# epfl-lasa/OptimalModulationDS

Measured on NVIDIA B200. Metric: mppi_rollout_state_steps_per_sec, higher is better.
Workload: dtype f32 (scoring: split-fp16 tcgen05, fp32 accumulate, fp32-accurate; obstacle-ranking prefilter: f16 tcgen05, re-scored in fp32 inside its calibrated guard band)

## Files before the change

### include/dsmppi_b200.h

```cpp
#ifndef DSMPPI_B200_H
#define DSMPPI_B200_H

#include <stdint.h>

#ifdef __cplusplus
extern "C" {
#endif

#define DSMPPI_N_KERNEL_MAX 50
#define DSMPPI_MAX_DOF 8
#define DSMPPI_MAX_LINKS 16
#define DSMPPI_MAX_CLOSEST 8
#define DSMPPI_HIDDEN 256
#define DSMPPI_MAX_HIDDEN_LAYERS 4

typedef struct dsmppi_ctx dsmppi_ctx;

typedef struct {
  int32_t n_dof;
  int32_t n_out;
  int32_t n_point_dim;
  int16_t n_hidden;
  int16_t hidden_width;
  const float* W_host[5];
  const float* b_host[5];
} dsmppi_net;

enum {
  DSMPPI_DS_LINEAR_ATTRACTOR = 0,
  DSMPPI_DS_MATRIX = 1,
  DSMPPI_DS_SEDS = 2
};
typedef struct {
  int32_t ds_kind;
  int32_t fold_activation;
  float lvel_mid, lvel_k;
  float dist_mid, dist_k;
  float ltau_max;
  float goal_act_thr;
  float repulsion;
  float reserved;
  float ds_A[DSMPPI_MAX_DOF * DSMPPI_MAX_DOF];
} dsmppi_modulation;

enum {
  DSMPPI_PASS1_EXACT_FP32 = 0,
  DSMPPI_PASS1_TC_F16 = 1,
  DSMPPI_PASS1_TC_BF16 = 2,
  DSMPPI_PASS1_AUTO = 3
};

enum {
  DSMPPI_SCORE_FFMA = 0,
  DSMPPI_SCORE_TC_SPLIT = 1,
  DSMPPI_SCORE_AUTO = 2
};

enum {
  DSMPPI_DISTANCE_NN = 0,
  DSMPPI_DISTANCE_FK = 1
};
#define DSMPPI_FK_MAX_PTS 32

typedef struct {
  int32_t N;
  int32_t H;
  int32_t q_cur_is_batch;
  int32_t n_kernels;
  int32_t n_closest;
  uint32_t ignored_link_mask;
  float dt;
  float dst_thr;
  float lin_thr;
  float rbf_p;
  float q_goal[DSMPPI_MAX_DOF];
  dsmppi_modulation mod;
  int32_t distance_provider;
  int32_t fk_n_pts;
  float fk_span[DSMPPI_FK_MAX_PTS];
  const float* q_cur_dev;
  const float* mu_tmp_dev;
  const float* sigma_tmp_dev;
  const float* alpha_tmp_dev;
  float* all_traj_dev;
  float* closest_dist_all_dev;
  float* kernel_val_all_dev;
  float* dot_products_dev;
  float* kernel_activations_dev;
  float* qdot_dev;
  float* nn_grad_all_dev;
  float* norm_basis_dev;
} dsmppi_rollout_args;

enum {
  DSMPPI_COST_JOINT_LIMITS = 1,
  DSMPPI_COST_TERMINAL_FK = 2,
  DSMPPI_COST_ALL = 3
};
typedef struct {
  int32_t N, H;
  int32_t terms;
  int32_t reserved;
  float q_goal[DSMPPI_MAX_DOF];
  float q_min[DSMPPI_MAX_DOF];
  float q_max[DSMPPI_MAX_DOF];
  const float* all_traj_dev;
  const float* closest_dist_all_dev;
  float* cost_dev;
} dsmppi_cost_args;

typedef struct {
  int32_t N, H;
  int32_t n_kernels;
  int32_t owns_sample0;
  int32_t variant;
  int32_t reserved;
  int64_t N_global;
  float ker_thr;
  float upd_rate;
  const float* cost_dev;
  const float* kernel_val_all_dev;
  const float* kernel_activations_dev;
  const float* mu_tmp_dev;
  const float* sigma_tmp_dev;
  const float* alpha_tmp_dev;
  float* mu_c_dev;
  float* sigma_c_dev;
  float* alpha_c_dev;
} dsmppi_update_args;

const char* dsmppi_last_error(void);
int dsmppi_version(void);
void dsmppi_modulation_default(dsmppi_modulation* out);
void dsmppi_modulation_toy(dsmppi_modulation* out);

int dsmppi_ctx_create(dsmppi_ctx** out, const dsmppi_net* net, const float* dh_params_host,
                      int32_t capacity, int32_t device);
int dsmppi_ctx_destroy(dsmppi_ctx* ctx);
int dsmppi_set_pass1_mode(dsmppi_ctx* ctx, int32_t mode, float guard_band);
int dsmppi_set_score_mode(dsmppi_ctx* ctx, int32_t mode);
int dsmppi_set_whole_horizon(dsmppi_ctx* ctx, int32_t on);

int dsmppi_set_obstacles(dsmppi_ctx* ctx, const float* obs_dev, int32_t M, void* stream);
int dsmppi_set_obstacles_host(dsmppi_ctx* ctx, const float* obs_host, int32_t M, void* stream);

typedef struct {
  int32_t n_gaussians;
  float seds_thr;
  const float* priors_host;
  const float* pdf_den_host;
  const float* mu_x_host;
  const float* mu_y_host;
  const float* sigma_inv_host;
  const float* A_host;
} dsmppi_seds;
int dsmppi_set_seds(dsmppi_ctx* ctx, const dsmppi_seds* seds, void* stream);

int dsmppi_rollout(dsmppi_ctx* ctx, const dsmppi_rollout_args* args, void* stream);

int dsmppi_distance_grad(dsmppi_ctx* ctx, const float* q_dev, int32_t n, int32_t n_closest,
                         uint32_t ignored_link_mask, float* distance_dev, float* nn_grad_dev, void* stream);

int dsmppi_distance_grad_fk(dsmppi_ctx* ctx, const float* q_dev, int32_t n, int32_t fk_n_pts, const float* span_host,
                            float* distance_dev, float* grad_dev, int32_t* closest_idx_dev, void* stream);

int dsmppi_debug_pass1(dsmppi_ctx* ctx, const float* q_dev, int32_t n, uint32_t ignored_link_mask, int32_t mode,
                       float* out_dev, void* stream);

int dsmppi_norm_basis(dsmppi_ctx* ctx, const float* grad_dev, int64_t n, float* basis_dev, void* stream);

int dsmppi_cost(dsmppi_ctx* ctx, const dsmppi_cost_args* args, void* stream);

int32_t dsmppi_update_packed_len(int32_t n_kernels, int32_t n_dof);
int dsmppi_update_cost_stats(dsmppi_ctx* ctx, const float* cost_dev, int32_t N, float* stats_dev, void* stream);
int dsmppi_update_partial(dsmppi_ctx* ctx, const dsmppi_update_args* args, const float* stats_dev,
                          float* packed_dev, void* stream);
int dsmppi_update_finalize(dsmppi_ctx* ctx, const dsmppi_update_args* args, const float* packed_dev,
                           int32_t* n_updated_dev, void* stream);

typedef struct {
  int32_t N, H;
  int32_t n_kernels;
  float rbf_p;
  float thr_dist, thr_kernel, thr_dot;
  const float* all_traj_dev;
  const float* closest_dist_all_dev;
  const float* dot_products_dev;
  const float* mu_c_dev;
  const float* sigma_c_dev;
  int32_t* out_index_dev;
  int32_t* count_dev;
  int64_t capacity;
} dsmppi_candidates_args;
int dsmppi_kernel_candidates(dsmppi_ctx* ctx, const dsmppi_candidates_args* args, void* stream);

enum { DSMPPI_EXCHANGE_COST_STATS = 0, DSMPPI_EXCHANGE_PACKED_SUMS = 1 };
typedef int (*dsmppi_exchange_fn)(void* user, int32_t phase);
typedef struct {
  dsmppi_rollout_args rollout;
  float q_min[DSMPPI_MAX_DOF];
  float q_max[DSMPPI_MAX_DOF];
  float ker_thr, upd_rate;
  int32_t cost_terms;
  int32_t update_variant;
  const float* q_cur_host;
  const float* mu_tmp_host;
  const float* sigma_tmp_host;
  const float* alpha_tmp_host;
  float* mu_c_host;
  float* sigma_c_host;
  float* alpha_c_host;
  float* all_traj_host;
  float* closest_dist_all_host;
  float* kernel_val_all_host;
  float* dot_products_host;
  float* kernel_activations_host;
  float* qdot_host;
  float* cost_host;
  int32_t* n_updated_host;
  int64_t h2d_bytes, d2h_bytes;
  dsmppi_exchange_fn exchange;
  void* exchange_user;
  float* stats_dev;
  float* packed_dev;
  int32_t owns_sample0;
  int32_t reserved2;
  int64_t N_global;
} dsmppi_iteration_host_args;
int dsmppi_iteration_host(dsmppi_ctx* ctx, dsmppi_iteration_host_args* args, void* stream);

typedef struct {
  dsmppi_rollout_args rollout;
  int32_t n_obs;
  int32_t reserved;
  const float* q_cur_host;
  const float* obs_host;
  const float* mu_tmp_host;
  const float* sigma_tmp_host;
  const float* alpha_tmp_host;
  float* all_traj_host;
  float* closest_dist_all_host;
  float* kernel_val_all_host;
  float* dot_products_host;
  float* kernel_activations_host;
  float* qdot_host;
  float* nn_grad_all_host;
  int32_t recaptured;
  int32_t reserved2;
} dsmppi_tick_args;
int dsmppi_tick(dsmppi_ctx* ctx, dsmppi_tick_args* args, void* stream);

int64_t dsmppi_launch_count(const dsmppi_ctx* ctx);
int dsmppi_pass1_stats(dsmppi_ctx* ctx, int64_t* rescored_pairs, int64_t* band_overflows, int32_t* mode,
                       void* stream);
int dsmppi_exactness_stats(dsmppi_ctx* ctx, int64_t* capacity_retries, int64_t* exact_fallbacks, float* guard_band,
                           float* calibration_error);
int dsmppi_score_stats(dsmppi_ctx* ctx, int32_t* mode, int64_t* range_fixup_rows, int64_t* dropped_rows, void* stream);
int dsmppi_enable_kernel_timing(dsmppi_ctx* ctx, int32_t on);
int dsmppi_kernel_timing(dsmppi_ctx* ctx, double* pass1_ms_per_launch, int32_t* pass1_launches,
                         double* exact_ms_per_launch, int32_t* exact_launches);
int dsmppi_kernel_timing_ex(dsmppi_ctx* ctx, int32_t* kind, double* ms_per_launch, int32_t* launches);

#ifdef __cplusplus
}
#endif
#endif
```

### optimalmodulationds_b200/MPPI.py

```python
import contextlib
import os
import time
from math import pi

import numpy as np
import torch
from torch.profiler import ProfilerActivity, profile, record_function

from . import _capi
from .cost import Cost
from .fk_num import *
from .policy import *
from .policy import TensorPolicyMPPI


def generalized_sigmoid(x, y_min, y_max, x0, x1, k):
    return y_min + (y_max - y_min) / (1 + torch.exp(k * (-x + (x0 + x1) / 2)))


_ROLLOUT_TAGS = ("TAG: Nominal vector field", "TAG: evaluate NN", "TAG: evaluate NN_2 (forward pass)",
                 "TAG: evaluate NN_3 (get closest obstacle)", "TAG: evaluate NN_4 (forward+backward pass)",
                 "TAG: evaluate NN_5 (process outputs)", "TAG: QR decomposition", "TAG: Modulation-propagation",
                 "TAG: Apply policies", "TAG: Apply policy", "TAG: Propagate")
_DISTANCE_TAGS = ("TAG: evaluate NN_1 (build input)",) + _ROLLOUT_TAGS[2:6]


@contextlib.contextmanager
def _stage_tags(names):
    if not torch.autograd._profiler_enabled():
        yield
        return
    with contextlib.ExitStack() as stack:
        for n in names:
            stack.enter_context(record_function(n))
        yield


_NET_FAMILY = ("the supported distance networks are 3(d+P) -> W -> ... -> W -> O MLPs without skips: 1 to 4 hidden "
               "layers of one width W <= 256, O <= 16 outputs")


def _network_arrays(nn_model):
    if len(getattr(nn_model.model, 'skips', ()) or ()) > 0:
        raise NotImplementedError(f"skip connections are not supported; {_NET_FAMILY}")
    lin = [m for m in nn_model.model.modules() if isinstance(m, torch.nn.Linear)]
    W = [m.weight.detach().to('cpu', torch.float32).contiguous() for m in lin]
    b = [m.bias.detach().to('cpu', torch.float32).contiguous() for m in lin]
    L = len(W) - 1
    if not 1 <= L <= _capi.MAX_HIDDEN_LAYERS:
        raise NotImplementedError(f"found {max(L, 0)} hidden layers; {_NET_FAMILY}")
    width = W[0].shape[0]
    shapes = [(width, 3 * nn_model.in_channels)] + [(width, width)] * (L - 1) + [(nn_model.out_channels, width)]
    if [tuple(w.shape) for w in W] != shapes or not 1 <= width <= _capi.MAX_HIDDEN \
            or not 1 <= nn_model.out_channels <= _capi.MAX_LINKS:
        raise NotImplementedError(f"layer shapes {[tuple(w.shape) for w in W]}; {_NET_FAMILY}")
    return W, b


class MPPI:
    _TOY = False
    _COST_TERMS = _capi.COST_ALL
    _UPDATE_VARIANT = 0
    _DEFAULT_DST_THR = 0.5
    _COST_CLASS = Cost

    def __init__(self, q0: torch.Tensor, qf: torch.Tensor, dh_params: torch.Tensor, obs: torch.Tensor, dt: float,
                 dt_H: int, N_traj: int, DS_ARRAY, dh_a, nn_model, n_closest_obs):
        self.tensor_args = {'device': q0.device, 'dtype': q0.dtype}
        if q0.dtype != torch.float32:
            raise NotImplementedError("the CUDA path computes in fp32 (as every reference script does)")
        if not torch.cuda.is_available():
            raise RuntimeError("optimalmodulationds_b200.MPPI needs a CUDA device (B200); there is no CPU fallback")
        self._lib = _capi.load()
        if q0.is_cuda:
            self._dev = q0.device
        else:
            self._dev = torch.device('cuda', int(os.environ.get('DSMPPI_DEVICE', os.environ.get('LOCAL_RANK', 0))))
        self.n_dof = q0.shape[0]
        self.Policy = TensorPolicyMPPI(N_traj, self.n_dof, self.tensor_args)
        self.Policy._backend = self
        self.q0 = q0
        self.DS_idx = 0
        self.DS_ARRAY = DS_ARRAY
        self.DS = DS_ARRAY[self.DS_idx]
        self.qf = self.DS.q_goal.squeeze()
        self.dh_params = dh_params
        self.obs = obs
        self.n_obs = obs.shape[0]
        self.dt = dt
        self.dt_H = dt_H
        self.N_traj = N_traj
        self.dh_a = dh_a
        self.nn_model = nn_model
        self.q_cur = q0
        self.policy_upd_rate = 0.1
        self.dst_thr = self._DEFAULT_DST_THR
        self.ker_thr = 1e-3
        self.ignored_links = [0, 1, 2] if self.n_dof >= 7 else []
        self.n_closest_obs = n_closest_obs
        self.distance_provider = 'nn'
        self.fk_n_pts = 10
        self.traj_range = torch.arange(self.N_traj, device=q0.device)
        self.kernel_obstacle_bases_tmp = torch.zeros((self.Policy.N_KERNEL_MAX, self.n_dof, self.n_dof),
                                                     **self.tensor_args)
        self._shard = None
        self._mirror = {}
        self._norm_basis = None
        self._ctx = None
        self._make_context()
        self.Cost = self._COST_CLASS(self.qf, self.dh_params, backend=self)
        self.reset_tensors()
        self.qdot = torch.zeros((self.N_traj, self.n_dof), **self.tensor_args)
        self.nn_grad = torch.zeros(N_traj, self.n_dof, **self.tensor_args)
        self.ker_w = torch.zeros((N_traj, 0, 1), **self.tensor_args)
        self.cur_cost = torch.zeros(N_traj, **self.tensor_args)
        for _ in range(5):
            self.Policy.sample_policy()
        self.propagate()

    def _make_context(self):
        W, b = _network_arrays(self.nn_model)
        self._point_dim = int(self.nn_model.in_channels) - self.n_dof
        if self._point_dim not in (2, 3):
            raise ValueError(f"network takes {self.nn_model.in_channels} inputs, q0 has {self.n_dof} joints: "
                             "expected n_dof + 3 (or n_dof + 2 for the planar toy net)")
        net = _capi.Net()
        net.n_dof, net.n_out, net.n_point_dim = self.n_dof, self.nn_model.out_channels, self._point_dim
        net.n_hidden, net.hidden_width = len(W) - 1, W[0].shape[0]
        for i in range(len(W)):
            net.W_host[i] = W[i].data_ptr()
            net.b_host[i] = b[i].data_ptr()
        dh = self.dh_params.detach().to('cpu', torch.float32).contiguous()
        if dh.dim() != 2 or dh.shape[1] != 4 or dh.shape[0] < self.n_dof + 1:
            raise ValueError("dh_params must be (n_dof + 1, 4) = [d, theta, a, alpha]")
        dh = dh[:self.n_dof + 1].contiguous()
        handle = _capi.C.c_void_p()
        with torch.cuda.device(self._dev):
            _capi.check(self._lib.dsmppi_ctx_create(_capi.C.byref(handle), _capi.C.byref(net), dh.data_ptr(),
                                                    int(self.N_traj), int(self._dev.index or 0)))
        self._ctx = handle

    def __del__(self):
        ctx, self._ctx = getattr(self, '_ctx', None), None
        if ctx:
            try:
                self._lib.dsmppi_ctx_destroy(ctx)
            except Exception:
                pass

    def _stream(self):
        return _capi.C.c_void_p(torch.cuda.current_stream(self._dev).cuda_stream)

    def _host_vec(self, t):
        if isinstance(t, torch.Tensor):
            cache = self.__dict__.setdefault('_hostvec_cache', {})
            hit = cache.get(id(t))
            if hit is not None and hit[0] is t and hit[1] == t._version:
                return hit[2]
            vals = t.detach().reshape(-1).to('cpu', torch.float32).tolist()
            if len(cache) > 64:
                cache.clear()
            cache[id(t)] = (t, t._version, vals)
            return vals
        return torch.as_tensor(t).detach().reshape(-1).to('cpu', torch.float32).tolist()

    def _d(self, t):
        return torch.as_tensor(t).detach().to(self._dev, torch.float32).contiguous()

    def _u(self, t):
        return t if t.device == self.tensor_args['device'] else t.to(self.tensor_args['device'])

    def _dev_of(self, user_tensor):
        hit = self._mirror.get(id(user_tensor))
        if hit is not None and hit[0] is user_tensor and hit[1] == user_tensor._version:
            return hit[2]
        return self._d(user_tensor)

    def _remember(self, user_tensor, dev_tensor):
        self._mirror[id(user_tensor)] = (user_tensor, user_tensor._version, dev_tensor)

    def set_pass1_mode(self, mode='auto', guard_band=0.0):
        code = {'exact': _capi.PASS1_EXACT_FP32, 'tc_f16': _capi.PASS1_TC_F16, 'tc_bf16': _capi.PASS1_TC_BF16,
                'auto': _capi.PASS1_AUTO}[mode]
        _capi.check(self._lib.dsmppi_set_pass1_mode(self._ctx, code, float(guard_band)))
        self._pass1_forced = mode
        self.__dict__.pop('_tick', None)

    def set_score_mode(self, mode='auto'):
        code = {'ffma': _capi.SCORE_FFMA, 'tc_split': _capi.SCORE_TC_SPLIT, 'auto': _capi.SCORE_AUTO}[mode]
        _capi.check(self._lib.dsmppi_set_score_mode(self._ctx, code))
        self.__dict__.pop('_tick', None)

    def score_stats(self):
        mode, fix, drop = _capi.C.c_int32(), _capi.C.c_int64(), _capi.C.c_int64()
        _capi.check(self._lib.dsmppi_score_stats(self._ctx, _capi.C.byref(mode), _capi.C.byref(fix),
                                                 _capi.C.byref(drop), self._stream()))
        return dict(mode={_capi.SCORE_FFMA: 'ffma', _capi.SCORE_TC_SPLIT: 'tc_split'}[mode.value],
                    range_fixup_rows=fix.value, dropped_rows=drop.value)

    def set_whole_horizon(self, on=True):
        _capi.check(self._lib.dsmppi_set_whole_horizon(self._ctx, 1 if on else 0))
        self.__dict__.pop('_tick', None)

    def _upload_obstacles(self):
        src = self.obs
        hit = getattr(self, '_obs_uploaded', None)
        if (hit is not None and isinstance(src, torch.Tensor) and hit[0] is src and hit[1] == src._version):
            return hit[2]
        obs = self._d(self.obs)
        if obs.dim() != 2 or obs.shape[1] != self._point_dim + 1:
            raise ValueError("obs must be (M, 4) = [x, y, z, r]" if self._point_dim == 3 else
                             "obs must be (M, 3) = [x, y, r] for a network with n_dof + 2 inputs")
        self.n_obs = obs.shape[0]
        _capi.check(self._lib.dsmppi_set_obstacles(self._ctx, obs.data_ptr(), int(obs.shape[0]), self._stream()))
        if isinstance(src, torch.Tensor):
            self._obs_uploaded = (src, src._version, obs)
        return obs

    def _ignore_mask(self):
        mask = 0
        for link in self.ignored_links:
            mask |= 1 << int(link)
        return mask

    def reset_DS(self, DS):
        self.DS = DS
        self.qf = DS.q_goal.squeeze()
        self._rebuild_cost()

    def switch_DS_idx(self, idx):
        self.DS_idx = idx
        self.DS = self.DS_ARRAY[idx]
        self.qf = self.DS.q_goal.squeeze()
        self._rebuild_cost()

    def _rebuild_cost(self):
        old = getattr(self, 'Cost', None)
        self.Cost = self._COST_CLASS(self.qf, self.dh_params, backend=self)
        if old is not None:
            self.Cost.q_min, self.Cost.q_max = old.q_min, old.q_max

    def reset_tensors(self):
        N, H, d = self.N_traj, self.dt_H, self.n_dof
        a = self.tensor_args
        self.all_traj = torch.zeros(N, H, d, **a)
        self.closest_dist_all = 100 + torch.zeros(N, H, **a)
        self.kernel_val_all = torch.zeros(N, H, self.Policy.N_KERNEL_MAX, **a)
        self.dot_products = torch.zeros(N, H, **a)
        self.kernel_activations = torch.zeros(N, H, **a)

    def build_nn_input(self, q_tens, obs_tens):
        self.nn_input = torch.hstack((q_tens.tile(obs_tens.shape[0], 1), obs_tens.repeat_interleave(q_tens.shape[0], 0)))
        return self.nn_input

    def _modulation(self, mod):
        if self._TOY:
            self._lib.dsmppi_modulation_toy(_capi.C.byref(mod))
        else:
            self._lib.dsmppi_modulation_default(_capi.C.byref(mod))
        if hasattr(self.DS, 'Mu') and hasattr(self.DS, 'Sigma'):
            mod.ds_kind = _capi.DS_SEDS
            self._upload_seds(self.DS)
        elif hasattr(self.DS, 'lin_thr'):
            mod.ds_kind = _capi.DS_LINEAR_ATTRACTOR
        elif hasattr(self.DS, 'A'):
            mod.ds_kind = _capi.DS_MATRIX
            A = torch.as_tensor(self.DS.A).detach().to('cpu', torch.float32)
            if A.shape != (self.n_dof, self.n_dof):
                raise ValueError("the matrix DS needs A of shape (n_dof, n_dof)")
            for r in range(self.n_dof):
                for c in range(self.n_dof):
                    mod.ds_A[r * _capi.MAX_DOF + c] = float(A[r, c])
        else:
            raise NotImplementedError("the CUDA rollout implements the LinDS attractor (LinDS.py), the SEDS mixture "
                                      "(SEDS.py) and the matrix DS v = (q - qf) @ A (MPPI_toy.py:89) as nominal "
                                      "dynamics")

    def _upload_seds(self, ds):
        if getattr(self, '_seds_uploaded', None) is ds:
            return
        from .SEDS import SEDS as _SEDS
        src = ds if isinstance(ds, _SEDS) else _SEDS.from_arrays(ds.Mu, ds.Sigma, ds.Priors, ds.q_goal)
        if src.dof != self.n_dof:
            raise ValueError(f"SEDS has {src.dof} joints, the robot {self.n_dof}")
        arrs = [t.detach().to('cpu', torch.float32).contiguous() for t in src.kernel_arrays()]
        sd = _capi.Seds()
        sd.n_gaussians, sd.seds_thr = int(src.n_gaussians), float(getattr(ds, 'seds_thr', 1e-2))
        (sd.priors_host, sd.pdf_den_host, sd.mu_x_host, sd.mu_y_host, sd.sigma_inv_host,
         sd.A_host) = (t.data_ptr() for t in arrs)
        with torch.cuda.device(self._dev):
            _capi.check(self._lib.dsmppi_set_seds(self._ctx, _capi.C.byref(sd), self._stream()))
        self._seds_uploaded = ds

    def _rollout_args(self, N, H, nk, q_cur, mu, sigma, alpha, out):
        a = _capi.RolloutArgs()
        a.N, a.H, a.n_kernels, a.n_closest = N, H, nk, int(self.n_closest_obs)
        a.q_cur_is_batch = 1 if q_cur.dim() == 2 else 0
        a.ignored_link_mask = self._ignore_mask()
        a.dt, a.dst_thr = float(self.dt), float(self.dst_thr)
        self._modulation(a.mod)
        if self.distance_provider == 'fk':
            a.distance_provider, a.fk_n_pts = _capi.DISTANCE_FK, int(self.fk_n_pts)
            for i, v in enumerate(torch.linspace(0.01, 1, int(self.fk_n_pts)).tolist()):
                a.fk_span[i] = v
        elif self.distance_provider != 'nn':
            raise ValueError("distance_provider must be 'nn' or 'fk'")
        a.lin_thr, a.rbf_p = float(getattr(self.DS, 'lin_thr', 0.0)), float(self.Policy.p)
        goal = self._host_vec(self.DS.q_goal)
        for i in range(self.n_dof):
            a.q_goal[i] = goal[i]
        a.q_cur_dev = q_cur.data_ptr()
        a.mu_tmp_dev, a.sigma_tmp_dev, a.alpha_tmp_dev = mu.data_ptr(), sigma.data_ptr(), alpha.data_ptr()
        a.all_traj_dev = out['all_traj'].data_ptr()
        a.closest_dist_all_dev = out['closest'].data_ptr()
        a.kernel_val_all_dev = out['kval'].data_ptr()
        a.dot_products_dev = out['dots'].data_ptr()
        a.kernel_activations_dev = out['acts'].data_ptr()
        a.qdot_dev = out['qdot'].data_ptr()
        a.nn_grad_all_dev = out['grads'].data_ptr()
        a.norm_basis_dev = None
        return a

    _TICK_MAX_STATE_STEPS = 4096

    def _tick_eligible(self, q_cur):
        if os.environ.get('DSMPPI_GRAPH_TICK', '1') == '0' or self.tensor_args['device'].type != 'cpu':
            return False
        if self.N_traj * self.dt_H > self._TICK_MAX_STATE_STEPS or self.distance_provider != 'nn':
            return False
        if self._shard is not None or hasattr(self.DS, 'Mu') or getattr(self, '_timing_on', False):
            return False
        if int(self.obs.shape[0]) >= 64 or getattr(self, '_pass1_forced', 'auto') not in ('auto', 'exact'):
            return False
        obs = self.obs
        return (isinstance(obs, torch.Tensor) and obs.dim() == 2 and obs.shape[1] == self._point_dim + 1
                and obs.dtype == torch.float32 and q_cur.dtype == torch.float32)

    def _tick_key(self, nk, q_batch):
        DS = self.DS
        A = getattr(DS, 'A', None)
        return (nk, q_batch, int(self.n_closest_obs), self._ignore_mask(), float(self.dt), float(self.dst_thr),
                float(self.Policy.p), type(DS), tuple(self._host_vec(DS.q_goal)), float(getattr(DS, 'lin_thr', 0.0)),
                None if A is None else tuple(self._host_vec(A)))

    def _propagate_tick(self, q_cur_user, nk):
        N, H, d = self.N_traj, self.dt_H, self.n_dof
        P = self.Policy
        q_batch = q_cur_user.dim() == 2
        key = self._tick_key(nk, q_batch)
        t = self.__dict__.get('_tick')
        if t is None or t['key'] != key:
            dummy = torch.empty(1, device=self._dev)
            probe = torch.empty((N, d) if q_batch else (d,), device='meta')
            out = {k: dummy for k in ('all_traj', 'closest', 'kval', 'dots', 'acts', 'qdot', 'grads')}
            ta = _capi.TickArgs()
            ta.rollout = self._rollout_args(N, H, nk, dummy, dummy, dummy, dummy, out)
            ta.rollout.q_cur_is_batch = 1 if probe.dim() == 2 else 0
            t = self._tick = dict(key=key, args=ta, keep=dummy)
        ta = t['args']
        obs = self.obs if self.obs.is_contiguous() else self.obs.contiguous()
        q = q_cur_user if q_cur_user.is_contiguous() else q_cur_user.contiguous()
        ta.n_obs = int(obs.shape[0])
        ta.q_cur_host, ta.obs_host = q.data_ptr(), obs.data_ptr()
        mu, sg, al = P.mu_tmp, P.sigma_tmp, P.alpha_tmp
        if nk > 0:
            if not (mu.is_contiguous() and sg.is_contiguous() and al.is_contiguous()):
                mu, sg, al = mu.contiguous(), sg.contiguous(), al.contiguous()
            ta.mu_tmp_host, ta.sigma_tmp_host, ta.alpha_tmp_host = mu.data_ptr(), sg.data_ptr(), al.data_ptr()
        traj, closest, kv = torch.empty(N, H, d), torch.empty(N, H), torch.empty(N, H, P.N_KERNEL_MAX)
        dots, acts, qdot, grads = torch.empty(N, H), torch.empty(N, H), torch.empty(N, d), torch.empty(N, H, d)
        ta.all_traj_host, ta.closest_dist_all_host, ta.kernel_val_all_host = traj.data_ptr(), closest.data_ptr(), kv.data_ptr()
        ta.dot_products_host, ta.kernel_activations_host = dots.data_ptr(), acts.data_ptr()
        ta.qdot_host, ta.nn_grad_all_host = qdot.data_ptr(), grads.data_ptr()
        _capi.check(self._lib.dsmppi_tick(self._ctx, _capi.C.byref(ta), self._stream()))
        self._mirror = {}
        self._obs_uploaded = None
        self._norm_basis = None
        self._dev_last = dict(grads=None, grads_host=grads, nk=nk)
        self.all_traj, self.closest_dist_all, self.kernel_val_all = traj, closest, kv
        self.dot_products, self.kernel_activations, self.qdot = dots, acts, qdot
        self.nn_grad = grads[:, H - 1, :]
        self.ker_w = kv[:, H - 1, :nk].unsqueeze(2)
        return (traj, closest, kv[:, :, 0:nk], dots, acts)

    def propagate(self):
        N, H, d = self.N_traj, self.dt_H, self.n_dof
        P = self.Policy
        nk = int(P.n_kernels)
        dev = self._dev
        q_user = torch.as_tensor(self.q_cur)
        if self._tick_eligible(q_user):
            if q_user.shape not in ((d,), (N, d)):
                raise ValueError(f"q_cur must be ({d},) or ({N}, {d}), got {tuple(q_user.shape)}")
            with _stage_tags(_ROLLOUT_TAGS):
                return self._propagate_tick(q_user, nk)
        with torch.cuda.device(dev):
            q_cur = self._d(self.q_cur)
            if q_cur.shape not in ((d,), (N, d)):
                raise ValueError(f"q_cur must be ({d},) or ({N}, {d}), got {tuple(q_cur.shape)}")
            mu, sigma, alpha = self._d(P.mu_tmp), self._d(P.sigma_tmp), self._d(P.alpha_tmp)
            if mu.shape != (N, P.N_KERNEL_MAX, d):
                raise ValueError("Policy.mu_tmp must be (N_traj, 50, n_dof)")
            self._upload_obstacles()
            out = dict(all_traj=torch.empty(N, H, d, device=dev), closest=torch.empty(N, H, device=dev),
                       kval=torch.zeros(N, H, P.N_KERNEL_MAX, device=dev), dots=torch.empty(N, H, device=dev),
                       acts=torch.empty(N, H, device=dev), qdot=torch.empty(N, d, device=dev),
                       grads=torch.empty(N, H, d, device=dev))
            args = self._rollout_args(N, H, nk, q_cur, mu, sigma, alpha, out)
            with _stage_tags(_ROLLOUT_TAGS):
                _capi.check(self._lib.dsmppi_rollout(self._ctx, _capi.C.byref(args), self._stream()))
        self._mirror = {}
        self._dev_last = dict(out, mu=mu, sigma=sigma, alpha=alpha, nk=nk)
        self._norm_basis = None
        if self.tensor_args['device'] == dev:
            self.all_traj, self.closest_dist_all, self.kernel_val_all = out['all_traj'], out['closest'], out['kval']
            self.dot_products, self.kernel_activations, self.qdot = out['dots'], out['acts'], out['qdot']
        else:
            self.all_traj, self.closest_dist_all = self._u(out['all_traj']), self._u(out['closest'])
            self.dot_products, self.kernel_activations = self._u(out['dots']), self._u(out['acts'])
            self.qdot = self._u(out['qdot'])
            kv = torch.zeros(N, H, P.N_KERNEL_MAX, **self.tensor_args)
            if nk > 0:
                kv[:, :, :nk] = self._u(out['kval'][:, :, :nk])
            self.kernel_val_all = kv
        for user, key in ((self.all_traj, 'all_traj'), (self.closest_dist_all, 'closest'),
                          (self.kernel_val_all, 'kval'), (self.kernel_activations, 'acts')):
            self._remember(user, out[key])
        self._remember(P.mu_tmp, mu), self._remember(P.sigma_tmp, sigma), self._remember(P.alpha_tmp, alpha)
        self.nn_grad = self._u(out['grads'][:, H - 1, :])
        self.ker_w = self.kernel_val_all[:, H - 1, :nk].unsqueeze(2)
        return (self.all_traj, self.closest_dist_all, self.kernel_val_all[:, :, 0:nk], self.dot_products,
                self.kernel_activations)

    @property
    def norm_basis(self):
        if self._norm_basis is None:
            g = self._dev_last['grads']
            if g is None:
                g = self._d(self._dev_last['grads_host'])
            N, H, d = g.shape
            with torch.cuda.device(self._dev):
                E = torch.empty(N, H, d, d, device=self._dev)
                _capi.check(self._lib.dsmppi_norm_basis(self._ctx, g.data_ptr(), N * H, E.data_ptr(), self._stream()))
            self._norm_basis = self._u(E)
        return self._norm_basis

    @norm_basis.setter
    def norm_basis(self, value):
        self._norm_basis = value

    def distance_repulsion_nn(self, q_prev, aot=False):
        q = self._d(q_prev)
        n = q.shape[0]
        with torch.cuda.device(self._dev):
            self._upload_obstacles()
            dist = torch.empty(n, device=self._dev)
            grad = torch.empty(n, self.n_dof, device=self._dev)
            with _stage_tags(_DISTANCE_TAGS):
                _capi.check(self._lib.dsmppi_distance_grad(self._ctx, q.data_ptr(), n, int(self.n_closest_obs),
                                                           self._ignore_mask(), dist.data_ptr(), grad.data_ptr(),
                                                           self._stream()))
        self.nn_grad = self._u(grad)
        return self._u(dist), self.nn_grad

    def distance_repulsion_fk(self, q_prev, return_indices=False):
        q = self._d(q_prev)
        n = q.shape[0]
        n_pts = int(self.fk_n_pts)
        span = torch.linspace(0.01, 1, n_pts).contiguous()
        with torch.cuda.device(self._dev):
            self._upload_obstacles()
            dist = torch.empty(n, device=self._dev)
            grad = torch.empty(n, self.n_dof, device=self._dev)
            idx = torch.empty(n, 3, dtype=torch.int32, device=self._dev)
            _capi.check(self._lib.dsmppi_distance_grad_fk(self._ctx, q.data_ptr(), n, n_pts, span.data_ptr(),
                                                          dist.data_ptr(), grad.data_ptr(), idx.data_ptr(),
                                                          self._stream()))
        rep = torch.zeros(n, max(7, self.n_dof), device=self._dev)
        rep[:, :self.n_dof] = grad
        rep = self._u(rep)
        self.nn_grad = rep[:, 0:self.n_dof]
        if return_indices:
            return self._u(dist), rep, self._u(idx)
        return self._u(dist), rep

    def update_kernel_normal_bases(self):
        nk = int(self.Policy.n_kernels)
        if nk > 0:
            _, grad = self.distance_repulsion_nn(self.Policy.mu_c[0:nk], aot=False)
            g = self._d(grad)
            with torch.cuda.device(self._dev):
                E = torch.empty(nk, self.n_dof, self.n_dof, device=self._dev)
                _capi.check(self._lib.dsmppi_norm_basis(self._ctx, g.data_ptr(), nk, E.data_ptr(), self._stream()))
            self.Policy.kernel_obstacle_bases[0:nk] = E.to(self.Policy.kernel_obstacle_bases.device)
        return 0

    def evaluate_costs(self, cost_obj, all_traj, closest_dist_all):
        N, H, d = all_traj.shape
        a = _capi.CostArgs()
        a.N, a.H, a.terms = N, H, self._COST_TERMS
        goal, qmin, qmax = self._host_vec(cost_obj.qf), self._host_vec(cost_obj.q_min), self._host_vec(cost_obj.q_max)
        if len(qmin) < d or len(qmax) < d:
            raise ValueError("Cost.q_min / q_max must have n_dof entries")
        for i in range(d):
            a.q_goal[i], a.q_min[i], a.q_max[i] = goal[i], qmin[i], qmax[i]
        with torch.cuda.device(self._dev):
            tr, cd = self._dev_of(all_traj), self._dev_of(closest_dist_all)
            cost = torch.empty(N, device=self._dev)
            a.all_traj_dev, a.closest_dist_all_dev, a.cost_dev = tr.data_ptr(), cd.data_ptr(), cost.data_ptr()
            _capi.check(self._lib.dsmppi_cost(self._ctx, _capi.C.byref(a), self._stream()))
        user = self._u(cost)
        self._remember(user, cost)
        return user

    def kernel_candidates(self, policy, all_traj, closest_dist_all, dot_products, thr_dist, thr_kernel, thr_dot):
        N, H, d = all_traj.shape
        nk = int(policy.n_kernels)
        a = _capi.CandidatesArgs()
        a.N, a.H, a.n_kernels, a.rbf_p = N, H, nk, float(policy.p)
        a.thr_dist, a.thr_kernel, a.thr_dot = float(thr_dist), float(thr_kernel), float(thr_dot)
        with torch.cuda.device(self._dev):
            tr, cd, dp = self._dev_of(all_traj), self._dev_of(closest_dist_all), self._dev_of(dot_products)
            mu_c, sigma_c = self._d(policy.mu_c), self._d(policy.sigma_c)
            count = torch.zeros(1, dtype=torch.int32, device=self._dev)
            cap = min(N * H, 1 << 20)
            while True:
                idx = torch.empty(cap, dtype=torch.int32, device=self._dev)
                a.all_traj_dev, a.closest_dist_all_dev, a.dot_products_dev = tr.data_ptr(), cd.data_ptr(), dp.data_ptr()
                a.mu_c_dev, a.sigma_c_dev = mu_c.data_ptr(), sigma_c.data_ptr()
                a.out_index_dev, a.count_dev, a.capacity = idx.data_ptr(), count.data_ptr(), cap
                _capi.check(self._lib.dsmppi_kernel_candidates(self._ctx, _capi.C.byref(a), self._stream()))
                n = int(count.item())
                if n <= cap:
                    break
                cap = N * H
            order = torch.sort(idx[:n].long())[0]
            cand = tr.reshape(-1, d)[order]
        return self._u(cand)

    def get_cost(self):
        self.cur_cost = self.Cost.evaluate_costs(self.all_traj, self.closest_dist_all)
        return self.cur_cost

    def get_qdot(self, mode='best'):
        qdot = 0
        if mode == 'best':
            qdot = self.qdot[torch.argmin(self.cur_cost), :]
        elif mode == 'weighted':
            beta = self.cur_cost.mean() / 50
            w = torch.exp(-1 / beta * self.cur_cost)
            w = w / w.sum()
            qdot = torch.sum(w.unsqueeze(1) * self.qdot, dim=0)
        return qdot

    def enable_sample_sharding(self, group=None):
        import torch.distributed as dist
        world = dist.get_world_size(group)
        n = torch.tensor([float(self.N_traj)], device=self._dev)
        dist.all_reduce(n, group=group)
        self._shard = dict(group=group, rank=dist.get_rank(group), world=world, N_global=int(round(float(n))))

    def shift_policy_means(self):
        P = self.Policy
        nk = int(P.n_kernels)
        N, H, d = self.N_traj, self.dt_H, self.n_dof
        dev = self._dev
        with torch.cuda.device(dev):
            a = _capi.UpdateArgs()
            a.N, a.H, a.n_kernels = N, H, nk
            a.owns_sample0, a.N_global, a.variant = 1, N, self._UPDATE_VARIANT
            a.ker_thr, a.upd_rate = float(self.ker_thr), float(self.policy_upd_rate)
            cost = self._dev_of(self.cur_cost)
            kv, acts = self._dev_of(self.kernel_val_all), self._dev_of(self.kernel_activations)
            mu, sigma, alpha = self._dev_of(P.mu_tmp), self._dev_of(P.sigma_tmp), self._dev_of(P.alpha_tmp)
            mu_c, sigma_c, alpha_c = (self._d(t).clone() for t in (P.mu_c, P.sigma_c, P.alpha_c))
            a.cost_dev, a.kernel_val_all_dev, a.kernel_activations_dev = cost.data_ptr(), kv.data_ptr(), acts.data_ptr()
            a.mu_tmp_dev, a.sigma_tmp_dev, a.alpha_tmp_dev = mu.data_ptr(), sigma.data_ptr(), alpha.data_ptr()
            a.mu_c_dev, a.sigma_c_dev, a.alpha_c_dev = mu_c.data_ptr(), sigma_c.data_ptr(), alpha_c.data_ptr()
            stats = torch.empty(4, device=dev)
            packed = torch.empty(int(self._lib.dsmppi_update_packed_len(nk, d)), device=dev)
            n_upd = torch.zeros(1, dtype=torch.int32, device=dev)
            st = self._stream()
            _capi.check(self._lib.dsmppi_update_cost_stats(self._ctx, cost.data_ptr(), N, stats.data_ptr(), st))
            if self._shard is not None:
                from .parallel import allreduce_cost_stats, allreduce_packed
                a.owns_sample0 = 1 if self._shard['rank'] == 0 else 0
                a.N_global = self._shard['N_global']
                allreduce_cost_stats(stats, self._shard['group'])
            _capi.check(self._lib.dsmppi_update_partial(self._ctx, _capi.C.byref(a), stats.data_ptr(),
                                                        packed.data_ptr(), st))
            if self._shard is not None:
                allreduce_packed(packed, self._shard['group'])
            _capi.check(self._lib.dsmppi_update_finalize(self._ctx, _capi.C.byref(a), packed.data_ptr(),
                                                         n_upd.data_ptr(), st))
        if nk > 0:
            P.mu_c[0:nk] = mu_c[0:nk].to(P.mu_c.device)
            P.sigma_c[0:nk] = sigma_c[0:nk].to(P.sigma_c.device)
            P.alpha_c[0:nk] = alpha_c[0:nk].to(P.alpha_c.device)
        self._last_stats = stats
        return 0, n_upd.to(self.tensor_args['device'])[0].to(torch.int64)

    def iteration_host(self, host):
        N, H, d = self.N_traj, self.dt_H, self.n_dof
        P = self.Policy
        a = _capi.IterationHostArgs()
        dummy = torch.empty(1, device=self._dev)
        out = {k: dummy for k in ('all_traj', 'closest', 'kval', 'dots', 'acts', 'qdot', 'grads')}
        r = self._rollout_args(N, H, int(P.n_kernels), host['q_cur'], dummy, dummy, dummy, out)
        a.rollout = r
        qmin, qmax = self._host_vec(self.Cost.q_min), self._host_vec(self.Cost.q_max)
        for i in range(d):
            a.q_min[i], a.q_max[i] = qmin[i], qmax[i]
        a.ker_thr, a.upd_rate = float(self.ker_thr), float(self.policy_upd_rate)
        a.cost_terms, a.update_variant = self._COST_TERMS, self._UPDATE_VARIANT
        for name in ('q_cur', 'mu_tmp', 'sigma_tmp', 'alpha_tmp', 'mu_c', 'sigma_c', 'alpha_c', 'all_traj',
                     'closest_dist_all', 'kernel_val_all', 'dot_products', 'kernel_activations', 'qdot', 'cost',
                     'n_updated'):
            t = host[name]
            assert t.device.type == 'cpu' and t.is_contiguous(), name
            setattr(a, name + '_host', t.data_ptr())
        with torch.cuda.device(self._dev):
            self._upload_obstacles()
            if self._shard is not None:
                from .parallel import allreduce_cost_stats, allreduce_packed
                group = self._shard['group']
                stats = torch.empty(4, device=self._dev)
                packed = torch.empty(int(self._lib.dsmppi_update_packed_len(int(P.n_kernels), d)), device=self._dev)

                def exchange(_user, phase):
                    try:
                        if phase == _capi.EXCHANGE_COST_STATS:
                            allreduce_cost_stats(stats, group)
                        else:
                            allreduce_packed(packed, group)
                        return 0
                    except Exception:
                        import traceback
                        traceback.print_exc()
                        return 1
                hook = _capi.ExchangeFn(exchange)
                a.exchange, a.stats_dev, a.packed_dev = hook, stats.data_ptr(), packed.data_ptr()
                a.owns_sample0 = 1 if self._shard['rank'] == 0 else 0
                a.N_global = self._shard['N_global']
            _capi.check(self._lib.dsmppi_iteration_host(self._ctx, _capi.C.byref(a), self._stream()))
        return int(a.h2d_bytes), int(a.d2h_bytes)

    def update_obstacles(self, obs):
        self.obs = obs
        self.n_obs = obs.shape[0]
        return 0

    def launch_count(self):
        return int(self._lib.dsmppi_launch_count(self._ctx))

    def exactness_stats(self):
        r, f, g, e = _capi.C.c_int64(), _capi.C.c_int64(), _capi.C.c_float(), _capi.C.c_float()
        _capi.check(self._lib.dsmppi_exactness_stats(self._ctx, _capi.C.byref(r), _capi.C.byref(f), _capi.C.byref(g),
                                                     _capi.C.byref(e)))
        return dict(capacity_retries=r.value, exact_fallbacks=f.value, guard_band=g.value, calibration_error=e.value)

    def pass1_stats(self):
        a, b, m = _capi.C.c_int64(), _capi.C.c_int64(), _capi.C.c_int32()
        _capi.check(self._lib.dsmppi_pass1_stats(self._ctx, _capi.C.byref(a), _capi.C.byref(b), _capi.C.byref(m),
                                                 self._stream()))
        return dict(rescored_pairs=a.value, band_overflows=b.value, mode=m.value)

    def debug_pass1(self, q, mode='exact'):
        code = {'exact': _capi.PASS1_EXACT_FP32, 'tc_f16': _capi.PASS1_TC_F16, 'tc_bf16': _capi.PASS1_TC_BF16}[mode]
        qd = self._d(q)
        with torch.cuda.device(self._dev):
            obs = self._upload_obstacles()
            out = torch.empty(qd.shape[0], obs.shape[0], device=self._dev)
            _capi.check(self._lib.dsmppi_debug_pass1(self._ctx, qd.data_ptr(), int(qd.shape[0]), self._ignore_mask(),
                                                     code, out.data_ptr(), self._stream()))
        return out

    def enable_kernel_timing(self, on=True):
        _capi.check(self._lib.dsmppi_enable_kernel_timing(self._ctx, 1 if on else 0))
        self._timing_on = bool(on)

    def kernel_timing_ex(self):
        k, ms, n = _capi.C.c_int32(), _capi.C.c_double(), _capi.C.c_int32()
        _capi.check(self._lib.dsmppi_kernel_timing_ex(self._ctx, _capi.C.byref(k), _capi.C.byref(ms), _capi.C.byref(n)))
        name = {0: 'exact_mlp_kernel', 1: 'tc_pass1_kernel', 2: 'rollout_fused_kernel', 3: 'tc_exact_kernel',
                4: 'tc_exact_kernel<whole horizon>'}[k.value]
        return dict(kernel=name, ms=ms.value, launches=n.value)

    def kernel_timing(self):
        p, pn, e, en = _capi.C.c_double(), _capi.C.c_int32(), _capi.C.c_double(), _capi.C.c_int32()
        _capi.check(self._lib.dsmppi_kernel_timing(self._ctx, _capi.C.byref(p), _capi.C.byref(pn), _capi.C.byref(e),
                                                   _capi.C.byref(en)))
        return dict(pass1_ms=p.value, pass1_launches=pn.value, exact_ms=e.value, exact_launches=en.value)
```

### optimalmodulationds_b200/_capi.py

```python
import ctypes as C
import os

_HERE = os.path.dirname(os.path.abspath(__file__))
LIB_PATH = os.environ.get("DSMPPI_LIB") or os.path.join(_HERE, "libdsmppi_b200.so")

N_KERNEL_MAX = 50
MAX_DOF = 8
MAX_LINKS = 16
MAX_CLOSEST = 8
MAX_HIDDEN = 256
MAX_HIDDEN_LAYERS = 4

PASS1_EXACT_FP32, PASS1_TC_F16, PASS1_TC_BF16, PASS1_AUTO = 0, 1, 2, 3
SCORE_FFMA, SCORE_TC_SPLIT, SCORE_AUTO = 0, 1, 2

_fp = C.c_void_p


DS_LINEAR_ATTRACTOR, DS_MATRIX, DS_SEDS = 0, 1, 2
DISTANCE_NN, DISTANCE_FK = 0, 1
FK_MAX_PTS = 32
COST_JOINT_LIMITS, COST_TERMINAL_FK, COST_ALL = 1, 2, 3


class Net(C.Structure):
    _fields_ = [("n_dof", C.c_int32), ("n_out", C.c_int32), ("n_point_dim", C.c_int32),
                ("n_hidden", C.c_int16), ("hidden_width", C.c_int16),
                ("W_host", _fp * 5), ("b_host", _fp * 5)]


class Modulation(C.Structure):
    _fields_ = [
        ("ds_kind", C.c_int32), ("fold_activation", C.c_int32),
        ("lvel_mid", C.c_float), ("lvel_k", C.c_float), ("dist_mid", C.c_float), ("dist_k", C.c_float),
        ("ltau_max", C.c_float), ("goal_act_thr", C.c_float), ("repulsion", C.c_float), ("reserved", C.c_float),
        ("ds_A", C.c_float * (MAX_DOF * MAX_DOF)),
    ]


class Seds(C.Structure):
    _fields_ = [("n_gaussians", C.c_int32), ("seds_thr", C.c_float), ("priors_host", _fp), ("pdf_den_host", _fp),
                ("mu_x_host", _fp), ("mu_y_host", _fp), ("sigma_inv_host", _fp), ("A_host", _fp)]


class RolloutArgs(C.Structure):
    _fields_ = [
        ("N", C.c_int32), ("H", C.c_int32), ("q_cur_is_batch", C.c_int32), ("n_kernels", C.c_int32),
        ("n_closest", C.c_int32), ("ignored_link_mask", C.c_uint32),
        ("dt", C.c_float), ("dst_thr", C.c_float), ("lin_thr", C.c_float), ("rbf_p", C.c_float),
        ("q_goal", C.c_float * MAX_DOF), ("mod", Modulation),
        ("distance_provider", C.c_int32), ("fk_n_pts", C.c_int32), ("fk_span", C.c_float * FK_MAX_PTS),
        ("q_cur_dev", _fp), ("mu_tmp_dev", _fp), ("sigma_tmp_dev", _fp), ("alpha_tmp_dev", _fp),
        ("all_traj_dev", _fp), ("closest_dist_all_dev", _fp), ("kernel_val_all_dev", _fp),
        ("dot_products_dev", _fp), ("kernel_activations_dev", _fp), ("qdot_dev", _fp),
        ("nn_grad_all_dev", _fp), ("norm_basis_dev", _fp),
    ]


class CostArgs(C.Structure):
    _fields_ = [
        ("N", C.c_int32), ("H", C.c_int32), ("terms", C.c_int32), ("reserved", C.c_int32),
        ("q_goal", C.c_float * MAX_DOF), ("q_min", C.c_float * MAX_DOF), ("q_max", C.c_float * MAX_DOF),
        ("all_traj_dev", _fp), ("closest_dist_all_dev", _fp), ("cost_dev", _fp),
    ]


class UpdateArgs(C.Structure):
    _fields_ = [
        ("N", C.c_int32), ("H", C.c_int32), ("n_kernels", C.c_int32), ("owns_sample0", C.c_int32),
        ("variant", C.c_int32), ("reserved", C.c_int32), ("N_global", C.c_int64), ("ker_thr", C.c_float), ("upd_rate", C.c_float),
        ("cost_dev", _fp), ("kernel_val_all_dev", _fp), ("kernel_activations_dev", _fp),
        ("mu_tmp_dev", _fp), ("sigma_tmp_dev", _fp), ("alpha_tmp_dev", _fp),
        ("mu_c_dev", _fp), ("sigma_c_dev", _fp), ("alpha_c_dev", _fp),
    ]


class CandidatesArgs(C.Structure):
    _fields_ = [
        ("N", C.c_int32), ("H", C.c_int32), ("n_kernels", C.c_int32), ("rbf_p", C.c_float),
        ("thr_dist", C.c_float), ("thr_kernel", C.c_float), ("thr_dot", C.c_float),
        ("all_traj_dev", _fp), ("closest_dist_all_dev", _fp), ("dot_products_dev", _fp),
        ("mu_c_dev", _fp), ("sigma_c_dev", _fp), ("out_index_dev", _fp), ("count_dev", _fp),
        ("capacity", C.c_int64),
    ]


EXCHANGE_COST_STATS, EXCHANGE_PACKED_SUMS = 0, 1
ExchangeFn = C.CFUNCTYPE(C.c_int, C.c_void_p, C.c_int32)


class IterationHostArgs(C.Structure):
    _fields_ = [
        ("rollout", RolloutArgs),
        ("q_min", C.c_float * MAX_DOF), ("q_max", C.c_float * MAX_DOF),
        ("ker_thr", C.c_float), ("upd_rate", C.c_float), ("cost_terms", C.c_int32), ("update_variant", C.c_int32),
        ("q_cur_host", _fp), ("mu_tmp_host", _fp), ("sigma_tmp_host", _fp), ("alpha_tmp_host", _fp),
        ("mu_c_host", _fp), ("sigma_c_host", _fp), ("alpha_c_host", _fp),
        ("all_traj_host", _fp), ("closest_dist_all_host", _fp), ("kernel_val_all_host", _fp),
        ("dot_products_host", _fp), ("kernel_activations_host", _fp), ("qdot_host", _fp),
        ("cost_host", _fp), ("n_updated_host", _fp),
        ("h2d_bytes", C.c_int64), ("d2h_bytes", C.c_int64),
        ("exchange", ExchangeFn), ("exchange_user", C.c_void_p), ("stats_dev", _fp), ("packed_dev", _fp),
        ("owns_sample0", C.c_int32), ("reserved2", C.c_int32), ("N_global", C.c_int64),
    ]


class TickArgs(C.Structure):
    _fields_ = [
        ("rollout", RolloutArgs), ("n_obs", C.c_int32), ("reserved", C.c_int32),
        ("q_cur_host", _fp), ("obs_host", _fp), ("mu_tmp_host", _fp), ("sigma_tmp_host", _fp), ("alpha_tmp_host", _fp),
        ("all_traj_host", _fp), ("closest_dist_all_host", _fp), ("kernel_val_all_host", _fp),
        ("dot_products_host", _fp), ("kernel_activations_host", _fp), ("qdot_host", _fp), ("nn_grad_all_host", _fp),
        ("recaptured", C.c_int32), ("reserved2", C.c_int32),
    ]


EXPORTS = {
    "dsmppi_last_error": (C.c_char_p, []),
    "dsmppi_version": (C.c_int, []),
    "dsmppi_modulation_default": (None, [C.POINTER(Modulation)]),
    "dsmppi_modulation_toy": (None, [C.POINTER(Modulation)]),
    "dsmppi_ctx_create": (C.c_int, [C.POINTER(C.c_void_p), C.POINTER(Net), _fp, C.c_int32, C.c_int32]),
    "dsmppi_ctx_destroy": (C.c_int, [C.c_void_p]),
    "dsmppi_set_pass1_mode": (C.c_int, [C.c_void_p, C.c_int32, C.c_float]),
    "dsmppi_set_score_mode": (C.c_int, [C.c_void_p, C.c_int32]),
    "dsmppi_set_whole_horizon": (C.c_int, [C.c_void_p, C.c_int32]),
    "dsmppi_set_seds": (C.c_int, [C.c_void_p, C.POINTER(Seds), C.c_void_p]),
    "dsmppi_set_obstacles": (C.c_int, [C.c_void_p, _fp, C.c_int32, C.c_void_p]),
    "dsmppi_set_obstacles_host": (C.c_int, [C.c_void_p, _fp, C.c_int32, C.c_void_p]),
    "dsmppi_rollout": (C.c_int, [C.c_void_p, C.POINTER(RolloutArgs), C.c_void_p]),
    "dsmppi_distance_grad": (C.c_int, [C.c_void_p, _fp, C.c_int32, C.c_int32, C.c_uint32, _fp, _fp, C.c_void_p]),
    "dsmppi_distance_grad_fk": (C.c_int, [C.c_void_p, _fp, C.c_int32, C.c_int32, _fp, _fp, _fp, _fp, C.c_void_p]),
    "dsmppi_debug_pass1": (C.c_int, [C.c_void_p, _fp, C.c_int32, C.c_uint32, C.c_int32, _fp, C.c_void_p]),
    "dsmppi_norm_basis": (C.c_int, [C.c_void_p, _fp, C.c_int64, _fp, C.c_void_p]),
    "dsmppi_cost": (C.c_int, [C.c_void_p, C.POINTER(CostArgs), C.c_void_p]),
    "dsmppi_kernel_candidates": (C.c_int, [C.c_void_p, C.POINTER(CandidatesArgs), C.c_void_p]),
    "dsmppi_update_packed_len": (C.c_int32, [C.c_int32, C.c_int32]),
    "dsmppi_update_cost_stats": (C.c_int, [C.c_void_p, _fp, C.c_int32, _fp, C.c_void_p]),
    "dsmppi_update_partial": (C.c_int, [C.c_void_p, C.POINTER(UpdateArgs), _fp, _fp, C.c_void_p]),
    "dsmppi_update_finalize": (C.c_int, [C.c_void_p, C.POINTER(UpdateArgs), _fp, _fp, C.c_void_p]),
    "dsmppi_iteration_host": (C.c_int, [C.c_void_p, C.POINTER(IterationHostArgs), C.c_void_p]),
    "dsmppi_tick": (C.c_int, [C.c_void_p, C.POINTER(TickArgs), C.c_void_p]),
    "dsmppi_launch_count": (C.c_int64, [C.c_void_p]),
    "dsmppi_pass1_stats": (C.c_int, [C.c_void_p, C.POINTER(C.c_int64), C.POINTER(C.c_int64), C.POINTER(C.c_int32),
                                     C.c_void_p]),
    "dsmppi_exactness_stats": (C.c_int, [C.c_void_p, C.POINTER(C.c_int64), C.POINTER(C.c_int64), C.POINTER(C.c_float),
                                         C.POINTER(C.c_float)]),
    "dsmppi_score_stats": (C.c_int, [C.c_void_p, C.POINTER(C.c_int32), C.POINTER(C.c_int64), C.POINTER(C.c_int64),
                                     C.c_void_p]),
    "dsmppi_enable_kernel_timing": (C.c_int, [C.c_void_p, C.c_int32]),
    "dsmppi_kernel_timing": (C.c_int, [C.c_void_p, C.POINTER(C.c_double), C.POINTER(C.c_int32),
                                       C.POINTER(C.c_double), C.POINTER(C.c_int32)]),
    "dsmppi_kernel_timing_ex": (C.c_int, [C.c_void_p, C.POINTER(C.c_int32), C.POINTER(C.c_double),
                                          C.POINTER(C.c_int32)]),
}

_lib = None


def load():
    global _lib
    if _lib is not None:
        return _lib
    if not os.path.exists(LIB_PATH):
        raise RuntimeError(
            f"{LIB_PATH} is missing: build it with `python -m optimalmodulationds_b200.build` "
            "(there is no CPU or PyTorch fallback for the MPPI rollout)")
    lib = C.CDLL(LIB_PATH)
    for name, (res, args) in EXPORTS.items():
        fn = getattr(lib, name)
        fn.restype = res
        fn.argtypes = args
    _lib = lib
    return lib


def check(status):
    if status != 0:
        msg = load().dsmppi_last_error()
        raise RuntimeError("libdsmppi_b200: " + (msg.decode() if msg else f"error {status}"))
```

### optimalmodulationds_b200/csrc/capi.cu

```cuda
#include <cstdlib>
#include <cstring>
#include <vector>

#include "internal.cuh"

static thread_local std::string g_last_error;
void dsmppi_set_error(const std::string& msg) { g_last_error = msg; }

namespace {

template <typename T>
int grow(T*& p, size_t& cap, size_t need) {
  if (need <= cap) return 0;
  if (p) CUDA_TRY(cudaFree(p));
  p = nullptr;
  const size_t n = need + need / 8;
  CUDA_TRY(cudaMalloc(reinterpret_cast<void**>(&p), n * sizeof(T)));
  cap = n;
  return 0;
}

template <typename T>
int alloc(T*& p, size_t n) {
  if (p) CUDA_TRY(cudaFree(p));
  p = nullptr;
  CUDA_TRY(cudaMalloc(reinterpret_cast<void**>(&p), (n ? n : 1) * sizeof(T)));
  return 0;
}

constexpr int FUSE_M_MAX = 16;

int resolve_mode(const dsmppi_ctx* c, int requested, int M) {
  int m = requested;
  if (m == DSMPPI_PASS1_AUTO) m = (M >= 64 && c->tc_blob) ? DSMPPI_PASS1_TC_F16 : DSMPPI_PASS1_EXACT_FP32;
  if (m != DSMPPI_PASS1_EXACT_FP32 && !c->tc_blob) m = DSMPPI_PASS1_EXACT_FP32;
  return m;
}

int band_slot(int mode) { return mode == DSMPPI_PASS1_TC_BF16 ? 1 : 0; }

long long sample_block(const dsmppi_ctx* c) {
  const long long block = (1LL << 28) / c->M;
  return block > (1 << 18) ? 1 << 18 : block < 1 ? 1 : block;
}

dsmppi_rollout_args slice_samples(const dsmppi_rollout_args& a, int d, long long off, int n) {
  dsmppi_rollout_args b = a;
  b.N = n;
  if (a.q_cur_is_batch) b.q_cur_dev = a.q_cur_dev + off * d;
  if (a.mu_tmp_dev) b.mu_tmp_dev = a.mu_tmp_dev + off * NKMAX * d;
  if (a.sigma_tmp_dev) b.sigma_tmp_dev = a.sigma_tmp_dev + off * NKMAX;
  if (a.alpha_tmp_dev) b.alpha_tmp_dev = a.alpha_tmp_dev + off * NKMAX * d;
  b.all_traj_dev = a.all_traj_dev + off * a.H * d;
  b.closest_dist_all_dev = a.closest_dist_all_dev + off * a.H;
  b.kernel_val_all_dev = a.kernel_val_all_dev + off * a.H * NKMAX;
  b.dot_products_dev = a.dot_products_dev + off * a.H;
  b.kernel_activations_dev = a.kernel_activations_dev + off * a.H;
  b.qdot_dev = a.qdot_dev + off * d;
  b.nn_grad_all_dev = a.nn_grad_all_dev + off * a.H * d;
  return b;
}

constexpr int WHOLE_M_MAX = 32;

bool use_whole_horizon(const dsmppi_ctx* c, int n, int mode) {
  if (!c->fused_rollout || mode != DSMPPI_PASS1_EXACT_FP32) return false;
  if (use_tc_scoring(c)) {
    if (c->M > WHOLE_M_MAX) return false;
    const long long per_pair = 2LL * (128 / c->M);
    return (n + per_pair - 1) / per_pair <= c->sm_count / 2;
  }
  if (c->M <= FUSE_M_MAX) return true;
  return c->M <= WHOLE_M_MAX && n <= 2 * c->sm_count;
}

int timing_mark(dsmppi_ctx* c, int kind, cudaStream_t st) {
  if (!c->timing) return 0;
  if (c->ev_used >= (int)c->ev.size()) {
    cudaEvent_t e;
    CUDA_TRY(cudaEventCreate(&e));
    c->ev.push_back(e);
  }
  c->ev_kind = kind;
  CUDA_TRY(cudaEventRecord(c->ev[c->ev_used++], st));
  return 0;
}

int average_event_pairs(dsmppi_ctx* c, double* avg_ms, int* pairs) {
  double tot = 0.0;
  int n = 0;
  for (int i = 0; i + 1 < c->ev_used; i += 2) {
    CUDA_TRY(cudaEventSynchronize(c->ev[i + 1]));
    float ms = 0.f;
    CUDA_TRY(cudaEventElapsedTime(&ms, c->ev[i], c->ev[i + 1]));
    tot += ms;
    ++n;
  }
  *avg_ms = n ? tot / n : 0.0;
  *pairs = n;
  return 0;
}

int ensure_workspace(dsmppi_ctx* c, int n, int M, int mode) {
  const size_t list_rows_now = cand_list_cap(c, n);
  if (n <= c->ws_n && M <= c->ws_M && mode == c->ws_mode && list_rows_now <= c->rowlist_cap) return 0;
  const int nn = n > c->ws_n ? n : c->ws_n;
  const int mm = M > c->ws_M ? M : c->ws_M;
  const int d = c->d;
  if (nn > c->ws_n) {
    if (alloc(c->q_work, (size_t)nn * d) || alloc(c->cand_cnt, (size_t)nn) ||
        alloc(c->row_base, (size_t)nn) || alloc(c->sel, (size_t)nn * MAXK) ||
        alloc(c->sel_rows, (size_t)nn * MAXK) || alloc(c->dist_tmp, (size_t)nn) || alloc(c->grad_tmp, (size_t)nn * d))
      return 1;
  }
  const size_t list_rows = cand_list_cap(c, nn);
  size_t rows = (mode == DSMPPI_PASS1_EXACT_FP32) ? (size_t)nn * mm : list_rows;
  if (rows < list_rows) rows = list_rows;
  if (grow(c->m_rows, c->m_rows_cap, rows)) return 1;
  size_t drows = list_rows;
  if (mm <= WHOLE_M_MAX && (size_t)nn * mm > drows) drows = (size_t)nn * mm;
  if (grow(c->row_dist, c->row_dist_cap, drows)) return 1;
  if (grow(c->row_grad, c->row_grad_cap, drows * d)) return 1;
  size_t cap = c->rowlist_cap;
  if (grow(c->row_sample, cap, list_rows)) return 1;
  if (grow(c->row_obs, c->rowlist_cap, list_rows)) return 1;
  if (mode != DSMPPI_PASS1_EXACT_FP32) {
    if (grow(c->mdist, c->mdist_cap, (size_t)nn * mm)) return 1;
  }
  c->ws_n = nn;
  c->ws_M = mm;
  c->ws_mode = mode;
  return 0;
}

struct Frame {
  std::vector<float> W[5], b[5];
  dsmppi_net net{};
};

Frame embed_net(const dsmppi_net* src, int nenc, int L, int W) {
  Frame f;
  const int O = src->n_out;
  for (int l = 0; l < 4; ++l) {
    const int in = l == 0 ? nenc : HID, in_src = l == 0 ? nenc : W;
    f.W[l].assign((size_t)HID * in, 0.f);
    f.b[l].assign(HID, 0.f);
    for (int o = 0; o < W; ++o) {
      if (l < L) {
        for (int k = 0; k < in_src; ++k) f.W[l][(size_t)o * in + k] = src->W_host[l][(size_t)o * in_src + k];
        f.b[l][o] = src->b_host[l][o];
      } else {
        f.W[l][(size_t)o * in + o] = 1.f;
      }
    }
  }
  f.W[4].assign((size_t)O * HID, 0.f);
  for (int o = 0; o < O; ++o)
    for (int k = 0; k < W; ++k) f.W[4][(size_t)o * HID + k] = src->W_host[L][(size_t)o * W + k];
  f.b[4].assign(src->b_host[L], src->b_host[L] + O);
  f.net = *src;
  f.net.n_hidden = MAXL;
  f.net.hidden_width = HID;
  for (int l = 0; l < 5; ++l) {
    f.net.W_host[l] = f.W[l].data();
    f.net.b_host[l] = f.b[l].data();
  }
  return f;
}

void tick_free(dsmppi_ctx* c);

}

extern "C" {

const char* dsmppi_last_error(void) { return g_last_error.c_str(); }
int dsmppi_version(void) { return 102; }

void dsmppi_modulation_default(dsmppi_modulation* m) {
  if (!m) return;
  std::memset(m, 0, sizeof(*m));
  m->ds_kind = DSMPPI_DS_LINEAR_ATTRACTOR;
  m->lvel_mid = (-1.f + 0.f) / 2.f; m->lvel_k = 10.f;
  m->dist_mid = (0.0f + 0.1f) / 2.f; m->dist_k = 100.f;
  m->ltau_max = 5.f;
  m->goal_act_thr = 0.5f;
  m->repulsion = 0.1f;
}

void dsmppi_modulation_toy(dsmppi_modulation* m) {
  if (!m) return;
  std::memset(m, 0, sizeof(*m));
  m->ds_kind = DSMPPI_DS_MATRIX;
  for (int i = 0; i < MAXD; ++i) m->ds_A[i * MAXD + i] = -1.f;
  m->fold_activation = 1;
  m->lvel_mid = (float)((-0.2 + 0.0) / 2); m->lvel_k = 100.f;
  m->dist_mid = (0.0f + 0.5f) / 2.f; m->dist_k = 30.f;
  m->ltau_max = 3.f;
  m->goal_act_thr = 0.3f;
  m->repulsion = 0.05f;
}

int dsmppi_ctx_create(dsmppi_ctx** out, const dsmppi_net* net, const float* dh_params_host, int32_t capacity,
                      int32_t device) {
  REQUIRE(out && net && dh_params_host, "null argument");
  REQUIRE(net->n_dof >= 1 && net->n_dof <= MAXD, "n_dof out of range (1..8)");
  REQUIRE(net->n_out >= 1 && net->n_out <= MAXO, "n_out out of range (1..16)");
  REQUIRE(capacity >= 1, "capacity must be positive");
  const int P = net->n_point_dim == 0 ? 3 : net->n_point_dim;
  REQUIRE(P == 2 || P == 3, "n_point_dim must be 2 or 3");
  const int L = net->n_hidden == 0 ? MAXL : net->n_hidden;
  const int W = net->hidden_width == 0 ? HID : net->hidden_width;
  REQUIRE(L >= 1 && L <= MAXL && W >= 1 && W <= HID,
          "unsupported network shape: the supported family is 1..4 hidden layers of one width 1..256 (n_hidden, "
          "hidden_width)");
  int ndev = 0;
  CUDA_TRY(cudaGetDeviceCount(&ndev));
  REQUIRE(ndev > 0 && device < ndev, "no such CUDA device (this library has no CPU fallback)");
  CUDA_TRY(cudaSetDevice(device));
  cudaDeviceProp prop;
  CUDA_TRY(cudaGetDeviceProperties(&prop, device));
  REQUIRE(prop.major == 10, "libdsmppi_b200 is built for sm_100a (B200) only");
  dsmppi_ctx* c = new dsmppi_ctx();
  c->device = device;
  c->sm_count = prop.multiProcessorCount;
  c->d = net->n_dof;
  c->O = net->n_out;
  c->P = P;
  c->nin = c->d + P;
  c->nenc = 3 * c->nin;
  c->capacity = capacity;
  for (int i = 0; i <= c->d; ++i)
    for (int j = 0; j < 4; ++j) c->dh.v[i][j] = dh_params_host[i * 4 + j];
  const Frame fr = embed_net(net, c->nenc, L, W);
  const dsmppi_net* fnet = &fr.net;
  const int in_dim[5] = {c->nenc, HID, HID, HID, HID};
  auto pad = [](size_t x) { return (x + 63) / 64 * 64; };
  size_t total = 0, off_f[4], off_b[4], off_w4, off_bias[5];
  for (int l = 0; l < 4; ++l) { off_f[l] = total; total += pad((size_t)in_dim[l] * HID); }
  for (int l = 0; l < 4; ++l) { off_b[l] = total; total += pad((size_t)in_dim[l] * HID); }
  off_w4 = total; total += pad((size_t)c->O * HID);
  for (int l = 0; l < 5; ++l) { off_bias[l] = total; total += pad(HID); }
  std::vector<float> blob(total, 0.f);
  for (int l = 0; l < 4; ++l) {
    const float* Wl = fnet->W_host[l];
    for (int o = 0; o < HID; ++o)
      for (int k = 0; k < in_dim[l]; ++k) {
        blob[off_f[l] + (size_t)k * HID + o] = Wl[(size_t)o * in_dim[l] + k];
        blob[off_b[l] + (size_t)o * in_dim[l] + k] = Wl[(size_t)o * in_dim[l] + k];
      }
    std::memcpy(&blob[off_bias[l]], fnet->b_host[l], HID * sizeof(float));
  }
  std::memcpy(&blob[off_w4], fnet->W_host[4], (size_t)c->O * HID * sizeof(float));
  std::memcpy(&blob[off_bias[4]], fnet->b_host[4], (size_t)c->O * sizeof(float));
  if (cudaMalloc(reinterpret_cast<void**>(&c->weights_blob), total * sizeof(float)) != cudaSuccess) {
    delete c;
    dsmppi_set_error("cudaMalloc(weights) failed");
    return 1;
  }
  CUDA_TRY(cudaMemcpy(c->weights_blob, blob.data(), total * sizeof(float), cudaMemcpyHostToDevice));
  c->net.d = c->d; c->net.nin = c->nin; c->net.nenc = c->nenc; c->net.O = c->O;
  c->net.scale = (c->O == 9) ? 0.01f : 1.f;
  c->net.nh = L;
  c->net.width = W;
  for (int l = 0; l < 4; ++l) {
    c->net.Wf[l] = c->weights_blob + off_f[l];
    c->net.Wb[l] = c->weights_blob + off_b[l];
  }
  c->net.W4 = c->weights_blob + off_w4;
  for (int l = 0; l < 5; ++l) c->net.b[l] = c->weights_blob + off_bias[l];
  if (exact_set_attributes()) { delete c; return 1; }
  if (tc_build_images(c, fnet)) { delete c; return 1; }
  if (tcx_build_images(c, fnet)) { delete c; return 1; }
  if (const char* e = std::getenv("DSMPPI_HALF_TILES")) c->half_tiles = std::atoi(e) != 0;
  if (const char* e = std::getenv("DSMPPI_PASS1_ACC")) c->pass1_hacc = std::strcmp(e, "f32") != 0;
  c->upd_blocks = c->sm_count * 4;
  CUDA_TRY(cudaMalloc(reinterpret_cast<void**>(&c->upd_partials),
                      (size_t)c->upd_blocks * dsmppi_update_packed_len(NKMAX, MAXD) * sizeof(float)));
  CUDA_TRY(cudaMalloc(reinterpret_cast<void**>(&c->stats_tmp), 4 * sizeof(float)));
  CUDA_TRY(cudaMalloc(reinterpret_cast<void**>(&c->stats_part), 3 * 1024 * sizeof(float)));
  CUDA_TRY(cudaMalloc(reinterpret_cast<void**>(&c->stats_ticket), sizeof(unsigned int)));
  CUDA_TRY(cudaMemset(c->stats_ticket, 0, sizeof(unsigned int)));
  CUDA_TRY(cudaMalloc(reinterpret_cast<void**>(&c->packed_tmp), dsmppi_update_packed_len(NKMAX, MAXD) * sizeof(float)));
  CUDA_TRY(cudaMalloc(reinterpret_cast<void**>(&c->counters), N_COUNTERS * sizeof(int)));
  CUDA_TRY(cudaMemset(c->counters, 0, N_COUNTERS * sizeof(int)));
  CUDA_TRY(cudaMallocHost(reinterpret_cast<void**>(&c->counters_host), N_COUNTERS * sizeof(int)));
  *out = c;
  return 0;
}

int dsmppi_ctx_destroy(dsmppi_ctx* c) {
  if (!c) return 0;
  cudaSetDevice(c->device);
  tc_free_images(c);
  tcx_free_images(c);
  void* ptrs[] = {c->weights_blob, c->seds, c->obs, c->obs_raw, c->obs_enc, c->q_work, c->m_rows, c->mdist, c->enc_q,
                  c->cand_cnt, c->row_base, c->row_sample, c->row_obs, c->counters, c->sel, c->fix_list,
                  c->sel_rows, c->row_dist, c->row_grad, c->dist_tmp, c->grad_tmp, c->upd_partials, c->stats_tmp, c->stats_part,
                  c->stats_ticket,
                  c->packed_tmp, c->stage};
  for (void* p : ptrs)
    if (p) cudaFree(p);
  tick_free(c);
  if (c->s_tick) cudaStreamDestroy(c->s_tick);
  if (c->tick_ev) cudaEventDestroy(c->tick_ev);
  if (c->counters_host) cudaFreeHost(c->counters_host);
  for (cudaEvent_t e : c->ev) cudaEventDestroy(e);
  for (cudaEvent_t e : c->pipe_ev) cudaEventDestroy(e);
  if (c->s_in) cudaStreamDestroy(c->s_in);
  if (c->s_out) cudaStreamDestroy(c->s_out);
  delete c;
  return 0;
}

int dsmppi_set_pass1_mode(dsmppi_ctx* c, int32_t mode, float guard_band) {
  REQUIRE(c, "null ctx");
  REQUIRE(mode >= 0 && mode <= 3, "bad pass-1 mode");
  c->pass1_mode = mode;
  c->guard_band = guard_band > 0.f ? guard_band : 0.f;
  return 0;
}

int dsmppi_set_score_mode(dsmppi_ctx* c, int32_t mode) {
  REQUIRE(c, "null ctx");
  REQUIRE(mode >= 0 && mode <= 2, "bad score mode");
  REQUIRE(mode != DSMPPI_SCORE_TC_SPLIT || c->tcx_blob, "this network does not fit the tensor-core scoring tiles");
  c->score_mode = mode;
  return 0;
}

int dsmppi_set_whole_horizon(dsmppi_ctx* c, int32_t on) {
  REQUIRE(c, "null ctx");
  c->fused_rollout = on ? 1 : 0;
  return 0;
}

int dsmppi_set_seds(dsmppi_ctx* c, const dsmppi_seds* sd, void* stream) {
  REQUIRE(c && sd, "null argument");
  REQUIRE(sd->n_gaussians >= 1 && sd->n_gaussians <= 32, "n_gaussians out of range (1..32)");
  REQUIRE(sd->priors_host && sd->pdf_den_host && sd->mu_x_host && sd->mu_y_host && sd->sigma_inv_host && sd->A_host,
          "null SEDS array");
  cudaStream_t st = static_cast<cudaStream_t>(stream);
  CUDA_TRY(cudaSetDevice(c->device));
  const int G = sd->n_gaussians, d = c->d;
  std::vector<float> blob;
  blob.insert(blob.end(), sd->priors_host, sd->priors_host + G);
  blob.insert(blob.end(), sd->pdf_den_host, sd->pdf_den_host + G);
  blob.insert(blob.end(), sd->mu_x_host, sd->mu_x_host + G * d);
  blob.insert(blob.end(), sd->mu_y_host, sd->mu_y_host + G * d);
  blob.insert(blob.end(), sd->sigma_inv_host, sd->sigma_inv_host + G * d * d);
  blob.insert(blob.end(), sd->A_host, sd->A_host + G * d * d);
  if (G > c->seds_G || !c->seds) {
    if (c->seds) CUDA_TRY(cudaFree(c->seds));
    c->seds = nullptr;
    CUDA_TRY(cudaMalloc(reinterpret_cast<void**>(&c->seds), blob.size() * sizeof(float)));
  }
  CUDA_TRY(cudaStreamSynchronize(st));
  CUDA_TRY(cudaMemcpy(c->seds, blob.data(), blob.size() * sizeof(float), cudaMemcpyHostToDevice));
  c->seds_G = G;
  c->seds_thr = sd->seds_thr;
  return 0;
}

int dsmppi_set_obstacles(dsmppi_ctx* c, const float* obs_dev, int32_t M, void* stream) {
  REQUIRE(c && obs_dev, "null argument");
  REQUIRE(M >= 1, "need at least one obstacle");
  cudaStream_t st = static_cast<cudaStream_t>(stream);
  CUDA_TRY(cudaSetDevice(c->device));
  if (M > c->obs_cap) {
    if (c->obs) CUDA_TRY(cudaFree(c->obs));
    c->obs = nullptr;
    CUDA_TRY(cudaMalloc(reinterpret_cast<void**>(&c->obs), (size_t)M * 4 * sizeof(float)));
    c->obs_cap = M;
  }
  if (c->P == 3) {
    CUDA_TRY(cudaMemcpyAsync(c->obs, obs_dev, (size_t)M * 4 * sizeof(float), cudaMemcpyDefault, st));
  } else {
    if (M > c->obs_raw_cap) {
      if (c->obs_raw) CUDA_TRY(cudaFree(c->obs_raw));
      c->obs_raw = nullptr;
      CUDA_TRY(cudaMalloc(reinterpret_cast<void**>(&c->obs_raw), (size_t)M * (c->P + 1) * sizeof(float)));
      c->obs_raw_cap = M;
    }
    CUDA_TRY(cudaMemcpyAsync(c->obs_raw, obs_dev, (size_t)M * (c->P + 1) * sizeof(float), cudaMemcpyDefault, st));
    if (launch_pack_obstacles(c, c->obs_raw, M, c->P, st)) return 1;
  }
  c->M = M;
  c->obs_tables_dirty = 1;
  return 0;
}

int dsmppi_set_obstacles_host(dsmppi_ctx* c, const float* obs_host, int32_t M, void* stream) {
  return dsmppi_set_obstacles(c, obs_host, M, stream);
}

}

constexpr int CAL_Q = 256;
constexpr float CAL_SAFETY = 3.f;

static int calibrate_band(dsmppi_ctx* c, const float* q, int q_stride, int n, uint32_t ignore_mask, int mode,
                          cudaStream_t st) {
  const int slot = band_slot(mode);
  const int d = c->d, M = c->M;
  const int n_act = n < CAL_Q ? n : CAL_Q;
  const int nq = CAL_Q + n_act;
  std::vector<float> hq((size_t)nq * d);
  uint64_t lcg = 0x9E3779B97F4A7C15ull;
  for (size_t i = 0; i < (size_t)CAL_Q * d; ++i) {
    lcg = lcg * 6364136223846793005ull + 1442695040888963407ull;
    hq[i] = ((float)((lcg >> 40) & 0xFFFFFF) / 16777216.f * 2.f - 1.f) * 3.14159265f;
  }
  float *dq = nullptr, *ref = nullptr, *err = nullptr;
  CUDA_TRY(cudaMalloc(reinterpret_cast<void**>(&dq), (size_t)nq * d * sizeof(float)));
  CUDA_TRY(cudaMalloc(reinterpret_cast<void**>(&ref), (size_t)nq * M * sizeof(float)));
  CUDA_TRY(cudaMalloc(reinterpret_cast<void**>(&err), sizeof(float)));
  CUDA_TRY(cudaMemcpyAsync(dq, hq.data(), (size_t)CAL_Q * d * sizeof(float), cudaMemcpyHostToDevice, st));
  CUDA_TRY(cudaMemcpy2DAsync(dq + (size_t)CAL_Q * d, d * sizeof(float), q, (size_t)q_stride * sizeof(float),
                             d * sizeof(float), n_act, cudaMemcpyDeviceToDevice, st));
  int rc = ensure_workspace(c, nq, M, mode);
  RowSrc src{};
  src.mode = ROWS_DENSE; src.M = M; src.n_rows = nq * M;
  if (!rc) rc = launch_exact_forward(c, dq, d, src, ignore_mask, ref, st);
  if (!rc) rc = tc_pass1(c, dq, d, nq, ignore_mask, mode, st);
  if (!rc) rc = launch_max_abs_diff(c, ref, c->mdist, (long long)nq * M, err, st);
  float h = 0.f;
  if (!rc) {
    CUDA_TRY(cudaMemcpyAsync(&h, err, sizeof(float), cudaMemcpyDeviceToHost, st));
    CUDA_TRY(cudaStreamSynchronize(st));
  }
  cudaFree(dq); cudaFree(ref); cudaFree(err);
  if (rc) return rc;
  c->band_cal_err[slot] = h;
  float band = CAL_SAFETY * h;
  const float floor_band = (c->O == 9 ? 1e-3f : 1e-2f);
  if (!(band > floor_band)) band = floor_band;
  c->band_cal[slot] = band;
  c->band_cal_M[slot] = M;
  return 0;
}

static int distance_pipeline(dsmppi_ctx* c, const float* q, int q_stride, int n, int K, uint32_t ignore_mask, int mode,
                             cudaStream_t st, bool table_ready = false, bool defer_rank = false) {
  REQUIRE(c->M >= 1, "obstacles not set");
  REQUIRE(K >= 1 && K <= MAXK, "n_closest_obs out of range (1..8)");
  REQUIRE(K <= c->M, "n_closest_obs exceeds the number of obstacles");
  if (mode != DSMPPI_PASS1_EXACT_FP32 && c->guard_band <= 0.f) {
    const int slot = band_slot(mode);
    if (c->band_cal[slot] <= 0.f || c->band_cal_M[slot] != c->M) {
      if (calibrate_band(c, q, q_stride, n, ignore_mask, mode, st)) return 1;
      table_ready = false;
    }
  }
  if (ensure_workspace(c, n, c->M, mode)) return 1;
  RowSrc src{};
  src.M = c->M;
  src.K = K;
  if (mode == DSMPPI_PASS1_EXACT_FP32 && c->M <= FUSE_M_MAX) {
    src.mode = ROWS_DENSE;
    src.n_rows = n * c->M;
    if (timing_mark(c, use_tc_scoring(c) ? 3 : 0, st)) return 1;
    if (launch_exact_fwdbwd(c, q, q_stride, src, ignore_mask, c->m_rows, c->row_dist, c->row_grad, 0, st)) return 1;
    if (timing_mark(c, use_tc_scoring(c) ? 3 : 0, st)) return 1;
    return launch_rank_dense(c, n, K, true, st);
  }
  if (mode == DSMPPI_PASS1_EXACT_FP32) {
    src.mode = ROWS_DENSE;
    src.n_rows = n * c->M;
    if (timing_mark(c, use_tc_scoring(c) ? 3 : 0, st)) return 1;
    if (launch_exact_forward(c, q, q_stride, src, ignore_mask, c->m_rows, st)) return 1;
    if (timing_mark(c, use_tc_scoring(c) ? 3 : 0, st)) return 1;
    if (launch_rank_dense(c, n, K, false, st)) return 1;
    RowSrc s2{};
    s2.mode = ROWS_SELECTED;
    s2.M = c->M;
    s2.K = K;
    s2.n_rows = n * K;
    s2.sel = c->sel;
    if (launch_exact_fwdbwd(c, q, q_stride, s2, ignore_mask, nullptr, c->row_dist, c->row_grad, 0, st)) return 1;
    return launch_identity_rows(c, n, K, st);
  }
  c->prefilter_used = 1;
  const float band = c->guard_band > 0.f ? c->guard_band : c->band_cal[band_slot(mode)];
  const size_t cap_rows = cand_list_cap(c, n);
  if (timing_mark(c, 1, st)) return 1;
  if (tc_pass1(c, q, q_stride, n, ignore_mask, mode, st, table_ready)) return 1;
  if (timing_mark(c, 1, st)) return 1;
  if (launch_select_candidates(c, n, K, band, cap_rows, st)) return 1;
  src.mode = ROWS_LIST;
  src.n_rows = (int)(cap_rows < 0x7fffffffu ? cap_rows : 0x7fffffffu);
  src.n_rows_dev = c->counters;
  src.row_sample = c->row_sample;
  src.row_obs = c->row_obs;
  if (launch_exact_fwdbwd(c, q, q_stride, src, ignore_mask, c->m_rows, c->row_dist, c->row_grad,
                          (long long)n * (K + 1), st))
    return 1;
  if (defer_rank) return 0;
  return launch_rank_candidates(c, n, K, st);
}

static int prefilter_verdict(dsmppi_ctx* c, int n_max, cudaStream_t st, int* verdict, int* exact_mode) {
  *verdict = 0;
  *exact_mode = 0;
  if (!c->prefilter_used) return 0;
  CUDA_TRY(cudaMemcpyAsync(c->counters_host, c->counters, N_COUNTERS * sizeof(int), cudaMemcpyDeviceToHost, st));
  CUDA_TRY(cudaStreamSynchronize(st));
  const int* h = c->counters_host;
  REQUIRE(h[7] == 0, "tensor-core scoring: rows left the fp16 range and did not fit the FFMA re-scoring list "
                     "(use dsmppi_set_score_mode(DSMPPI_SCORE_FFMA) for this network)");
  if (h[9] != 0) {
    *verdict = 1;
    *exact_mode = 1;
    c->exact_fallbacks++;
    return 0;
  }
  const size_t high = (size_t)(unsigned)h[8];
  if (high <= cand_list_cap(c, n_max)) return 0;
  *verdict = 1;
  const size_t want = high + high / 4;
  if (want > ((size_t)1 << 27)) {
    *exact_mode = 1;
    c->exact_fallbacks++;
  } else {
    c->cand_rows_want = want;
    c->capacity_retries++;
  }
  return 0;
}

template <typename Run>
static int run_exact(dsmppi_ctx* c, int mode, int n_max, cudaStream_t st, Run&& run) {
  for (int attempt = 0;; ++attempt) {
    c->prefilter_used = 0;
    CUDA_TRY(cudaMemsetAsync(c->counters + 8, 0, 2 * sizeof(int), st));
    if (const int rc = run(mode, attempt)) return rc;
    int verdict = 0, exact = 0;
    if (const int rc = prefilter_verdict(c, n_max, st, &verdict, &exact)) return rc;
    if (!verdict) return 0;
    REQUIRE(attempt < 4, "candidate row list still too small after four attempts");
    if (exact) return run(DSMPPI_PASS1_EXACT_FP32, -1);
  }
}

static int rollout_once(dsmppi_ctx* c, const dsmppi_rollout_args* a, int mode, cudaStream_t st) {
  const int d = c->d;
  const long long block = sample_block(c);
  for (long long off = 0; off < a->N; off += block) {
    dsmppi_rollout_args b = slice_samples(*a, d, off, (int)(a->N - off < block ? a->N - off : block));
    if (launch_init_traj(c, &b, st)) return 1;
    if (a->distance_provider == DSMPPI_DISTANCE_FK) {
      if (ensure_workspace(c, b.N, c->M, mode)) return 1;
      if (launch_identity_rows(c, b.N, 1, st)) return 1;
      b.n_closest = 1;
      for (int t = 1; t <= b.H; ++t) {
        const float* q = b.all_traj_dev + (size_t)(t - 1) * d;
        if (launch_fk_distance(c, q, b.H * d, b.N, b.fk_n_pts, b.fk_span, c->row_dist, c->row_grad, d, nullptr, st))
          return 1;
        if (launch_step(c, &b, t, st)) return 1;
      }
      continue;
    }
    if (use_whole_horizon(c, b.N, mode)) {
      REQUIRE(b.n_closest >= 1 && b.n_closest <= MAXK, "n_closest_obs out of range (1..8)");
      REQUIRE(b.n_closest <= c->M, "n_closest_obs exceeds the number of obstacles");
      if (ensure_workspace(c, b.N, c->M, mode)) return 1;
      const bool tcx = use_tc_scoring(c);
      if (timing_mark(c, tcx ? 4 : 2, st)) return 1;
      if (tcx ? launch_tc_rollout(c, &b, st) : launch_rollout_fused(c, &b, st)) return 1;
      if (timing_mark(c, tcx ? 4 : 2, st)) return 1;
      continue;
    }
    if (mode != DSMPPI_PASS1_EXACT_FP32) {
      if (tc_reserve_sample_table(c, b.N)) return 1;
      for (int t = 1; t <= b.H; ++t) {
        const float* q = b.all_traj_dev + (size_t)(t - 1) * d;
        if (distance_pipeline(c, q, b.H * d, b.N, b.n_closest, b.ignored_link_mask, mode, st, t > 1, true)) return 1;
        if (launch_rank_step(c, &b, t, mode, st)) return 1;
      }
      continue;
    }
    for (int t = 1; t <= b.H; ++t) {
      const float* q = b.all_traj_dev + (size_t)(t - 1) * d;
      if (distance_pipeline(c, q, b.H * d, b.N, b.n_closest, b.ignored_link_mask, mode, st)) return 1;
      if (launch_step(c, &b, t, st)) return 1;
    }
  }
  if (a->norm_basis_dev)
    if (launch_basis(c, a->nn_grad_all_dev, (int64_t)a->N * a->H, a->norm_basis_dev, st)) return 1;
  return 0;
}

extern "C" {

int dsmppi_rollout(dsmppi_ctx* c, const dsmppi_rollout_args* a, void* stream) {
  REQUIRE(c && a, "null argument");
  REQUIRE(a->N >= 1 && a->H >= 1, "N and H must be positive");
  REQUIRE(a->n_kernels >= 0 && a->n_kernels <= NKMAX, "n_kernels out of range");
  REQUIRE(a->q_cur_dev && a->all_traj_dev && a->closest_dist_all_dev && a->kernel_val_all_dev &&
              a->dot_products_dev && a->kernel_activations_dev && a->qdot_dev && a->nn_grad_all_dev,
          "null device pointer");
  REQUIRE(a->n_kernels == 0 || (a->mu_tmp_dev && a->sigma_tmp_dev && a->alpha_tmp_dev), "null policy pointer");
  REQUIRE(a->distance_provider == DSMPPI_DISTANCE_NN || a->distance_provider == DSMPPI_DISTANCE_FK,
          "unknown distance_provider");
  REQUIRE(a->distance_provider != DSMPPI_DISTANCE_FK || (c->P == 3 && a->fk_n_pts >= 1 && a->fk_n_pts <= DSMPPI_FK_MAX_PTS),
          "the FK distance provider needs 3-D obstacles and 1..32 points per link");
  REQUIRE(a->mod.ds_kind == DSMPPI_DS_LINEAR_ATTRACTOR || a->mod.ds_kind == DSMPPI_DS_MATRIX ||
              a->mod.ds_kind == DSMPPI_DS_SEDS, "unknown mod.ds_kind");
  REQUIRE(a->mod.ds_kind != DSMPPI_DS_SEDS || (c->seds && c->seds_G > 0), "SEDS parameters not set (dsmppi_set_seds)");
  REQUIRE(a->mod.lvel_k != 0.f && a->mod.dist_k != 0.f,
          "rollout_args.mod is not initialised (dsmppi_modulation_default / _toy)");
  cudaStream_t st = static_cast<cudaStream_t>(stream);
  CUDA_TRY(cudaSetDevice(c->device));
  REQUIRE(c->M >= 1, "obstacles not set");
  if (!c->keep_counters) c->ev_used = 0;
  const int ev_start = c->ev_used;
  const long long block = sample_block(c);
  const int n_max = (int)(a->N < block ? a->N : block);
  return run_exact(c, resolve_mode(c, c->pass1_mode, c->M), n_max, st, [&](int mode, int attempt) {
    c->ev_used = ev_start;
    if (attempt > 0 || (attempt == 0 && !c->keep_counters))
      CUDA_TRY(cudaMemsetAsync(c->counters + 1, 0, 3 * sizeof(int), st));
    return rollout_once(c, a, mode, st);
  });
}

int dsmppi_distance_grad(dsmppi_ctx* c, const float* q_dev, int32_t n, int32_t n_closest, uint32_t ignored_link_mask,
                         float* distance_dev, float* nn_grad_dev, void* stream) {
  REQUIRE(c && q_dev && distance_dev && nn_grad_dev, "null argument");
  REQUIRE(n >= 1, "n must be positive");
  cudaStream_t st = static_cast<cudaStream_t>(stream);
  CUDA_TRY(cudaSetDevice(c->device));
  REQUIRE(c->M >= 1, "obstacles not set");
  const long long block = sample_block(c);
  const int mode = resolve_mode(c, c->pass1_mode, c->M);
  for (long long off = 0; off < n; off += block) {
    const int nb = (int)(n - off < block ? n - off : block);
    const int rc = run_exact(c, mode, nb, st, [&](int m, int) {
      const int r = distance_pipeline(c, q_dev + off * c->d, c->d, nb, n_closest, ignored_link_mask, m, st);
      return r ? r : launch_blend(c, nb, n_closest, distance_dev + off, nn_grad_dev + off * c->d, st);
    });
    if (rc) return rc;
  }
  return 0;
}

int dsmppi_distance_grad_fk(dsmppi_ctx* c, const float* q_dev, int32_t n, int32_t fk_n_pts, const float* span_host,
                            float* distance_dev, float* grad_dev, int32_t* closest_idx_dev, void* stream) {
  REQUIRE(c && q_dev && distance_dev && grad_dev, "null argument");
  REQUIRE(n >= 1, "n must be positive");
  REQUIRE(c->M >= 1, "obstacles not set");
  REQUIRE(c->P == 3, "the FK distance provider needs 3-D obstacles");
  CUDA_TRY(cudaSetDevice(c->device));
  return launch_fk_distance(c, q_dev, c->d, n, fk_n_pts, span_host, distance_dev, grad_dev, c->d, closest_idx_dev,
                            static_cast<cudaStream_t>(stream));
}

int dsmppi_debug_pass1(dsmppi_ctx* c, const float* q_dev, int32_t n, uint32_t ignored_link_mask, int32_t mode,
                       float* out_dev, void* stream) {
  REQUIRE(c && q_dev && out_dev, "null argument");
  REQUIRE(mode >= DSMPPI_PASS1_EXACT_FP32 && mode <= DSMPPI_PASS1_TC_BF16,
          "bad pass-1 mode (EXACT_FP32, TC_F16 or TC_BF16; AUTO is not a kernel)");
  REQUIRE(c->M >= 1, "obstacles not set");
  cudaStream_t st = static_cast<cudaStream_t>(stream);
  CUDA_TRY(cudaSetDevice(c->device));
  if (ensure_workspace(c, n, c->M, resolve_mode(c, mode, c->M))) return 1;
  const size_t bytes = (size_t)n * c->M * sizeof(float);
  if (mode == DSMPPI_PASS1_EXACT_FP32) {
    RowSrc src{};
    src.mode = ROWS_DENSE; src.M = c->M; src.n_rows = n * c->M;
    if (launch_exact_forward(c, q_dev, c->d, src, ignored_link_mask, c->m_rows, st)) return 1;
    CUDA_TRY(cudaMemcpyAsync(out_dev, c->m_rows, bytes, cudaMemcpyDeviceToDevice, st));
  } else {
    REQUIRE(c->tc_blob, "tensor-core path unavailable for this network");
    if (tc_pass1(c, q_dev, c->d, n, ignored_link_mask, mode, st)) return 1;
    CUDA_TRY(cudaMemcpyAsync(out_dev, c->mdist, bytes, cudaMemcpyDeviceToDevice, st));
  }
  return 0;
}

int dsmppi_norm_basis(dsmppi_ctx* c, const float* grad_dev, int64_t n, float* basis_dev, void* stream) {
  REQUIRE(c && grad_dev && basis_dev, "null argument");
  CUDA_TRY(cudaSetDevice(c->device));
  return launch_basis(c, grad_dev, n, basis_dev, static_cast<cudaStream_t>(stream));
}

int dsmppi_kernel_candidates(dsmppi_ctx* c, const dsmppi_candidates_args* a, void* stream) {
  REQUIRE(c && a && a->all_traj_dev && a->closest_dist_all_dev && a->dot_products_dev && a->out_index_dev &&
              a->count_dev,
          "null argument");
  REQUIRE(a->N >= 1 && a->H >= 1 && (long long)a->N * a->H < (1LL << 31), "N * H must fit 31 bits");
  REQUIRE(a->n_kernels >= 0 && a->n_kernels <= NKMAX, "n_kernels out of range");
  REQUIRE(a->n_kernels == 0 || (a->mu_c_dev && a->sigma_c_dev), "null policy pointer");
  REQUIRE(a->capacity >= 1, "capacity must be positive");
  CUDA_TRY(cudaSetDevice(c->device));
  return launch_kernel_candidates(c, a, static_cast<cudaStream_t>(stream));
}

int dsmppi_cost(dsmppi_ctx* c, const dsmppi_cost_args* a, void* stream) {
  REQUIRE(c && a && a->all_traj_dev && a->closest_dist_all_dev && a->cost_dev, "null argument");
  CUDA_TRY(cudaSetDevice(c->device));
  return launch_cost(c, a, static_cast<cudaStream_t>(stream));
}

int32_t dsmppi_update_packed_len(int32_t nk, int32_t d) { return 1 + nk * (2 * d + 3); }

int dsmppi_update_cost_stats(dsmppi_ctx* c, const float* cost_dev, int32_t N, float* stats_dev, void* stream) {
  REQUIRE(c && cost_dev && stats_dev, "null argument");
  CUDA_TRY(cudaSetDevice(c->device));
  return launch_cost_stats(c, cost_dev, N, stats_dev, static_cast<cudaStream_t>(stream));
}

int dsmppi_update_partial(dsmppi_ctx* c, const dsmppi_update_args* a, const float* stats_dev, float* packed_dev,
                          void* stream) {
  REQUIRE(c && a && stats_dev && packed_dev, "null argument");
  REQUIRE(a->n_kernels >= 0 && a->n_kernels <= NKMAX, "n_kernels out of range");
  CUDA_TRY(cudaSetDevice(c->device));
  return launch_update_partial(c, a, stats_dev, packed_dev, static_cast<cudaStream_t>(stream));
}

int dsmppi_update_finalize(dsmppi_ctx* c, const dsmppi_update_args* a, const float* packed_dev,
                           int32_t* n_updated_dev, void* stream) {
  REQUIRE(c && a && packed_dev && n_updated_dev, "null argument");
  CUDA_TRY(cudaSetDevice(c->device));
  return launch_update_finalize(c, a, packed_dev, n_updated_dev, static_cast<cudaStream_t>(stream));
}

int dsmppi_iteration_host(dsmppi_ctx* c, dsmppi_iteration_host_args* h, void* stream) {
  REQUIRE(c && h, "null argument");
  cudaStream_t st = static_cast<cudaStream_t>(stream);
  CUDA_TRY(cudaSetDevice(c->device));
  const dsmppi_rollout_args& r = h->rollout;
  const size_t N = r.N, H = r.H, d = c->d;
  REQUIRE(N >= 1 && H >= 1, "N and H must be positive");
  const size_t nk = r.n_kernels;
  size_t off = 0;
  auto take = [&](size_t n) { size_t o = off; off += (n + 3) / 4 * 4; return o; };
  const size_t o_q = take(r.q_cur_is_batch ? N * d : d), o_mu = take(N * NKMAX * d), o_sg = take(N * NKMAX),
               o_al = take(N * NKMAX * d), o_tr = take(N * H * d), o_cd = take(N * H), o_kv = take(N * H * NKMAX),
               o_dp = take(N * H), o_ka = take(N * H), o_qd = take(N * d), o_gr = take(N * H * d), o_co = take(N),
               o_muc = take(NKMAX * d), o_sgc = take(NKMAX), o_alc = take(NKMAX * d), o_nu = take(4);
  if (grow(c->stage, c->stage_cap, off)) return 1;
  float* S = c->stage;
  int64_t h2d = 0, d2h = 0;
  auto up = [&](size_t o, const float* src, size_t n) {
    h2d += (int64_t)(n * sizeof(float));
    return cudaMemcpyAsync(S + o, src, n * sizeof(float), cudaMemcpyHostToDevice, st);
  };
  auto down = [&](float* dst, size_t o, size_t n) {
    d2h += (int64_t)(n * sizeof(float));
    return cudaMemcpyAsync(dst, S + o, n * sizeof(float), cudaMemcpyDeviceToHost, st);
  };
  size_t CHUNK = (size_t)1 << 17;
  if (const char* e = std::getenv("DSMPPI_HOST_CHUNK")) CHUNK = (size_t)std::atoll(e);
  const bool pipelined = CHUNK > 0 && N > 2 * CHUNK;
  h2d += (int64_t)((r.q_cur_is_batch ? N * d : d) * sizeof(float)) + (int64_t)(N * nk * (2 * d + 1) * sizeof(float));
  if (!pipelined || !r.q_cur_is_batch)
    CUDA_TRY(cudaMemcpyAsync(S + o_q, h->q_cur_host, (r.q_cur_is_batch ? N * d : d) * sizeof(float),
                             cudaMemcpyHostToDevice, st));
  if (nk > 0 && !pipelined) {
    CUDA_TRY(cudaMemcpy2DAsync(S + o_mu, NKMAX * d * sizeof(float), h->mu_tmp_host, NKMAX * d * sizeof(float),
                               nk * d * sizeof(float), N, cudaMemcpyHostToDevice, st));
    CUDA_TRY(cudaMemcpy2DAsync(S + o_al, NKMAX * d * sizeof(float), h->alpha_tmp_host, NKMAX * d * sizeof(float),
                               nk * d * sizeof(float), N, cudaMemcpyHostToDevice, st));
    CUDA_TRY(cudaMemcpy2DAsync(S + o_sg, NKMAX * sizeof(float), h->sigma_tmp_host, NKMAX * sizeof(float),
                               nk * sizeof(float), N, cudaMemcpyHostToDevice, st));
  }
  CUDA_TRY(up(o_muc, h->mu_c_host, NKMAX * d));
  CUDA_TRY(up(o_sgc, h->sigma_c_host, NKMAX));
  CUDA_TRY(up(o_alc, h->alpha_c_host, NKMAX * d));
  dsmppi_rollout_args a = r;
  a.q_cur_dev = S + o_q; a.mu_tmp_dev = S + o_mu; a.sigma_tmp_dev = S + o_sg; a.alpha_tmp_dev = S + o_al;
  a.all_traj_dev = S + o_tr; a.closest_dist_all_dev = S + o_cd; a.kernel_val_all_dev = S + o_kv;
  a.dot_products_dev = S + o_dp; a.kernel_activations_dev = S + o_ka; a.qdot_dev = S + o_qd;
  a.nn_grad_all_dev = S + o_gr; a.norm_basis_dev = nullptr;
  dsmppi_cost_args ca{};
  ca.N = r.N; ca.H = r.H; ca.terms = h->cost_terms;
  for (int i = 0; i < MAXD; ++i) { ca.q_goal[i] = r.q_goal[i]; ca.q_min[i] = h->q_min[i]; ca.q_max[i] = h->q_max[i]; }
  ca.all_traj_dev = a.all_traj_dev; ca.closest_dist_all_dev = a.closest_dist_all_dev; ca.cost_dev = S + o_co;
  if (!pipelined) {
    if (dsmppi_rollout(c, &a, stream)) return 1;
    if (launch_cost(c, &ca, st)) return 1;
  } else {
    const size_t n_chunks = (N + CHUNK - 1) / CHUNK;
    if (!c->s_in) CUDA_TRY(cudaStreamCreateWithFlags(&c->s_in, cudaStreamNonBlocking));
    if (!c->s_out) CUDA_TRY(cudaStreamCreateWithFlags(&c->s_out, cudaStreamNonBlocking));
    while (c->pipe_ev.size() < 2 * n_chunks + 2) {
      cudaEvent_t e;
      CUDA_TRY(cudaEventCreateWithFlags(&e, cudaEventDisableTiming));
      c->pipe_ev.push_back(e);
    }
    cudaEvent_t ev_start = c->pipe_ev[2 * n_chunks], ev_drained = c->pipe_ev[2 * n_chunks + 1];
    CUDA_TRY(cudaEventRecord(ev_start, st));
    CUDA_TRY(cudaStreamWaitEvent(c->s_in, ev_start, 0));
    CUDA_TRY(cudaStreamWaitEvent(c->s_out, ev_start, 0));
    c->ev_used = 0;
    CUDA_TRY(cudaMemsetAsync(c->counters + 1, 0, 3 * sizeof(int), st));
    struct KeepCounters {
      dsmppi_ctx* c;
      explicit KeepCounters(dsmppi_ctx* ctx) : c(ctx) { c->keep_counters = 1; }
      ~KeepCounters() { c->keep_counters = 0; }
    } keep(c);
    int rc = 0;
    for (size_t k = 0; k < n_chunks && !rc; ++k) {
      const size_t o = k * CHUNK, n = N - o < CHUNK ? N - o : CHUNK;
      cudaEvent_t ev_in = c->pipe_ev[2 * k], ev_out = c->pipe_ev[2 * k + 1];
      if (r.q_cur_is_batch)
        CUDA_TRY(cudaMemcpyAsync(S + o_q + o * d, h->q_cur_host + o * d, n * d * sizeof(float), cudaMemcpyHostToDevice,
                                 c->s_in));
      if (nk > 0) {
        CUDA_TRY(cudaMemcpy2DAsync(S + o_mu + o * NKMAX * d, NKMAX * d * sizeof(float), h->mu_tmp_host + o * NKMAX * d,
                                   NKMAX * d * sizeof(float), nk * d * sizeof(float), n, cudaMemcpyHostToDevice, c->s_in));
        CUDA_TRY(cudaMemcpy2DAsync(S + o_al + o * NKMAX * d, NKMAX * d * sizeof(float), h->alpha_tmp_host + o * NKMAX * d,
                                   NKMAX * d * sizeof(float), nk * d * sizeof(float), n, cudaMemcpyHostToDevice, c->s_in));
        CUDA_TRY(cudaMemcpy2DAsync(S + o_sg + o * NKMAX, NKMAX * sizeof(float), h->sigma_tmp_host + o * NKMAX,
                                   NKMAX * sizeof(float), nk * sizeof(float), n, cudaMemcpyHostToDevice, c->s_in));
      }
      CUDA_TRY(cudaEventRecord(ev_in, c->s_in));
      CUDA_TRY(cudaStreamWaitEvent(st, ev_in, 0));
      const dsmppi_rollout_args b = slice_samples(a, c->d, (long long)o, (int)n);
      rc = dsmppi_rollout(c, &b, stream);
      if (rc) break;
      dsmppi_cost_args cb = ca;
      cb.N = (int)n;
      cb.all_traj_dev = b.all_traj_dev; cb.closest_dist_all_dev = b.closest_dist_all_dev; cb.cost_dev = ca.cost_dev + o;
      rc = launch_cost(c, &cb, st);
      if (rc) break;
      CUDA_TRY(cudaEventRecord(ev_out, st));
      CUDA_TRY(cudaStreamWaitEvent(c->s_out, ev_out, 0));
      auto down_c = [&](float* dst, size_t off_f, size_t per_sample) {
        return cudaMemcpyAsync(dst + o * per_sample, S + off_f + o * per_sample, n * per_sample * sizeof(float),
                               cudaMemcpyDeviceToHost, c->s_out);
      };
      CUDA_TRY(down_c(h->all_traj_host, o_tr, H * d));
      CUDA_TRY(down_c(h->closest_dist_all_host, o_cd, H));
      if (nk > 0)
        CUDA_TRY(cudaMemcpy2DAsync(h->kernel_val_all_host + o * H * NKMAX, NKMAX * sizeof(float),
                                   S + o_kv + o * H * NKMAX, NKMAX * sizeof(float), nk * sizeof(float), n * H,
                                   cudaMemcpyDeviceToHost, c->s_out));
      CUDA_TRY(down_c(h->dot_products_host, o_dp, H));
      CUDA_TRY(down_c(h->kernel_activations_host, o_ka, H));
      CUDA_TRY(down_c(h->qdot_host, o_qd, d));
      CUDA_TRY(down_c(h->cost_host, o_co, 1));
    }
    if (rc) return rc;
    CUDA_TRY(cudaEventRecord(ev_drained, c->s_out));
    CUDA_TRY(cudaStreamWaitEvent(st, ev_drained, 0));
  }
  const bool sharded = h->exchange != nullptr;
  REQUIRE(!sharded || (h->stats_dev && h->packed_dev && h->N_global >= r.N),
          "a sharded iteration needs stats_dev, packed_dev and N_global");
  float* stats_buf = sharded ? h->stats_dev : c->stats_tmp;
  float* packed_buf = sharded ? h->packed_dev : c->packed_tmp;
  dsmppi_update_args ua{};
  ua.N = r.N; ua.H = r.H; ua.n_kernels = r.n_kernels; ua.variant = h->update_variant;
  ua.owns_sample0 = sharded ? h->owns_sample0 : 1;
  ua.N_global = sharded ? h->N_global : r.N;
  ua.ker_thr = h->ker_thr; ua.upd_rate = h->upd_rate;
  ua.cost_dev = S + o_co; ua.kernel_val_all_dev = a.kernel_val_all_dev;
  ua.kernel_activations_dev = a.kernel_activations_dev;
  ua.mu_tmp_dev = a.mu_tmp_dev; ua.sigma_tmp_dev = a.sigma_tmp_dev; ua.alpha_tmp_dev = a.alpha_tmp_dev;
  ua.mu_c_dev = S + o_muc; ua.sigma_c_dev = S + o_sgc; ua.alpha_c_dev = S + o_alc;
  if (launch_cost_stats(c, ua.cost_dev, r.N, stats_buf, st)) return 1;
  if (sharded) REQUIRE(h->exchange(h->exchange_user, DSMPPI_EXCHANGE_COST_STATS) == 0, "exchange hook failed (cost stats)");
  if (launch_update_partial(c, &ua, stats_buf, packed_buf, st)) return 1;
  if (sharded) REQUIRE(h->exchange(h->exchange_user, DSMPPI_EXCHANGE_PACKED_SUMS) == 0, "exchange hook failed (packed sums)");
  if (launch_update_finalize(c, &ua, packed_buf, reinterpret_cast<int*>(S + o_nu), st)) return 1;
  if (!pipelined) {
    CUDA_TRY(down(h->all_traj_host, o_tr, N * H * d));
    CUDA_TRY(down(h->closest_dist_all_host, o_cd, N * H));
    if (nk > 0) {
      CUDA_TRY(cudaMemcpy2DAsync(h->kernel_val_all_host, NKMAX * sizeof(float), S + o_kv, NKMAX * sizeof(float),
                                 nk * sizeof(float), N * H, cudaMemcpyDeviceToHost, st));
    }
    CUDA_TRY(down(h->dot_products_host, o_dp, N * H));
    CUDA_TRY(down(h->kernel_activations_host, o_ka, N * H));
    CUDA_TRY(down(h->qdot_host, o_qd, N * d));
    CUDA_TRY(down(h->cost_host, o_co, N));
  } else {
    d2h += (int64_t)((N * H * d + 3 * N * H + N * d + N) * sizeof(float));
  }
  if (nk > 0) d2h += (int64_t)(N * H * nk * sizeof(float));
  CUDA_TRY(down(h->mu_c_host, o_muc, NKMAX * d));
  CUDA_TRY(down(h->sigma_c_host, o_sgc, NKMAX));
  CUDA_TRY(down(h->alpha_c_host, o_alc, NKMAX * d));
  CUDA_TRY(cudaMemcpyAsync(h->n_updated_host, S + o_nu, sizeof(int), cudaMemcpyDeviceToHost, st));
  d2h += sizeof(int);
  CUDA_TRY(cudaStreamSynchronize(st));
  h->h2d_bytes = h2d;
  h->d2h_bytes = d2h;
  return 0;
}

int64_t dsmppi_launch_count(const dsmppi_ctx* c) { return c ? c->launches : 0; }

int dsmppi_pass1_stats(dsmppi_ctx* c, int64_t* rescored_pairs, int64_t* band_overflows, int32_t* mode, void* stream) {
  REQUIRE(c, "null ctx");
  cudaStream_t st = static_cast<cudaStream_t>(stream);
  int host[4] = {0, 0, 0, 0};
  CUDA_TRY(cudaMemcpyAsync(host, c->counters, sizeof(host), cudaMemcpyDeviceToHost, st));
  CUDA_TRY(cudaStreamSynchronize(st));
  if (band_overflows) *band_overflows = host[1];
  if (rescored_pairs) {
    unsigned long long v;
    std::memcpy(&v, &host[2], sizeof(v));
    *rescored_pairs = (int64_t)v;
  }
  if (mode) *mode = resolve_mode(c, c->pass1_mode, c->M);
  return 0;
}

int dsmppi_exactness_stats(dsmppi_ctx* c, int64_t* capacity_retries, int64_t* exact_fallbacks, float* guard_band,
                           float* calibration_error) {
  REQUIRE(c, "null ctx");
  const int slot = band_slot(resolve_mode(c, c->pass1_mode, c->M));
  if (capacity_retries) *capacity_retries = c->capacity_retries;
  if (exact_fallbacks) *exact_fallbacks = c->exact_fallbacks;
  if (guard_band) *guard_band = c->guard_band > 0.f ? c->guard_band : c->band_cal[slot];
  if (calibration_error) *calibration_error = c->band_cal_err[slot];
  return 0;
}

int dsmppi_score_stats(dsmppi_ctx* c, int32_t* mode, int64_t* range_fixup_rows, int64_t* dropped_rows, void* stream) {
  REQUIRE(c, "null ctx");
  cudaStream_t st = static_cast<cudaStream_t>(stream);
  int host[2] = {0, 0};
  CUDA_TRY(cudaMemcpyAsync(host, c->counters + 6, sizeof(host), cudaMemcpyDeviceToHost, st));
  CUDA_TRY(cudaStreamSynchronize(st));
  if (mode) *mode = use_tc_scoring(c) ? DSMPPI_SCORE_TC_SPLIT : DSMPPI_SCORE_FFMA;
  if (range_fixup_rows) *range_fixup_rows = host[0];
  if (dropped_rows) *dropped_rows = host[1];
  return 0;
}

int dsmppi_enable_kernel_timing(dsmppi_ctx* c, int32_t on) {
  REQUIRE(c, "null ctx");
  c->timing = on;
  return 0;
}

int dsmppi_kernel_timing_ex(dsmppi_ctx* c, int32_t* kind, double* ms_per_launch, int32_t* launches) {
  REQUIRE(c, "null ctx");
  double avg;
  int n;
  if (average_event_pairs(c, &avg, &n)) return 1;
  if (kind) *kind = c->ev_kind;
  if (ms_per_launch) *ms_per_launch = avg;
  if (launches) *launches = n;
  return 0;
}

int dsmppi_kernel_timing(dsmppi_ctx* c, double* pass1_ms, int32_t* pass1_n, double* exact_ms, int32_t* exact_n) {
  REQUIRE(c, "null ctx");
  double avg;
  int n;
  if (average_event_pairs(c, &avg, &n)) return 1;
  if (pass1_ms) *pass1_ms = c->ev_kind == 1 ? avg : 0.0;
  if (pass1_n) *pass1_n = c->ev_kind == 1 ? n : 0;
  if (exact_ms) *exact_ms = c->ev_kind == 0 ? avg : 0.0;
  if (exact_n) *exact_n = c->ev_kind == 0 ? n : 0;
  return 0;
}

}

namespace {
struct TickLayout {
  size_t q, obs, mu, sg, al, in_total;
  size_t tr, cd, dp, ka, qd, gr, kv, out_total;
};
TickLayout tick_layout(const dsmppi_ctx* c, const dsmppi_rollout_args& r, int M) {
  TickLayout L{};
  const size_t N = r.N, H = r.H, d = c->d, P1 = c->P + 1;
  size_t off = 0;
  auto take = [&](size_t n) { size_t o = off; off += (n + 3) / 4 * 4; return o; };
  L.q = take(r.q_cur_is_batch ? N * d : d); L.obs = take((size_t)M * P1);
  L.mu = take(N * NKMAX * d); L.sg = take(N * NKMAX); L.al = take(N * NKMAX * d);
  L.in_total = off;
  off = 0;
  L.tr = take(N * H * d); L.cd = take(N * H); L.dp = take(N * H); L.ka = take(N * H); L.qd = take(N * d);
  L.gr = take(N * H * d); L.kv = take(N * H * NKMAX);
  L.out_total = off;
  return L;
}
void tick_free(dsmppi_ctx* c) {
  if (c->tick_exec) cudaGraphExecDestroy(c->tick_exec);
  if (c->tick_graph) cudaGraphDestroy(c->tick_graph);
  c->tick_exec = nullptr; c->tick_graph = nullptr;
  if (c->tick_h_in) cudaFreeHost(c->tick_h_in);
  if (c->tick_h_out) cudaFreeHost(c->tick_h_out);
  if (c->tick_d_in) cudaFree(c->tick_d_in);
  if (c->tick_d_out) cudaFree(c->tick_d_out);
  c->tick_h_in = c->tick_h_out = c->tick_d_in = c->tick_d_out = nullptr;
  c->tick_in_floats = c->tick_out_floats = 0;
  c->tick_key.clear();
}
}

extern "C" int dsmppi_tick(dsmppi_ctx* c, dsmppi_tick_args* t, void* stream) {
  REQUIRE(c && t, "null argument");
  const dsmppi_rollout_args& r = t->rollout;
  REQUIRE(r.N >= 1 && r.H >= 1 && t->n_obs >= 1, "N, H and n_obs must be positive");
  REQUIRE(t->q_cur_host && t->obs_host && t->all_traj_host && t->closest_dist_all_host && t->kernel_val_all_host &&
              t->dot_products_host && t->kernel_activations_host && t->qdot_host && t->nn_grad_all_host,
          "null host pointer");
  REQUIRE(r.n_kernels == 0 || (t->mu_tmp_host && t->sigma_tmp_host && t->alpha_tmp_host), "null policy pointer");
  REQUIRE(r.mod.ds_kind != DSMPPI_DS_SEDS && r.distance_provider == DSMPPI_DISTANCE_NN,
          "the graphed tick covers the linear / matrix nominal DS with the network distance");
  CUDA_TRY(cudaSetDevice(c->device));
  REQUIRE(resolve_mode(c, c->pass1_mode, t->n_obs) == DSMPPI_PASS1_EXACT_FP32,
          "the graphed tick needs the dense fp32 scoring path (few obstacles)");
  REQUIRE(!c->timing, "kernel timing events cannot be recorded into a graph");
  cudaStream_t caller = static_cast<cudaStream_t>(stream);
  if (!c->s_tick) {
    CUDA_TRY(cudaStreamCreateWithFlags(&c->s_tick, cudaStreamNonBlocking));
    CUDA_TRY(cudaEventCreateWithFlags(&c->tick_ev, cudaEventDisableTiming));
  }
  const TickLayout L = tick_layout(c, r, t->n_obs);
  const size_t d = c->d, N = r.N, H = r.H, P1 = c->P + 1;
  dsmppi_rollout_args k = r;
  k.q_cur_dev = k.mu_tmp_dev = k.sigma_tmp_dev = k.alpha_tmp_dev = nullptr;
  k.all_traj_dev = k.closest_dist_all_dev = k.kernel_val_all_dev = k.dot_products_dev = k.kernel_activations_dev = nullptr;
  k.qdot_dev = k.nn_grad_all_dev = k.norm_basis_dev = nullptr;
  std::vector<unsigned char> key(sizeof(k) + sizeof(int32_t) + 3 * sizeof(int));
  std::memcpy(key.data(), &k, sizeof(k));
  std::memcpy(key.data() + sizeof(k), &t->n_obs, sizeof(int32_t));
  const int modes[3] = {c->pass1_mode, c->score_mode, c->fused_rollout};
  std::memcpy(key.data() + sizeof(k) + sizeof(int32_t), modes, sizeof(modes));
  const bool rebuild = !c->tick_exec || key != c->tick_key;
  t->recaptured = rebuild ? 1 : 0;
  if (rebuild) {
    CUDA_TRY(cudaStreamSynchronize(c->s_tick));
    if (L.in_total != c->tick_in_floats || L.out_total != c->tick_out_floats) {
      tick_free(c);
      CUDA_TRY(cudaMallocHost(reinterpret_cast<void**>(&c->tick_h_in), L.in_total * sizeof(float)));
      CUDA_TRY(cudaMallocHost(reinterpret_cast<void**>(&c->tick_h_out), L.out_total * sizeof(float)));
      CUDA_TRY(cudaMalloc(reinterpret_cast<void**>(&c->tick_d_in), L.in_total * sizeof(float)));
      CUDA_TRY(cudaMalloc(reinterpret_cast<void**>(&c->tick_d_out), L.out_total * sizeof(float)));
      std::memset(c->tick_h_in, 0, L.in_total * sizeof(float));
      c->tick_in_floats = L.in_total; c->tick_out_floats = L.out_total;
    } else {
      if (c->tick_exec) cudaGraphExecDestroy(c->tick_exec);
      if (c->tick_graph) cudaGraphDestroy(c->tick_graph);
      c->tick_exec = nullptr; c->tick_graph = nullptr;
    }
    CUDA_TRY(cudaMemset(c->tick_d_out, 0, L.out_total * sizeof(float)));
    CUDA_TRY(cudaDeviceSynchronize());
  }
  float* hi = c->tick_h_in;
  std::memcpy(hi + L.q, t->q_cur_host, (r.q_cur_is_batch ? N * d : d) * sizeof(float));
  std::memcpy(hi + L.obs, t->obs_host, (size_t)t->n_obs * P1 * sizeof(float));
  if (r.n_kernels > 0) {
    std::memcpy(hi + L.mu, t->mu_tmp_host, N * NKMAX * d * sizeof(float));
    std::memcpy(hi + L.sg, t->sigma_tmp_host, N * NKMAX * sizeof(float));
    std::memcpy(hi + L.al, t->alpha_tmp_host, N * NKMAX * d * sizeof(float));
  }
  dsmppi_rollout_args a = r;
  float* di = c->tick_d_in; float* do_ = c->tick_d_out;
  a.q_cur_dev = di + L.q; a.mu_tmp_dev = di + L.mu; a.sigma_tmp_dev = di + L.sg; a.alpha_tmp_dev = di + L.al;
  a.all_traj_dev = do_ + L.tr; a.closest_dist_all_dev = do_ + L.cd; a.kernel_val_all_dev = do_ + L.kv;
  a.dot_products_dev = do_ + L.dp; a.kernel_activations_dev = do_ + L.ka; a.qdot_dev = do_ + L.qd;
  a.nn_grad_all_dev = do_ + L.gr; a.norm_basis_dev = nullptr;
  auto sequence = [&](cudaStream_t st) -> int {
    CUDA_TRY(cudaMemcpyAsync(di, hi, L.in_total * sizeof(float), cudaMemcpyHostToDevice, st));
    if (dsmppi_set_obstacles(c, di + L.obs, t->n_obs, st)) return 1;
    if (dsmppi_rollout(c, &a, st)) return 1;
    CUDA_TRY(cudaMemcpyAsync(c->tick_h_out, do_, L.out_total * sizeof(float), cudaMemcpyDeviceToHost, st));
    return 0;
  };
  CUDA_TRY(cudaEventRecord(c->tick_ev, caller));
  CUDA_TRY(cudaStreamWaitEvent(c->s_tick, c->tick_ev, 0));
  if (rebuild) {
    if (sequence(c->s_tick)) return 1;
    CUDA_TRY(cudaStreamSynchronize(c->s_tick));
    CUDA_TRY(cudaStreamBeginCapture(c->s_tick, cudaStreamCaptureModeThreadLocal));
    const int rc = sequence(c->s_tick);
    cudaGraph_t g = nullptr;
    const cudaError_t e = cudaStreamEndCapture(c->s_tick, &g);
    if (rc || e != cudaSuccess) {
      if (g) cudaGraphDestroy(g);
      if (!rc) dsmppi_set_error(std::string("cudaStreamEndCapture: ") + cudaGetErrorString(e));
      return 1;
    }
    c->tick_graph = g;
    CUDA_TRY(cudaGraphInstantiate(&c->tick_exec, g, 0));
    c->tick_key = key;
  }
  CUDA_TRY(cudaGraphLaunch(c->tick_exec, c->s_tick));
  CUDA_TRY(cudaStreamSynchronize(c->s_tick));
  const float* ho = c->tick_h_out;
  std::memcpy(t->all_traj_host, ho + L.tr, N * H * d * sizeof(float));
  std::memcpy(t->closest_dist_all_host, ho + L.cd, N * H * sizeof(float));
  std::memcpy(t->dot_products_host, ho + L.dp, N * H * sizeof(float));
  std::memcpy(t->kernel_activations_host, ho + L.ka, N * H * sizeof(float));
  std::memcpy(t->qdot_host, ho + L.qd, N * d * sizeof(float));
  std::memcpy(t->nn_grad_all_host, ho + L.gr, N * H * d * sizeof(float));
  std::memcpy(t->kernel_val_all_host, ho + L.kv, N * H * NKMAX * sizeof(float));
  return 0;
}
```

### optimalmodulationds_b200/csrc/internal.cuh

```cuda
#pragma once
#include <cuda_runtime.h>
#include <stdint.h>
#include <string>
#include <vector>

#include "dsmppi_b200.h"

#define HID DSMPPI_HIDDEN
#define MAXL DSMPPI_MAX_HIDDEN_LAYERS
#define MAXD DSMPPI_MAX_DOF
#define MAXO DSMPPI_MAX_LINKS
#define MAXK DSMPPI_MAX_CLOSEST
#define NKMAX DSMPPI_N_KERNEL_MAX
#define CAND_MAX 16
#define N_COUNTERS 16

void dsmppi_set_error(const std::string& msg);

#define CUDA_TRY(expr)                                                                     \
  do {                                                                                     \
    cudaError_t _e = (expr);                                                               \
    if (_e != cudaSuccess) {                                                               \
      dsmppi_set_error(std::string(#expr) + ": " + cudaGetErrorString(_e) + " (" __FILE__ + \
                       ":" + std::to_string(__LINE__) + ")");                              \
      return 1;                                                                            \
    }                                                                                      \
  } while (0)

#define REQUIRE(cond, msg)                                    \
  do {                                                        \
    if (!(cond)) {                                            \
      dsmppi_set_error(std::string(msg) + " [" #cond "]");    \
      return 2;                                               \
    }                                                         \
  } while (0)

struct NetDev {
  int d;
  int nin;
  int nenc;
  int O;
  float scale;
  int nh;
  int width;
  const float* Wf[4];
  const float* Wb[4];
  const float* W4;
  const float* b[5];
};

enum { ROWS_DENSE = 0, ROWS_SELECTED = 1, ROWS_LIST = 2 };
struct RowSrc {
  int mode;
  int M;
  int K;
  int n_rows;
  const int* n_rows_dev;
  const int* sel;
  const int* row_sample;
  const int* row_obs;
  const int* out_row;
};

struct DhTable { float v[MAXD + 1][4]; };

struct dsmppi_ctx {
  int device = 0;
  int d = 0, O = 0, nin = 0, nenc = 0;
  int P = 3;
  int capacity = 0;
  int M = 0;
  int pass1_mode = DSMPPI_PASS1_AUTO;
  float guard_band = 0.f;
  float band_cal[2] = {0.f, 0.f};
  int band_cal_M[2] = {0, 0};
  float band_cal_err[2] = {0.f, 0.f};
  NetDev net{};
  DhTable dh{};
  float* weights_blob = nullptr;
  void* tc_blob = nullptr;
  size_t tc_blob_bytes = 0;
  void* tcx_blob = nullptr;
  int* fix_list = nullptr; size_t fix_cap = 0;
  int fix_parity = 0;
  int score_mode = DSMPPI_SCORE_AUTO;
  float* obs = nullptr; int obs_cap = 0;
  float* obs_raw = nullptr; int obs_raw_cap = 0;
  void* obs_enc = nullptr; size_t obs_enc_cap = 0;
  float* seds = nullptr; int seds_G = 0; float seds_thr = 0.f;
  int ws_n = 0, ws_M = 0;
  int ws_mode = -1;
  size_t cand_rows_want = 0;
  int* counters_host = nullptr;
  int obs_tables_dirty = 1;
  int pass1_hacc = 1;
  int half_tiles = 1;
  int prefilter_used = 0;
  int64_t capacity_retries = 0;
  int64_t exact_fallbacks = 0;
  float* q_work = nullptr;
  float* m_rows = nullptr;
  size_t m_rows_cap = 0;
  float* mdist = nullptr;
  size_t mdist_cap = 0;
  void* enc_q = nullptr; size_t enc_q_cap = 0;
  int* cand_cnt = nullptr;
  int* row_base = nullptr;
  int* row_sample = nullptr; int* row_obs = nullptr; size_t rowlist_cap = 0;
  int* counters = nullptr;
  int* sel = nullptr;
  int* sel_rows = nullptr;
  float* row_dist = nullptr;
  float* row_grad = nullptr;
  size_t row_dist_cap = 0, row_grad_cap = 0;
  float* dist_tmp = nullptr;
  float* grad_tmp = nullptr;
  float* upd_partials = nullptr; int upd_blocks = 0;
  float* stats_tmp = nullptr;
  float* stats_part = nullptr;
  unsigned int* stats_ticket = nullptr;
  float* packed_tmp = nullptr;
  float* stage = nullptr; size_t stage_cap = 0;
  int64_t launches = 0;
  int sm_count = 148;
  int timing = 0;
  std::vector<cudaEvent_t> ev;
  int ev_used = 0;
  int ev_kind = 0;
  int fused_rollout = 1;
  cudaStream_t s_in = nullptr, s_out = nullptr;
  std::vector<cudaEvent_t> pipe_ev;
  cudaStream_t s_tick = nullptr; cudaEvent_t tick_ev = nullptr;
  cudaGraph_t tick_graph = nullptr; cudaGraphExec_t tick_exec = nullptr;
  std::vector<unsigned char> tick_key;
  float* tick_h_in = nullptr; float* tick_h_out = nullptr; float* tick_d_in = nullptr; float* tick_d_out = nullptr;
  size_t tick_in_floats = 0, tick_out_floats = 0;
  int keep_counters = 0;
};

int launch_exact_forward(dsmppi_ctx* c, const float* q, int q_stride, const RowSrc& src, uint32_t ignore_mask,
                         float* m_rows, cudaStream_t st);
int launch_exact_fwdbwd(dsmppi_ctx* c, const float* q, int q_stride, const RowSrc& src, uint32_t ignore_mask,
                        float* m_rows, float* row_dist, float* row_grad, long long rows_estimate, cudaStream_t st);
int launch_rollout_fused(dsmppi_ctx* c, const dsmppi_rollout_args* a, cudaStream_t st);
int launch_exact_fixup(dsmppi_ctx* c, const float* q, int q_stride, const RowSrc& src, uint32_t ignore_mask,
                       float* m_rows, float* row_dist, float* row_grad, bool bwd, cudaStream_t st);
int tcx_build_images(dsmppi_ctx* c, const dsmppi_net* frame);
void tcx_free_images(dsmppi_ctx* c);
int launch_tc_exact(dsmppi_ctx* c, const float* q, int q_stride, const RowSrc& src, uint32_t ignore_mask, float* m_rows,
                    float* row_dist, float* row_grad, bool bwd, cudaStream_t st);
int launch_tc_rollout(dsmppi_ctx* c, const dsmppi_rollout_args* a, cudaStream_t st);
inline bool use_tc_scoring(const dsmppi_ctx* c) { return c->tcx_blob && c->score_mode != DSMPPI_SCORE_FFMA; }
int tc_build_images(dsmppi_ctx* c, const dsmppi_net* frame);
void tc_free_images(dsmppi_ctx* c);
int tc_set_obstacles(dsmppi_ctx* c, cudaStream_t st);
int tc_pass1(dsmppi_ctx* c, const float* q, int q_stride, int n, uint32_t ignore_mask, int mode, cudaStream_t st,
             bool table_ready = false);
int tc_reserve_sample_table(dsmppi_ctx* c, int n);
int tc_sample_table(dsmppi_ctx* c, const float* q, int q_stride, int n, int mode, cudaStream_t st);
int launch_rank_dense(dsmppi_ctx* c, int n, int K, bool rows_out, cudaStream_t st);
int launch_identity_rows(dsmppi_ctx* c, int n, int K, cudaStream_t st);
int launch_pack_obstacles(dsmppi_ctx* c, const float* raw, int M, int P, cudaStream_t st);
int launch_select_candidates(dsmppi_ctx* c, int n, int K, float band, size_t cap_rows, cudaStream_t st);
int launch_max_abs_diff(dsmppi_ctx* c, const float* a, const float* b, long long n, float* out, cudaStream_t st);
int exact_set_attributes();
inline size_t cand_list_cap(const dsmppi_ctx* c, int n) {
  const size_t base = (size_t)n * (CAND_MAX + (c->pass1_hacc ? CAND_MAX / 2 : 0));
  return base > c->cand_rows_want ? base : c->cand_rows_want;
}
int launch_rank_candidates(dsmppi_ctx* c, int n, int K, cudaStream_t st);
int launch_blend(dsmppi_ctx* c, int n, int K, float* dist_out, float* grad_out, cudaStream_t st);
int launch_step(dsmppi_ctx* c, const dsmppi_rollout_args* a, int t, cudaStream_t st);
int launch_rank_step(dsmppi_ctx* c, const dsmppi_rollout_args* a, int t, int table_mode, cudaStream_t st);
int launch_init_traj(dsmppi_ctx* c, const dsmppi_rollout_args* a, cudaStream_t st);
int launch_cost(dsmppi_ctx* c, const dsmppi_cost_args* a, cudaStream_t st);
int launch_basis(dsmppi_ctx* c, const float* grad, int64_t n, float* basis, cudaStream_t st);
int launch_fk_distance(dsmppi_ctx* c, const float* q, int q_stride, int n, int n_pts, const float* span_host,
                       float* dist, float* grad, int grad_stride, int* idx, cudaStream_t st);
int launch_cost_stats(dsmppi_ctx* c, const float* cost, int N, float* stats, cudaStream_t st);
int launch_update_partial(dsmppi_ctx* c, const dsmppi_update_args* a, const float* stats, float* packed,
                          cudaStream_t st);
int launch_update_finalize(dsmppi_ctx* c, const dsmppi_update_args* a, const float* packed, int* n_updated,
                           cudaStream_t st);
int launch_kernel_candidates(dsmppi_ctx* c, const dsmppi_candidates_args* a, cudaStream_t st);
```

### optimalmodulationds_b200/csrc/tc_pass1.cu

```cuda
#include <cuda_bf16.h>
#include <cuda_fp16.h>

#include <cstdlib>
#include <cstring>
#include <type_traits>
#include <utility>
#include <vector>

#include "internal.cuh"
#include "l1_table.cuh"

namespace {

constexpr int ROWS = 128;
constexpr int NHID = 3;
constexpr int MMA_WARP = 8;
constexpr int NTHREADS = 12 * 32;
constexpr int ROW_REGS = 232, ISSUER_REGS = 40;

constexpr int OFF_WH = 0;
constexpr int SZ_WHH = 64 * HID * 2;
constexpr int OFF_W5 = OFF_WH + NHID * 2 * SZ_WHH;
constexpr int SZ_W5 = 16 * HID * 2;
constexpr int OFF_BIAS = OFF_W5 + SZ_W5;
constexpr int SZ_BIAS = (NHID * HID + 16) * 4;
constexpr int IMG_BYTES = OFF_BIAS + SZ_BIAS;
constexpr int OFF_BAR = IMG_BYTES;
constexpr int NBAR = 20;
constexpr int OFF_TMEMPTR = OFF_BAR + NBAR * 8;
constexpr int OFF_MBUF = OFF_TMEMPTR + 16;
constexpr int OFF_BIASH = OFF_MBUF + 2 * 2 * ROWS * 4;
constexpr int OFF_ABUF = OFF_BIASH + NHID * HID * 2;
constexpr int SMEM_BYTES = OFF_ABUF + 8 * 2 * 32 * 16;
static_assert(IMG_BYTES % 16 == 0, "bulk copies need 16-byte granularity");
static_assert(SMEM_BYTES <= 232448, "exceeds the 227 KB shared-memory budget");

enum { BAR_W = 0, BAR_AREADY0 = 1, BAR_AREADY1 = 2, BAR_DFREE0 = 3, BAR_DFREE1 = 4,
       BAR_DFULL00 = 5, BAR_DFULL01 = 6, BAR_DFULL10 = 7, BAR_DFULL11 = 8,
       BAR_MFULL = 9,
       BAR_MEMPTY = 13 };

constexpr uint32_t TM_A0 = 0, TM_A1 = 128, TM_DLO = 256, TM_DHI = 384;

struct TcImages {
  uint8_t* img[2];
};

__device__ __forceinline__ uint32_t smem_u32(const void* p) { return (uint32_t)__cvta_generic_to_shared(p); }
__device__ __forceinline__ uint32_t cluster_ctarank() {
  uint32_t r;
  asm volatile("mov.u32 %0, %%cluster_ctarank;" : "=r"(r));
  return r;
}
__device__ __forceinline__ void cluster_sync_all() {
  asm volatile("barrier.cluster.arrive.release.aligned;\n\tbarrier.cluster.wait.acquire.aligned;" ::: "memory");
}
__device__ __forceinline__ void mbar_init(uint32_t bar, uint32_t count) {
  asm volatile("mbarrier.init.shared::cta.b64 [%0], %1;" ::"r"(bar), "r"(count));
}
__device__ __forceinline__ void mbar_arrive_local(uint32_t bar) {
  asm volatile("mbarrier.arrive.shared::cta.b64 _, [%0];" ::"r"(bar) : "memory");
}
__device__ __forceinline__ void mbar_expect_tx(uint32_t bar, uint32_t bytes) {
  asm volatile("mbarrier.arrive.expect_tx.shared::cta.b64 _, [%0], %1;" ::"r"(bar), "r"(bytes) : "memory");
}
__device__ __forceinline__ bool mbar_try_wait(uint32_t bar, uint32_t parity) {
  uint32_t ok;
  asm volatile(
      "{\n\t.reg .pred p;\n\t"
      "mbarrier.try_wait.parity.shared::cta.b64 p, [%1], %2;\n\t"
      "selp.u32 %0, 1, 0, p;\n\t}"
      : "=r"(ok)
      : "r"(bar), "r"(parity)
      : "memory");
  return ok != 0;
}
__device__ __forceinline__ void mbar_wait(uint32_t bar, uint32_t parity) {
  if (mbar_try_wait(bar, parity)) return;
  const long long t0 = clock64();
  while (!mbar_try_wait(bar, parity)) {
    if (clock64() - t0 > 4000000000LL) __trap();
  }
}
__device__ __forceinline__ void mbar_arrive_remote(uint32_t bar, uint32_t rank) {
  asm volatile(
      "{\n\t.reg .b32 ra;\n\t"
      "mapa.shared::cluster.u32 ra, %0, %1;\n\t"
      "mbarrier.arrive.shared::cluster.b64 _, [ra];\n\t}" ::"r"(bar),
      "r"(rank)
      : "memory");
}
__device__ __forceinline__ void bulk_g2s(uint32_t dst, const void* src, uint32_t bytes, uint32_t bar) {
  asm volatile("cp.async.bulk.shared::cluster.global.mbarrier::complete_tx::bytes [%0], [%1], %2, [%3];" ::"r"(dst),
               "l"(src), "r"(bytes), "r"(bar)
               : "memory");
}
__device__ __forceinline__ void tc_fence_before() { asm volatile("tcgen05.fence::before_thread_sync;" ::: "memory"); }
__device__ __forceinline__ void tc_fence_after() { asm volatile("tcgen05.fence::after_thread_sync;" ::: "memory"); }
__device__ __forceinline__ void tc_wait_ld() { asm volatile("tcgen05.wait::ld.sync.aligned;" ::: "memory"); }
__device__ __forceinline__ void tc_wait_st() { asm volatile("tcgen05.wait::st.sync.aligned;" ::: "memory"); }

__device__ __forceinline__ void tmem_alloc_512(uint32_t dst_smem) {
  asm volatile("tcgen05.alloc.cta_group::2.sync.aligned.shared::cta.b32 [%0], 512;" ::"r"(dst_smem) : "memory");
  asm volatile("tcgen05.relinquish_alloc_permit.cta_group::2.sync.aligned;" ::: "memory");
}
__device__ __forceinline__ void tmem_free_512(uint32_t taddr) {
  asm volatile("tcgen05.dealloc.cta_group::2.sync.aligned.b32 %0, 512;" ::"r"(taddr) : "memory");
}

__device__ __forceinline__ void mma_ts_2cta(uint32_t d_tmem, uint32_t a_tmem, uint64_t b_desc, uint32_t idesc,
                                            uint32_t accumulate) {
  asm volatile(
      "{\n\t.reg .pred p;\n\t"
      "setp.ne.b32 p, %4, 0;\n\t"
      "tcgen05.mma.cta_group::2.kind::f16 [%0], [%1], %2, %3, p;\n\t}" ::"r"(d_tmem),
      "r"(a_tmem), "l"(b_desc), "r"(idesc), "r"(accumulate)
      : "memory");
}
template <uint32_t D_COL, uint32_t A_COL, uint32_t DESC_IMM, uint32_t DESC_HI, uint32_t IDESC, bool ACC>
__device__ __forceinline__ void mma_ts_2cta_imm(uint32_t tmem_base, uint32_t sb4) {
  asm volatile(
      "{\n\t.reg .pred p;\n\t.reg .b64 bd;\n\t.reg .b32 dl, td, ta;\n\t"
      "add.u32 td, %0, %2;\n\t"
      "add.u32 ta, %0, %3;\n\t"
      "add.u32 dl, %1, %4;\n\t"
      "mov.b64 bd, {dl, %5};\n\t"
      "setp.ne.b32 p, %7, 0;\n\t"
      "tcgen05.mma.cta_group::2.kind::f16 [td], [ta], bd, %6, p;\n\t}" ::"r"(tmem_base),
      "r"(sb4), "n"(D_COL), "n"(A_COL), "n"(DESC_IMM), "n"(DESC_HI), "n"(IDESC), "n"(ACC ? 1 : 0)
      : "memory");
}
template <uint32_t D_COL, uint32_t A_COL, uint32_t B_OFF, uint32_t LBO, uint32_t IDESC, int... KS>
__device__ __forceinline__ void mma_group(uint32_t tmem_base, uint32_t sb4, std::integer_sequence<int, KS...>) {
  constexpr uint32_t DESC_HI = (128u >> 4) | (1u << 14);
  (mma_ts_2cta_imm<D_COL, A_COL + KS * 8, (B_OFF >> 4) + ((LBO >> 4) << 16) + KS * ((2 * LBO) >> 4), DESC_HI, IDESC,
                   (KS > 0)>(tmem_base, sb4), ...);
}
__device__ __forceinline__ bool elect_one() {
  uint32_t pred;
  asm volatile(
      "{\n\t.reg .pred p;\n\t"
      "elect.sync _|p, 0xffffffff;\n\t"
      "selp.u32 %0, 1, 0, p;\n\t}"
      : "=r"(pred));
  return pred != 0;
}
__device__ __forceinline__ void mma_commit_2cta(uint32_t bar) {
  asm volatile(
      "tcgen05.commit.cta_group::2.mbarrier::arrive::one.shared::cluster.multicast::cluster.b64 [%0], %1;" ::"r"(bar),
      "h"((uint16_t)3)
      : "memory");
}

#define R8(v, o) "=r"(v[o + 0]), "=r"(v[o + 1]), "=r"(v[o + 2]), "=r"(v[o + 3]), "=r"(v[o + 4]), "=r"(v[o + 5]), "=r"(v[o + 6]), "=r"(v[o + 7])
#define W8(v, o) "r"(v[o + 0]), "r"(v[o + 1]), "r"(v[o + 2]), "r"(v[o + 3]), "r"(v[o + 4]), "r"(v[o + 5]), "r"(v[o + 6]), "r"(v[o + 7])

__device__ __forceinline__ void tmem_ld32(uint32_t taddr, uint32_t (&v)[32]) {
  asm volatile(
      "tcgen05.ld.sync.aligned.32x32b.x32.b32 "
      "{%0,%1,%2,%3,%4,%5,%6,%7,%8,%9,%10,%11,%12,%13,%14,%15,%16,%17,%18,%19,%20,%21,%22,%23,%24,%25,%26,%27,%28,%29,%30,%31}, [%32];"
      : R8(v, 0), R8(v, 8), R8(v, 16), R8(v, 24)
      : "r"(taddr)
      : "memory");
}
__device__ __forceinline__ void tmem_ld32p(uint32_t taddr, uint32_t (&v)[32]) {
  asm volatile(
      "tcgen05.ld.sync.aligned.32x32b.x32.pack::16b.b32 "
      "{%0,%1,%2,%3,%4,%5,%6,%7,%8,%9,%10,%11,%12,%13,%14,%15,%16,%17,%18,%19,%20,%21,%22,%23,%24,%25,%26,%27,%28,%29,%30,%31}, [%32];"
      : R8(v, 0), R8(v, 8), R8(v, 16), R8(v, 24)
      : "r"(taddr)
      : "memory");
}
__device__ __forceinline__ void tmem_ld16(uint32_t taddr, uint32_t (&v)[16]) {
  asm volatile(
      "tcgen05.ld.sync.aligned.32x32b.x16.b32 {%0,%1,%2,%3,%4,%5,%6,%7,%8,%9,%10,%11,%12,%13,%14,%15}, [%16];"
      : R8(v, 0), R8(v, 8)
      : "r"(taddr)
      : "memory");
}
template <int OFF, int N>
__device__ __forceinline__ void tmem_st32(uint32_t taddr, const uint32_t (&v)[N]) {
  static_assert(OFF + 32 <= N, "out of range");
  asm volatile(
      "tcgen05.st.sync.aligned.32x32b.x32.b32 [%32], "
      "{%0,%1,%2,%3,%4,%5,%6,%7,%8,%9,%10,%11,%12,%13,%14,%15,%16,%17,%18,%19,%20,%21,%22,%23,%24,%25,%26,%27,%28,%29,%30,%31};" ::
          W8(v, OFF + 0), W8(v, OFF + 8), W8(v, OFF + 16), W8(v, OFF + 24), "r"(taddr)
      : "memory");
}

template <bool BF16>
__device__ __forceinline__ uint32_t pack2(float lo, float hi) {
  uint32_t r;
  if (BF16) asm("cvt.rn.bf16x2.f32 %0, %1, %2;" : "=r"(r) : "f"(hi), "f"(lo));
  else asm("cvt.rn.satfinite.f16x2.f32 %0, %1, %2;" : "=r"(r) : "f"(hi), "f"(lo));
  return r;
}
template <bool BF16>
__device__ __forceinline__ uint32_t pack2_relu(uint32_t lo, uint32_t hi) {
  uint32_t r;
  if (BF16) asm("cvt.rn.relu.bf16x2.f32 %0, %1, %2;" : "=r"(r) : "f"(__uint_as_float(hi)), "f"(__uint_as_float(lo)));
  else asm("cvt.rn.relu.satfinite.f16x2.f32 %0, %1, %2;" : "=r"(r) : "f"(__uint_as_float(hi)), "f"(__uint_as_float(lo)));
  return r;
}
__device__ __forceinline__ void add2(uint32_t a0, uint32_t a1, float b0, float b1, uint32_t& s0, uint32_t& s1) {
  asm("{\n\t.reg .b64 x, y, z;\n\t"
      "mov.b64 x, {%2, %3};\n\t"
      "mov.b64 y, {%4, %5};\n\t"
      "add.rn.f32x2 z, x, y;\n\t"
      "mov.b64 {%0, %1}, z;\n\t}"
      : "=r"(s0), "=r"(s1)
      : "r"(a0), "r"(a1), "r"(__float_as_uint(b0)), "r"(__float_as_uint(b1)));
}

__device__ __forceinline__ uint64_t make_b_desc(uint32_t smem_addr, uint32_t lbo_bytes, uint32_t sbo_bytes) {
  uint64_t d = 0;
  d |= (uint64_t)((smem_addr >> 4) & 0x3FFF);
  d |= (uint64_t)((lbo_bytes >> 4) & 0x3FFF) << 16;
  d |= (uint64_t)((sbo_bytes >> 4) & 0x3FFF) << 32;
  d |= (uint64_t)1 << 46;
  return d;
}
__host__ __device__ constexpr uint32_t make_idesc(int fmt , int M, int N, bool acc_f32 = true) {
  return (acc_f32 ? (1u << 4) : 0u) | ((uint32_t)fmt << 7) | ((uint32_t)fmt << 10) | ((uint32_t)(N >> 3) << 17) |
         ((uint32_t)(M >> 4) << 24);
}

template <bool BF16>
__global__ void __launch_bounds__(HID) l1_table_kernel(const float* __restrict__ x, int x_stride, int n, int ncomp,
                                                       int comp0, int nin, const float* __restrict__ Wf0,
                                                       const float* __restrict__ bias, int transposed, int M,
                                                       uint16_t* __restrict__ out) {
  const int i = blockIdx.x, k = threadIdx.x;
  __shared__ float xs[3 * MAXD];
  if (k < ncomp) {
    const float v = x[(size_t)i * x_stride + k];
    float sn, cs;
    sincosf(v, &sn, &cs);
    xs[3 * k] = v; xs[3 * k + 1] = sn; xs[3 * k + 2] = cs;
  }
  __syncthreads();
  const float acc = l1_feature(Wf0, bias, k, xs, ncomp, comp0, nin);
  const size_t o = transposed ? ((size_t)(k >> 3) * M + i) * 8 + (k & 7) : (size_t)i * HID + k;
  out[o] = l1_to_half_bits(acc, BF16);
  (void)n;
}

struct TcArgs {
  const uint8_t* img0; const uint8_t* img1;
  const uint4* tabA; const uint4* tabB;
  const float* obs;
  float* mdist;
  long long n_rows;
  int n, M, O;
  uint32_t ignore_mask;
  float inv_scale_div;
  uint32_t zero;
  int use_writers;
  long long* prof;
  int* nonfinite;
};

#ifdef DSMPPI_TC_PROF
#define PROF_DECL long long _pt = clock64(); long long _pc[8] = {0, 0, 0, 0, 0, 0, 0, 0}
#define PROF_ADD(i) do { const long long _n = clock64(); _pc[i] += _n - _pt; _pt = _n; } while (0)
#define PROF_FLUSH(a, w) do { if ((a).prof && (threadIdx.x & 31) == 0) for (int _i = 0; _i < 8; ++_i) \
    (a).prof[((size_t)blockIdx.x * 9 + (w)) * 8 + _i] = _pc[_i]; } while (0)
#else
#define PROF_DECL do { } while (0)
#define PROF_ADD(i) do { } while (0)
#define PROF_FLUSH(a, w) do { } while (0)
#endif

template <bool BF16, int OFF, int NPK>
__device__ __forceinline__ void relu_pack32(const uint32_t (&v)[32], const float* __restrict__ bias32,
                                            uint32_t (&pk)[NPK]) {
  const float4* b4 = reinterpret_cast<const float4*>(bias32);
#pragma unroll
  for (int k = 0; k < 8; ++k) {
    const float4 bb = b4[k];
    uint32_t s0, s1, s2, s3;
    add2(v[4 * k + 0], v[4 * k + 1], bb.x, bb.y, s0, s1);
    add2(v[4 * k + 2], v[4 * k + 3], bb.z, bb.w, s2, s3);
    pk[OFF + 2 * k + 0] = pack2_relu<BF16>(s0, s1);
    pk[OFF + 2 * k + 1] = pack2_relu<BF16>(s2, s3);
  }
}

template <int OFF, int BOFF, int NPK>
__device__ __forceinline__ void relu_h2_32(const uint32_t (&v)[32], const uint4 (&b)[16], uint32_t (&pk)[NPK]) {
  const uint32_t one = 0x3c003c00u;
#pragma unroll
  for (int k = 0; k < 8; ++k) {
    const uint4 bb = b[BOFF + k];
    asm("fma.rn.relu.f16x2 %0, %1, %2, %3;" : "=r"(pk[OFF + 4 * k + 0]) : "r"(v[4 * k + 0]), "r"(one), "r"(bb.x));
    asm("fma.rn.relu.f16x2 %0, %1, %2, %3;" : "=r"(pk[OFF + 4 * k + 1]) : "r"(v[4 * k + 1]), "r"(one), "r"(bb.y));
    asm("fma.rn.relu.f16x2 %0, %1, %2, %3;" : "=r"(pk[OFF + 4 * k + 2]) : "r"(v[4 * k + 2]), "r"(one), "r"(bb.z));
    asm("fma.rn.relu.f16x2 %0, %1, %2, %3;" : "=r"(pk[OFF + 4 * k + 3]) : "r"(v[4 * k + 3]), "r"(one), "r"(bb.w));
  }
}
__device__ __forceinline__ void load_bias16(const uint4* __restrict__ src, uint4 (&b)[16]) {
  const uint32_t sa = smem_u32(src);
#pragma unroll
  for (int k = 0; k < 16; ++k)
    asm volatile("ld.shared.v4.u32 {%0, %1, %2, %3}, [%4];"
                 : "=r"(b[k].x), "=r"(b[k].y), "=r"(b[k].z), "=r"(b[k].w) : "r"(sa + 16u * k));
}

template <bool BF16>
__device__ __forceinline__ uint32_t add_relu_h2(uint32_t a, uint32_t b) {
  uint32_t r;
  if (BF16) asm("fma.rn.relu.bf16x2 %0, %1, %2, %3;" : "=r"(r) : "r"(a), "r"(0x3f803f80u), "r"(b));
  else asm("fma.rn.relu.f16x2 %0, %1, %2, %3;" : "=r"(r) : "r"(a), "r"(0x3c003c00u), "r"(b));
  return r;
}

__device__ __forceinline__ uint4 ldg_nc_v4(const uint4* p) {
  uint4 v;
  asm volatile("ld.global.nc.v4.u32 {%0, %1, %2, %3}, [%4];" : "=r"(v.x), "=r"(v.y), "=r"(v.z), "=r"(v.w) : "l"(p));
  return v;
}

template <bool BF16>
__device__ __forceinline__ void first_layer(const TcArgs& a, int i, int j, uint32_t dep, uint32_t (&pk)[128]) {
  if (i < a.n) {
    const uint4* ta = a.tabA + (size_t)i * 32 + dep;
    const uint4* tb = a.tabB + j + dep;
    const uint32_t strideM = (uint32_t)a.M + dep;
#pragma unroll
    for (int hf = 0; hf < 2; ++hf) {
      uint4 x[16], y[16];
#pragma unroll
      for (int kb = 0; kb < 16; ++kb) {
        x[kb] = ldg_nc_v4(ta + 16 * hf + kb);
        y[kb] = ldg_nc_v4(tb + (size_t)((16 * hf + kb) * strideM));
      }
#pragma unroll
      for (int kb = 0; kb < 16; ++kb) {
        pk[64 * hf + 4 * kb + 0] = add_relu_h2<BF16>(x[kb].x, y[kb].x);
        pk[64 * hf + 4 * kb + 1] = add_relu_h2<BF16>(x[kb].y, y[kb].y);
        pk[64 * hf + 4 * kb + 2] = add_relu_h2<BF16>(x[kb].z, y[kb].z);
        pk[64 * hf + 4 * kb + 3] = add_relu_h2<BF16>(x[kb].w, y[kb].w);
      }
      if (hf == 0) {
        const uint32_t d2 = (pk[3] | pk[11] | pk[19] | pk[27] | pk[35] | pk[43] | pk[51] | pk[59] | pk[63]) & a.zero;
        ta += d2;
        tb += d2;
      }
    }
  } else {
#pragma unroll
    for (int k = 0; k < 128; ++k) pk[k] = 0u;
  }
}
struct TableLoads {
  uint4 y[32];
  uint4 a0, a1;
  int i0;
};
__device__ __forceinline__ void first_layer_issue(const TcArgs& a, int i, int j, uint32_t dep, int lane, TableLoads& t) {
  t.i0 = __shfl_sync(0xffffffffu, i, 0);
  const uint4* ta = a.tabA + dep;
  t.a0 = ldg_nc_v4(ta + (size_t)min(t.i0, a.n - 1) * 32 + lane);
  t.a1 = ldg_nc_v4(ta + (size_t)min(t.i0 + 1, a.n - 1) * 32 + lane);
  const uint4* tb = a.tabB + j + dep;
  const uint32_t strideM = (uint32_t)a.M + dep;
#pragma unroll
  for (int kb = 0; kb < 32; ++kb) t.y[kb] = ldg_nc_v4(tb + (size_t)(kb * strideM));
}
template <bool BF16>
__device__ __forceinline__ void first_layer_finish(const TcArgs& a, int i, const TableLoads& t, uint4* abuf, int lane,
                                                   uint32_t (&pk)[128]) {
  abuf[lane] = t.a0;
  abuf[32 + lane] = t.a1;
  __syncwarp();
  const uint4* ar = abuf + (i - t.i0) * 32;
#pragma unroll
  for (int kb = 0; kb < 32; ++kb) {
    const uint4 x = ar[kb];
    pk[4 * kb + 0] = add_relu_h2<BF16>(x.x, t.y[kb].x);
    pk[4 * kb + 1] = add_relu_h2<BF16>(x.y, t.y[kb].y);
    pk[4 * kb + 2] = add_relu_h2<BF16>(x.z, t.y[kb].z);
    pk[4 * kb + 3] = add_relu_h2<BF16>(x.w, t.y[kb].w);
  }
  __syncwarp();
}
__device__ __forceinline__ void store_operand(uint32_t tA, const uint32_t (&pk)[128]) {
  tmem_st32<0>(tA, pk);
  tmem_st32<32>(tA + 32, pk);
  tmem_st32<64>(tA + 64, pk);
  tmem_st32<96>(tA + 96, pk);
}

template <bool BF16, bool HACC = false, bool ASM = false>
__global__ void __cluster_dims__(2, 1, 1) __launch_bounds__(NTHREADS, 1)
tc_pass1_kernel(const __grid_constant__ TcArgs a) {
  static_assert(!(BF16 && HACC), "bf16 operands accumulate in fp32");
  extern __shared__ __align__(1024) uint8_t smem[];
  const uint32_t sbase = smem_u32(smem);
  const uint32_t bar0 = sbase + OFF_BAR;
  auto BAR = [&](int i) { return bar0 + (uint32_t)i * 8u; };
  const float* bias = reinterpret_cast<const float*>(smem + OFF_BIAS);
  volatile uint32_t* tmem_ptr_smem = reinterpret_cast<volatile uint32_t*>(smem + OFF_TMEMPTR);

  const int tid = threadIdx.x;
  const int warp = tid >> 5, lane = tid & 31;
  const uint32_t rank = cluster_ctarank();
  const int pair = blockIdx.x >> 1, npairs = gridDim.x >> 1;

  float* mbuf = reinterpret_cast<float*>(smem + OFF_MBUF);
  if (warp == MMA_WARP) {
    if (lane == 0) {
      mbar_init(BAR(BAR_W), 1);
      mbar_init(BAR(BAR_AREADY0), 8);
      mbar_init(BAR(BAR_AREADY1), 8);
      mbar_init(BAR(BAR_DFREE0), 8);
      mbar_init(BAR(BAR_DFREE1), 8);
      for (int i = BAR_DFULL00; i <= BAR_DFULL11; ++i) mbar_init(BAR(i), 1);
      for (int i = 0; i < 4; ++i) { mbar_init(BAR(BAR_MFULL + i), 4); mbar_init(BAR(BAR_MEMPTY + i), 1); }
      asm volatile("fence.mbarrier_init.release.cluster;" ::: "memory");
    }
    __syncwarp();
    tmem_alloc_512(smem_u32((const void*)tmem_ptr_smem));
    if (lane == 0) {
      const uint8_t* img = rank == 0 ? a.img0 : a.img1;
      mbar_expect_tx(BAR(BAR_W), IMG_BYTES);
      constexpr int CH = 32768;
      for (int off = 0; off < IMG_BYTES; off += CH) {
        const int n = IMG_BYTES - off < CH ? IMG_BYTES - off : CH;
        bulk_g2s(sbase + off, img + off, n, BAR(BAR_W));
      }
    }
  }
  tc_fence_before();
  __syncthreads();
  tc_fence_after();
  const uint32_t tmem_base = *tmem_ptr_smem;
  mbar_wait(BAR(BAR_W), 0);
  if constexpr (HACC) {
    uint32_t* bh = reinterpret_cast<uint32_t*>(smem + OFF_BIASH);
    for (int k = tid; k < NHID * HID / 2; k += NTHREADS) bh[k] = pack2<false>(bias[2 * k], bias[2 * k + 1]);
    __syncthreads();
  }
  cluster_sync_all();

  const long long n_tiles = (a.n_rows + 2 * ROWS - 1) / (2 * ROWS);

  if (warp < MMA_WARP) {
    asm volatile("setmaxnreg.inc.sync.aligned.u32 %0;" ::"n"(ROW_REGS));
    const int slot = warp >> 2;
    const int row = ((warp & 3) << 5) | lane;
    const uint32_t lane_addr = (uint32_t)((warp & 3) * 32) << 16;
    const uint32_t tA = tmem_base + lane_addr + (slot ? TM_A1 : TM_A0);
    const uint32_t tDlo = tmem_base + lane_addr + TM_DLO, tDhi = tmem_base + lane_addr + TM_DHI;
    const uint32_t bar_aready = BAR(slot ? BAR_AREADY1 : BAR_AREADY0);
    const uint32_t bar_full_lo = BAR(slot ? BAR_DFULL10 : BAR_DFULL00);
    const uint32_t bar_full_hi = BAR(slot ? BAR_DFULL11 : BAR_DFULL01);
    uint4* abuf = reinterpret_cast<uint4*>(smem + OFF_ABUF) + warp * 64;

    auto signal = [&](uint32_t bar) {
      tc_fence_before();
      __syncwarp();
      if (lane == 0) mbar_arrive_remote(bar, 0);
    };
    const long long stride = 2LL * npairs * (2 * ROWS);
    const int di = (int)(stride / a.M), dj = (int)(stride % a.M);
    const long long r0 = ((long long)slot * npairs + pair) * (2 * ROWS) + (long long)rank * ROWS + row;
    int i_cur = (int)min(r0 / a.M, (long long)a.n), j_cur = (int)(r0 % a.M);
    if ((long long)pair < n_tiles) {
      uint32_t pk[128];
      if constexpr (ASM) {
        TableLoads t;
        first_layer_issue(a, i_cur, j_cur, a.zero, lane, t);
        first_layer_finish<BF16>(a, i_cur, t, abuf, lane, pk);
      } else {
        first_layer<BF16>(a, i_cur, j_cur, a.zero, pk);
      }
      store_operand(tA, pk);
      tc_wait_st();
      signal(bar_aready);
    }
    PROF_DECL;
    for (long long it = 0;; ++it) {
      const long long tX = (it * 2) * npairs + pair;
      if (tX >= n_tiles) break;
      const bool more = ((it + 1) * 2) * npairs + pair < n_tiles;
      int i_next = min(i_cur + di, a.n), j_next = j_cur + dj;
      if (j_next >= a.M) { j_next -= a.M; i_next = min(i_next + 1, a.n); }
      uint32_t tile_dep = 0;
      auto hacc_layer = [&](auto L) {
        constexpr int l = decltype(L)::value;
        PROF_ADD(7);
        uint32_t pk[64], raw[2][32];
        const uint4* bsm = reinterpret_cast<const uint4*>(smem + OFF_BIASH) + l * (HID / 8);
        uint4 bq[16];
        load_bias16(bsm, bq);
        mbar_wait(bar_full_lo, (uint32_t)(l & 1));
        tc_fence_after();
        PROF_ADD(0);
        tmem_ld32p(tDlo, raw[0]);
        tmem_ld32p(tDlo + 64, raw[1]);
        tc_wait_ld();
        signal(BAR(BAR_DFREE0));
        PROF_ADD(1);
        relu_h2_32<0, 0>(raw[0], bq, pk);
        relu_h2_32<32, 8>(raw[1], bq, pk);
        PROF_ADD(2);
        load_bias16(bsm + 16, bq);
        mbar_wait(bar_full_hi, (uint32_t)((it + l) & 1));
        tc_fence_after();
        PROF_ADD(3);
        tmem_ld32p(tDhi, raw[0]);
        tmem_ld32p(tDhi + 64, raw[1]);
        tmem_st32<0>(tA, pk);
        tmem_st32<32>(tA + 32, pk);
        tc_wait_ld();
        signal(BAR(BAR_DFREE1));
        PROF_ADD(4);
        relu_h2_32<0, 0>(raw[0], bq, pk);
        relu_h2_32<32, 8>(raw[1], bq, pk);
        tmem_st32<0>(tA + 64, pk);
        tmem_st32<32>(tA + 96, pk);
        tc_wait_st();
        signal(bar_aready);
        if (l == NHID - 1) tile_dep = (pk[7] | pk[23] | pk[39] | pk[63]) & a.zero;
        PROF_ADD(5);
      };
      if constexpr (HACC) {
        hacc_layer(std::integral_constant<int, 0>{});
        hacc_layer(std::integral_constant<int, 1>{});
        hacc_layer(std::integral_constant<int, 2>{});
        static_assert(NHID == 3, "three hidden GEMMs");
      } else {
#pragma unroll
      for (int l = 0; l < NHID; ++l) {
        const float* bl = bias + l * HID;
        PROF_ADD(7);
        uint32_t pk[64], raw[4][32];
        mbar_wait(bar_full_lo, (uint32_t)(l & 1));
        tc_fence_after();
        PROF_ADD(0);
        tmem_ld32(tDlo, raw[0]);
        tmem_ld32(tDlo + 32, raw[1]);
        tmem_ld32(tDlo + 64, raw[2]);
        tmem_ld32(tDlo + 96, raw[3]);
        tc_wait_ld();
        signal(BAR(BAR_DFREE0));
        PROF_ADD(1);
        relu_pack32<BF16, 0>(raw[0], bl, pk);
        relu_pack32<BF16, 16>(raw[1], bl + 32, pk);
        relu_pack32<BF16, 32>(raw[2], bl + 64, pk);
        relu_pack32<BF16, 48>(raw[3], bl + 96, pk);
        PROF_ADD(2);
        mbar_wait(bar_full_hi, (uint32_t)((it + l) & 1));
        tc_fence_after();
        PROF_ADD(3);
        tmem_ld32(tDhi, raw[0]);
        tmem_ld32(tDhi + 32, raw[1]);
        tmem_ld32(tDhi + 64, raw[2]);
        tmem_ld32(tDhi + 96, raw[3]);
        tmem_st32<0>(tA, pk);
        tmem_st32<32>(tA + 32, pk);
        tc_wait_ld();
        signal(BAR(BAR_DFREE1));
        PROF_ADD(4);
        relu_pack32<BF16, 0>(raw[0], bl + 128, pk);
        relu_pack32<BF16, 16>(raw[1], bl + 160, pk);
        relu_pack32<BF16, 32>(raw[2], bl + 192, pk);
        relu_pack32<BF16, 48>(raw[3], bl + 224, pk);
        tmem_st32<0>(tA + 64, pk);
        tmem_st32<32>(tA + 96, pk);
        tc_wait_st();
        signal(bar_aready);
        if (l == NHID - 1) tile_dep = (pk[7] | pk[23] | pk[39] | pk[63]) & a.zero;
        PROF_ADD(5);
      }
      }
      const bool valid = i_cur < a.n;
      float rad = 0.f;
      if (valid) rad = __ldg(a.obs + (size_t)j_cur * 4 + 3);
      auto finish_tile = [&](const uint32_t (&v)[16]) {
        float m = 3.0e38f;
        if (valid) {
          bool finite = true;
#pragma unroll
          for (int o = 0; o < 16; ++o) {
            if (o < a.O) {
              float y = __uint_as_float(v[o]) + bias[NHID * HID + o];
              finite = finite && (fabsf(y) <= 3.0e38f);
              y = y / a.inv_scale_div - rad;
              if ((a.ignore_mask >> o) & 1u) y = 1e6f;
              m = fminf(m, y);
            }
          }
          if (!finite) {
            m = -3.0e38f;
            atomicAdd(a.nonfinite, 1);
          }
        }
        if (a.use_writers) {
          const int b = (int)(it & 1);
          if (it >= 2) mbar_wait(BAR(BAR_MEMPTY + slot * 2 + b), (uint32_t)(((it >> 1) - 1) & 1));
          mbuf[(slot * 2 + b) * ROWS + row] = m;
          __syncwarp();
          if (lane == 0) mbar_arrive_local(BAR(BAR_MFULL + slot * 2 + b));
        } else if (valid) {
          a.mdist[(size_t)i_cur * a.M + j_cur] = m;
        }
      };
      uint32_t v[16];
      if (more) {
        uint32_t nxt[128];
        if constexpr (ASM) {
          TableLoads t;
          first_layer_issue(a, i_next, j_next, tile_dep, lane, t);
          first_layer_finish<BF16>(a, i_next, t, abuf, lane, nxt);
        } else {
          first_layer<BF16>(a, i_next, j_next, tile_dep, nxt);
        }
        PROF_ADD(6);
        mbar_wait(bar_full_lo, 1u);
        tc_fence_after();
        PROF_ADD(0);
        tmem_ld16(tDlo, v);
        store_operand(tA, nxt);
        tc_wait_ld();
        signal(BAR(BAR_DFREE0));
        tc_wait_st();
        signal(bar_aready);
        finish_tile(v);
      } else {
        PROF_ADD(6);
        mbar_wait(bar_full_lo, 1u);
        tc_fence_after();
        PROF_ADD(0);
        tmem_ld16(tDlo, v);
        tc_wait_ld();
        signal(BAR(BAR_DFREE0));
        finish_tile(v);
      }
      i_cur = i_next;
      j_cur = j_next;
      PROF_ADD(6);
    }
    PROF_FLUSH(a, warp);
  } else {
    asm volatile("setmaxnreg.dec.sync.aligned.u32 %0;" ::"n"(ISSUER_REGS));
  }
  if (warp == MMA_WARP && rank == 0) {
    constexpr int fmt = BF16 ? 1 : 0;
    constexpr uint32_t idesc128 = make_idesc(fmt, 256, 128, !HACC);
    constexpr uint32_t idesc32 = make_idesc(fmt, 256, 32);
    const uint32_t sb4 = sbase >> 4;
    uint32_t ph_a[2] = {0, 0}, ph_free[2] = {0, 0};
    PROF_DECL;
    auto group = [&](auto L, auto S, auto H) {
      constexpr int l = decltype(L)::value, s = decltype(S)::value, h = decltype(H)::value;
      PROF_ADD(2);
      mbar_wait(BAR(h ? BAR_DFREE1 : BAR_DFREE0), ph_free[h] ^ 1);
      ph_free[h] ^= 1;
      tc_fence_after();
      PROF_ADD(1);
      constexpr uint32_t boff = l < NHID ? OFF_WH + (l * 2 + h) * SZ_WHH : OFF_W5;
      constexpr uint32_t lbo = l < NHID ? 64 * 16 : 16 * 16;
      constexpr int ksteps = HID / 16;
      constexpr uint32_t idesc = l < NHID ? idesc128 : idesc32;
      constexpr uint32_t dcol = h ? TM_DHI : TM_DLO, acol = s ? TM_A1 : TM_A0;
      if (elect_one()) {
        mma_group<dcol, acol, boff, lbo, idesc>(tmem_base, sb4, std::make_integer_sequence<int, ksteps>{});
        mma_commit_2cta(BAR(BAR_DFULL00 + s * 2 + h));
      }
      __syncwarp();
    };
    auto step = [&](auto S, auto L) {
      constexpr int l = decltype(L)::value, s = decltype(S)::value;
      PROF_ADD(2);
      mbar_wait(BAR(s ? BAR_AREADY1 : BAR_AREADY0), ph_a[s]);
      ph_a[s] ^= 1;
      tc_fence_after();
      PROF_ADD(0);
      group(L, S, std::integral_constant<int, 0>{});
      if constexpr (l < NHID) group(L, S, std::integral_constant<int, 1>{});
    };
    using I0 = std::integral_constant<int, 0>;
    using I1 = std::integral_constant<int, 1>;
    using I2 = std::integral_constant<int, 2>;
    using I3 = std::integral_constant<int, 3>;
    const long long n_it = (n_tiles - pair + 2LL * npairs - 1) / (2LL * npairs);
    if (n_it > 0) {
      step(I0{}, I0{});
      step(I0{}, I1{});
    }
    for (long long it = 0; it < n_it; ++it) {
      const bool more = it + 1 < n_it;
      step(I0{}, I2{}); step(I1{}, I0{});
      step(I0{}, I3{}); step(I1{}, I1{});
      if (more) step(I0{}, I0{});
      step(I1{}, I2{});
      if (more) step(I0{}, I1{});
      step(I1{}, I3{});
    }
    PROF_ADD(2);
    PROF_FLUSH(a, MMA_WARP);
  }
  if ((warp == MMA_WARP + 1 || warp == MMA_WARP + 2) && a.use_writers) {
    const int slot = warp - (MMA_WARP + 1);
    for (long long it = 0;; ++it) {
      const long long tX = (it * 2) * npairs + pair;
      if (tX >= n_tiles) break;
      const long long tile = (it * 2 + slot) * npairs + pair;
      const int b = (int)(it & 1);
      mbar_wait(BAR(BAR_MFULL + slot * 2 + b), (uint32_t)((it >> 1) & 1));
      float vals[4];
#pragma unroll
      for (int w = 0; w < 4; ++w) vals[w] = mbuf[(slot * 2 + b) * ROWS + 32 * w + lane];
      __syncwarp();
      if (lane == 0) mbar_arrive_local(BAR(BAR_MEMPTY + slot * 2 + b));
      const long long r0 = tile * (2 * ROWS) + (long long)rank * ROWS;
#pragma unroll
      for (int w = 0; w < 4; ++w) {
        const long long r = r0 + 32 * w + lane;
        if (r < a.n_rows) a.mdist[r] = vals[w];
      }
    }
  }
  tc_fence_before();
  __syncthreads();
  cluster_sync_all();
  if (warp == MMA_WARP) {
    __syncwarp();
    tmem_free_512(tmem_base);
  }
}

uint16_t f2h(float f) {
  __half h = __float2half_rn(f);
  uint16_t u;
  std::memcpy(&u, &h, 2);
  return u;
}
uint16_t f2bf(float f) {
  __nv_bfloat16 h = __float2bfloat16_rn(f);
  uint16_t u;
  std::memcpy(&u, &h, 2);
  return u;
}

inline size_t canon(int n, int k, int rows) {
  return (size_t)(k / 8) * rows * 16 + (size_t)(n / 8) * 128 + (size_t)(n % 8) * 16 + (size_t)(k % 8) * 2;
}

}

int tc_build_images(dsmppi_ctx* c, const dsmppi_net* net) {
  c->tc_blob = nullptr;
  if (c->O > 16) return 0;
  const char* dis = std::getenv("DSMPPI_DISABLE_TC");
  if (dis && dis[0] == '1') return 0;
  TcImages* t = new TcImages();
  uint8_t* dev = nullptr;
  if (cudaMalloc(reinterpret_cast<void**>(&dev), (size_t)4 * IMG_BYTES) != cudaSuccess) {
    dsmppi_set_error("cudaMalloc(tc images) failed");
    delete t;
    return 1;
  }
  std::vector<uint8_t> host((size_t)4 * IMG_BYTES, 0);
  for (int fmt = 0; fmt < 2; ++fmt)
    for (int rank = 0; rank < 2; ++rank) {
      uint8_t* img = host.data() + (size_t)(fmt * 2 + rank) * IMG_BYTES;
      auto put = [&](size_t off, float v) {
        const uint16_t u = fmt ? f2bf(v) : f2h(v);
        std::memcpy(img + off, &u, 2);
      };
      for (int h = 0; h < 2; ++h)
        for (int n = 0; n < 64; ++n) {
          const int feat = 128 * h + 64 * rank + n;
          for (int l = 0; l < NHID; ++l)
            for (int k = 0; k < HID; ++k)
              put(OFF_WH + (l * 2 + h) * SZ_WHH + canon(n, k, 64), net->W_host[l + 1][(size_t)feat * HID + k]);
        }
      for (int n = 0; n < 16; ++n) {
        const int o = 16 * rank + n;
        for (int k = 0; k < HID; ++k)
          put(OFF_W5 + canon(n, k, 16), o < c->O ? net->W_host[4][(size_t)o * HID + k] : 0.f);
      }
      float* bias = reinterpret_cast<float*>(img + OFF_BIAS);
      for (int l = 0; l < NHID; ++l)
        for (int k = 0; k < HID; ++k) bias[l * HID + k] = net->b_host[l + 1][k];
      for (int o = 0; o < 16; ++o) bias[NHID * HID + o] = o < c->O ? net->b_host[4][o] : 0.f;
    }
  CUDA_TRY(cudaMemcpy(dev, host.data(), host.size(), cudaMemcpyHostToDevice));
  t->img[0] = dev;
  t->img[1] = nullptr;
  c->tc_blob = t;
  c->tc_blob_bytes = host.size();
  auto opt_in = [](auto kernel) {
    return cudaFuncSetAttribute(kernel, cudaFuncAttributeMaxDynamicSharedMemorySize, SMEM_BYTES);
  };
  CUDA_TRY(opt_in(tc_pass1_kernel<false, false, false>));
  CUDA_TRY(opt_in(tc_pass1_kernel<false, false, true>));
  CUDA_TRY(opt_in(tc_pass1_kernel<true, false, false>));
  CUDA_TRY(opt_in(tc_pass1_kernel<true, false, true>));
  CUDA_TRY(opt_in(tc_pass1_kernel<false, true, false>));
  CUDA_TRY(opt_in(tc_pass1_kernel<false, true, true>));
  return 0;
}

void tc_free_images(dsmppi_ctx* c) {
  if (!c->tc_blob) return;
  TcImages* t = static_cast<TcImages*>(c->tc_blob);
  if (t->img[0]) cudaFree(t->img[0]);
  delete t;
  c->tc_blob = nullptr;
}

int tc_set_obstacles(dsmppi_ctx* c, cudaStream_t st) {
  const size_t need = (size_t)2 * c->M * HID * 2;
  if (need > c->obs_enc_cap) {
    if (c->obs_enc) CUDA_TRY(cudaFree(c->obs_enc));
    c->obs_enc = nullptr;
    CUDA_TRY(cudaMalloc(&c->obs_enc, need));
    c->obs_enc_cap = need;
  }
  uint16_t* out = static_cast<uint16_t*>(c->obs_enc);
  l1_table_kernel<false><<<c->M, HID, 0, st>>>(c->obs, 4, c->M, c->P, c->d, c->nin, c->net.Wf[0], nullptr, 1, c->M, out);
  l1_table_kernel<true><<<c->M, HID, 0, st>>>(c->obs, 4, c->M, c->P, c->d, c->nin, c->net.Wf[0], nullptr, 1, c->M,
                                              out + (size_t)c->M * HID);
  CUDA_TRY(cudaGetLastError());
  c->launches += 2;
  return 0;
}

int tc_reserve_sample_table(dsmppi_ctx* c, int n) {
  const size_t need = (size_t)n * HID * 2;
  if (need > c->enc_q_cap) {
    if (c->enc_q) CUDA_TRY(cudaFree(c->enc_q));
    c->enc_q = nullptr;
    CUDA_TRY(cudaMalloc(&c->enc_q, need + need / 8));
    c->enc_q_cap = need + need / 8;
  }
  return 0;
}

int tc_sample_table(dsmppi_ctx* c, const float* q, int q_stride, int n, int mode, cudaStream_t st) {
  const bool bf16 = mode == DSMPPI_PASS1_TC_BF16;
  if (tc_reserve_sample_table(c, n)) return 1;
  uint16_t* ta = static_cast<uint16_t*>(c->enc_q);
  if (bf16) l1_table_kernel<true><<<n, HID, 0, st>>>(q, q_stride, n, c->d, 0, c->nin, c->net.Wf[0], c->net.b[0], 0, 0, ta);
  else l1_table_kernel<false><<<n, HID, 0, st>>>(q, q_stride, n, c->d, 0, c->nin, c->net.Wf[0], c->net.b[0], 0, 0, ta);
  CUDA_TRY(cudaGetLastError());
  c->launches++;
  return 0;
}

int tc_pass1(dsmppi_ctx* c, const float* q, int q_stride, int n, uint32_t ignore_mask, int mode, cudaStream_t st,
             bool table_ready) {
  REQUIRE(c->tc_blob, "tensor-core images not built");
  TcImages* t = static_cast<TcImages*>(c->tc_blob);
  const bool bf16 = mode == DSMPPI_PASS1_TC_BF16;
  if (c->obs_tables_dirty) {
    if (tc_set_obstacles(c, st)) return 1;
    c->obs_tables_dirty = 0;
  }
  if (!table_ready && tc_sample_table(c, q, q_stride, n, mode, st)) return 1;
  TcArgs a;
  const uint8_t* base = t->img[0] + (size_t)(bf16 ? 2 : 0) * IMG_BYTES;
  a.img0 = base;
  a.img1 = base + IMG_BYTES;
  a.tabA = reinterpret_cast<const uint4*>(c->enc_q);
  a.tabB = reinterpret_cast<const uint4*>(static_cast<uint16_t*>(c->obs_enc) + (bf16 ? (size_t)c->M * HID : 0));
  a.obs = c->obs;
  a.mdist = c->mdist;
  a.n_rows = (long long)n * c->M;
  a.n = n;
  a.M = c->M;
  a.O = c->O;
  a.ignore_mask = ignore_mask;
  a.inv_scale_div = (c->O == 9) ? 100.f : 1.f;
  a.zero = 0u;
  a.use_writers = 1;
  a.nonfinite = c->counters + 9;
  a.prof = nullptr;
#ifdef DSMPPI_TC_PROF
  a.prof = reinterpret_cast<long long*>(c->stage);
#endif
  const long long n_tiles = (a.n_rows + 2 * ROWS - 1) / (2 * ROWS);
  long long pairs = c->sm_count / 2;
  if (pairs > (n_tiles + 1) / 2) pairs = (n_tiles + 1) / 2;
  if (pairs < 1) pairs = 1;
  const dim3 grid((unsigned)(2 * pairs));
  const bool stage_a = c->M >= 32;
  auto launch = [&](auto kernel) { kernel<<<grid, NTHREADS, SMEM_BYTES, st>>>(a); };
  if (bf16) stage_a ? launch(tc_pass1_kernel<true, false, true>) : launch(tc_pass1_kernel<true, false, false>);
  else if (c->pass1_hacc) stage_a ? launch(tc_pass1_kernel<false, true, true>) : launch(tc_pass1_kernel<false, true, false>);
  else stage_a ? launch(tc_pass1_kernel<false, false, true>) : launch(tc_pass1_kernel<false, false, false>);
  CUDA_TRY(cudaGetLastError());
  c->launches++;
  return 0;
}
```

Measured before the change: 1.715 million.

## Reorder hidden features by firing rate and skip all-zero tail K-steps in pass1

On first use, a sampling kernel counts how often each hidden unit fires over a subset of sample/obstacle pairs. The hidden units are then permuted so rarely-active ones sit in the last K-steps, and the tensor-core weight images are rebuilt to match. Activation warps test whether the tail K-chunks of each tile are entirely zero and send a liveness mask to the MMA warp over the cluster using st.async. The MMA warp predicates off tcgen05.mma issues for dead K-steps, which should cut tensor-core work in the prefilter at the cost of extra signalling, a one-time host round-trip, and counter atomics.

```diff
diff --git a/include/dsmppi_b200.h b/include/dsmppi_b200.h
--- a/include/dsmppi_b200.h
+++ b/include/dsmppi_b200.h
@@ -253,6 +253,7 @@
 int64_t dsmppi_launch_count(const dsmppi_ctx* ctx);
 int dsmppi_pass1_stats(dsmppi_ctx* ctx, int64_t* rescored_pairs, int64_t* band_overflows, int32_t* mode,
                        void* stream);
+int dsmppi_pass1_ksteps(dsmppi_ctx* ctx, int64_t* issued, int64_t* possible, void* stream);
 int dsmppi_exactness_stats(dsmppi_ctx* ctx, int64_t* capacity_retries, int64_t* exact_fallbacks, float* guard_band,
                            float* calibration_error);
 int dsmppi_score_stats(dsmppi_ctx* ctx, int32_t* mode, int64_t* range_fixup_rows, int64_t* dropped_rows, void* stream);
diff --git a/optimalmodulationds_b200/MPPI.py b/optimalmodulationds_b200/MPPI.py
--- a/optimalmodulationds_b200/MPPI.py
+++ b/optimalmodulationds_b200/MPPI.py
@@ -663,7 +663,11 @@
         a, b, m = _capi.C.c_int64(), _capi.C.c_int64(), _capi.C.c_int32()
         _capi.check(self._lib.dsmppi_pass1_stats(self._ctx, _capi.C.byref(a), _capi.C.byref(b), _capi.C.byref(m),
                                                  self._stream()))
-        return dict(rescored_pairs=a.value, band_overflows=b.value, mode=m.value)
+        issued, possible = _capi.C.c_int64(), _capi.C.c_int64()
+        _capi.check(self._lib.dsmppi_pass1_ksteps(self._ctx, _capi.C.byref(issued), _capi.C.byref(possible),
+                                                  self._stream()))
+        return dict(rescored_pairs=a.value, band_overflows=b.value, mode=m.value, issued_ksteps=issued.value,
+                    possible_ksteps=possible.value)
 
     def debug_pass1(self, q, mode='exact'):
         code = {'exact': _capi.PASS1_EXACT_FP32, 'tc_f16': _capi.PASS1_TC_F16, 'tc_bf16': _capi.PASS1_TC_BF16}[mode]
diff --git a/optimalmodulationds_b200/_capi.py b/optimalmodulationds_b200/_capi.py
--- a/optimalmodulationds_b200/_capi.py
+++ b/optimalmodulationds_b200/_capi.py
@@ -144,6 +144,7 @@
     "dsmppi_launch_count": (C.c_int64, [C.c_void_p]),
     "dsmppi_pass1_stats": (C.c_int, [C.c_void_p, C.POINTER(C.c_int64), C.POINTER(C.c_int64), C.POINTER(C.c_int32),
                                      C.c_void_p]),
+    "dsmppi_pass1_ksteps": (C.c_int, [C.c_void_p, C.POINTER(C.c_int64), C.POINTER(C.c_int64), C.c_void_p]),
     "dsmppi_exactness_stats": (C.c_int, [C.c_void_p, C.POINTER(C.c_int64), C.POINTER(C.c_int64), C.POINTER(C.c_float),
                                          C.POINTER(C.c_float)]),
     "dsmppi_score_stats": (C.c_int, [C.c_void_p, C.POINTER(C.c_int32), C.POINTER(C.c_int64), C.POINTER(C.c_int64),
diff --git a/optimalmodulationds_b200/csrc/capi.cu b/optimalmodulationds_b200/csrc/capi.cu
--- a/optimalmodulationds_b200/csrc/capi.cu
+++ b/optimalmodulationds_b200/csrc/capi.cu
@@ -175,7 +175,7 @@
 extern "C" {
 
 const char* dsmppi_last_error(void) { return g_last_error.c_str(); }
-int dsmppi_version(void) { return 102; }
+int dsmppi_version(void) { return 103; }
 
 void dsmppi_modulation_default(dsmppi_modulation* m) {
   if (!m) return;
@@ -274,6 +274,7 @@
   if (tcx_build_images(c, fnet)) { delete c; return 1; }
   if (const char* e = std::getenv("DSMPPI_HALF_TILES")) c->half_tiles = std::atoi(e) != 0;
   if (const char* e = std::getenv("DSMPPI_PASS1_ACC")) c->pass1_hacc = std::strcmp(e, "f32") != 0;
+  if (const char* e = std::getenv("DSMPPI_PASS1_SKIP")) c->pass1_skip = std::strcmp(e, "0") != 0;
   c->upd_blocks = c->sm_count * 4;
   CUDA_TRY(cudaMalloc(reinterpret_cast<void**>(&c->upd_partials),
                       (size_t)c->upd_blocks * dsmppi_update_packed_len(NKMAX, MAXD) * sizeof(float)));
@@ -909,6 +910,17 @@
   return 0;
 }
 
+int dsmppi_pass1_ksteps(dsmppi_ctx* c, int64_t* issued, int64_t* possible, void* stream) {
+  REQUIRE(c, "null ctx");
+  cudaStream_t st = static_cast<cudaStream_t>(stream);
+  unsigned long long host[2] = {0, 0};
+  CUDA_TRY(cudaMemcpyAsync(host, c->counters + 10, sizeof(host), cudaMemcpyDeviceToHost, st));
+  CUDA_TRY(cudaStreamSynchronize(st));
+  if (issued) *issued = (int64_t)host[0];
+  if (possible) *possible = (int64_t)host[1];
+  return 0;
+}
+
 int dsmppi_exactness_stats(dsmppi_ctx* c, int64_t* capacity_retries, int64_t* exact_fallbacks, float* guard_band,
                            float* calibration_error) {
   REQUIRE(c, "null ctx");
diff --git a/optimalmodulationds_b200/csrc/internal.cuh b/optimalmodulationds_b200/csrc/internal.cuh
--- a/optimalmodulationds_b200/csrc/internal.cuh
+++ b/optimalmodulationds_b200/csrc/internal.cuh
@@ -94,6 +94,9 @@
   int* counters_host = nullptr;
   int obs_tables_dirty = 1;
   int pass1_hacc = 1;
+  int pass1_skip = 1;
+  int pass1_ordered = 0;
+  uint32_t pass1_skip_layers = 0;
   int half_tiles = 1;
   int prefilter_used = 0;
   int64_t capacity_retries = 0;
@@ -154,6 +157,7 @@
 int tc_build_images(dsmppi_ctx* c, const dsmppi_net* frame);
 void tc_free_images(dsmppi_ctx* c);
 int tc_set_obstacles(dsmppi_ctx* c, cudaStream_t st);
+int tc_order_features(dsmppi_ctx* c, const float* q, int q_stride, int n, cudaStream_t st);
 int tc_pass1(dsmppi_ctx* c, const float* q, int q_stride, int n, uint32_t ignore_mask, int mode, cudaStream_t st,
              bool table_ready = false);
 int tc_reserve_sample_table(dsmppi_ctx* c, int n);
diff --git a/optimalmodulationds_b200/csrc/tc_pass1.cu b/optimalmodulationds_b200/csrc/tc_pass1.cu
--- a/optimalmodulationds_b200/csrc/tc_pass1.cu
+++ b/optimalmodulationds_b200/csrc/tc_pass1.cu
@@ -1,6 +1,7 @@
 #include <cuda_bf16.h>
 #include <cuda_fp16.h>
 
+#include <algorithm>
 #include <cstdlib>
 #include <cstring>
 #include <type_traits>
@@ -31,7 +32,9 @@
 constexpr int OFF_MBUF = OFF_TMEMPTR + 16;
 constexpr int OFF_BIASH = OFF_MBUF + 2 * 2 * ROWS * 4;
 constexpr int OFF_ABUF = OFF_BIASH + NHID * HID * 2;
-constexpr int SMEM_BYTES = OFF_ABUF + 8 * 2 * 32 * 16;
+constexpr int OFF_LIVE = OFF_ABUF + 8 * 2 * 32 * 16;
+constexpr int SMEM_BYTES = OFF_LIVE + 2 * 8 * 4;
+constexpr int TAIL0 = 8;
 static_assert(IMG_BYTES % 16 == 0, "bulk copies need 16-byte granularity");
 static_assert(SMEM_BYTES <= 232448, "exceeds the 227 KB shared-memory budget");
 
@@ -90,6 +93,23 @@
       "r"(rank)
       : "memory");
 }
+__device__ __forceinline__ void st_async_remote(uint32_t addr, uint32_t v, uint32_t bar, uint32_t rank) {
+  asm volatile(
+      "{\n\t.reg .b32 ra, rb;\n\t"
+      "mapa.shared::cluster.u32 ra, %0, %2;\n\t"
+      "mapa.shared::cluster.u32 rb, %1, %2;\n\t"
+      "st.async.shared::cluster.mbarrier::complete_tx::bytes.b32 [ra], %3, [rb];\n\t}" ::"r"(addr),
+      "r"(bar), "r"(rank), "r"(v)
+      : "memory");
+}
+__device__ __forceinline__ void mbar_arrive_expect_tx_remote(uint32_t bar, uint32_t rank, uint32_t bytes) {
+  asm volatile(
+      "{\n\t.reg .b32 ra;\n\t"
+      "mapa.shared::cluster.u32 ra, %0, %1;\n\t"
+      "mbarrier.arrive.expect_tx.shared::cluster.b64 _, [ra], %2;\n\t}" ::"r"(bar),
+      "r"(rank), "r"(bytes)
+      : "memory");
+}
 __device__ __forceinline__ void bulk_g2s(uint32_t dst, const void* src, uint32_t bytes, uint32_t bar) {
   asm volatile("cp.async.bulk.shared::cluster.global.mbarrier::complete_tx::bytes [%0], [%1], %2, [%3];" ::"r"(dst),
                "l"(src), "r"(bytes), "r"(bar)
@@ -118,23 +138,26 @@
       : "memory");
 }
 template <uint32_t D_COL, uint32_t A_COL, uint32_t DESC_IMM, uint32_t DESC_HI, uint32_t IDESC, bool ACC>
-__device__ __forceinline__ void mma_ts_2cta_imm(uint32_t tmem_base, uint32_t sb4) {
-  asm volatile(
-      "{\n\t.reg .pred p;\n\t.reg .b64 bd;\n\t.reg .b32 dl, td, ta;\n\t"
-      "add.u32 td, %0, %2;\n\t"
-      "add.u32 ta, %0, %3;\n\t"
-      "add.u32 dl, %1, %4;\n\t"
-      "mov.b64 bd, {dl, %5};\n\t"
-      "setp.ne.b32 p, %7, 0;\n\t"
-      "tcgen05.mma.cta_group::2.kind::f16 [td], [ta], bd, %6, p;\n\t}" ::"r"(tmem_base),
-      "r"(sb4), "n"(D_COL), "n"(A_COL), "n"(DESC_IMM), "n"(DESC_HI), "n"(IDESC), "n"(ACC ? 1 : 0)
+__device__ __forceinline__ void mma_ts_2cta_imm(uint32_t tmem_base, uint32_t sb4, uint32_t issue) {
+  asm volatile(
+      "{\n\t.reg .pred p, q;\n\t.reg .b64 bd;\n\t.reg .b32 dl, td, ta;\n\t"
+      "add.u32 td, %0, %3;\n\t"
+      "add.u32 ta, %0, %4;\n\t"
+      "add.u32 dl, %1, %5;\n\t"
+      "mov.b64 bd, {dl, %6};\n\t"
+      "setp.ne.b32 p, %8, 0;\n\t"
+      "setp.ne.b32 q, %2, 0;\n\t"
+      "@q tcgen05.mma.cta_group::2.kind::f16 [td], [ta], bd, %7, p;\n\t}" ::"r"(tmem_base),
+      "r"(sb4), "r"(issue), "n"(D_COL), "n"(A_COL), "n"(DESC_IMM), "n"(DESC_HI), "n"(IDESC), "n"(ACC ? 1 : 0)
       : "memory");
 }
 template <uint32_t D_COL, uint32_t A_COL, uint32_t B_OFF, uint32_t LBO, uint32_t IDESC, int... KS>
-__device__ __forceinline__ void mma_group(uint32_t tmem_base, uint32_t sb4, std::integer_sequence<int, KS...>) {
+__device__ __forceinline__ void mma_group(uint32_t tmem_base, uint32_t sb4, uint32_t live,
+                                          std::integer_sequence<int, KS...>) {
   constexpr uint32_t DESC_HI = (128u >> 4) | (1u << 14);
   (mma_ts_2cta_imm<D_COL, A_COL + KS * 8, (B_OFF >> 4) + ((LBO >> 4) << 16) + KS * ((2 * LBO) >> 4), DESC_HI, IDESC,
-                   (KS > 0)>(tmem_base, sb4), ...);
+                   (KS > 0)>(tmem_base, sb4, KS < TAIL0 ? 1u : (live >> (KS < TAIL0 ? 0 : KS - TAIL0)) & 1u),
+   ...);
 }
 __device__ __forceinline__ bool elect_one() {
   uint32_t pred;
@@ -258,6 +281,8 @@
   int use_writers;
   long long* prof;
   int* nonfinite;
+  uint32_t skip_layers;
+  unsigned long long* ksteps;
 };
 
 #ifdef DSMPPI_TC_PROF
@@ -304,6 +329,17 @@
   for (int k = 0; k < 16; ++k)
     asm volatile("ld.shared.v4.u32 {%0, %1, %2, %3}, [%4];"
                  : "=r"(b[k].x), "=r"(b[k].y), "=r"(b[k].z), "=r"(b[k].w) : "r"(sa + 16u * k));
+}
+
+__device__ __forceinline__ uint32_t tail_live(const uint32_t (&pk)[64]) {
+  uint32_t m = 0;
+#pragma unroll
+  for (int k = 0; k < 16 - TAIL0; ++k) {
+    const uint32_t t = pk[8 * k] | pk[8 * k + 1] | pk[8 * k + 2] | pk[8 * k + 3] | pk[8 * k + 4] | pk[8 * k + 5] |
+                       pk[8 * k + 6] | pk[8 * k + 7];
+    m |= (t != 0u ? 1u : 0u) << k;
+  }
+  return __reduce_or_sync(0xffffffffu, m);
 }
 
 template <bool BF16>
@@ -461,6 +497,22 @@
       tc_fence_before();
       __syncwarp();
       if (lane == 0) mbar_arrive_remote(bar, 0);
+    };
+    const uint32_t live_word = sbase + OFF_LIVE + (uint32_t)(slot * 8 + rank * 4 + (warp & 3)) * 4u;
+    auto signal_operand = [&](int l, const uint32_t (&pk)[64]) {
+      const bool chk = (a.skip_layers >> l) & 1u;
+      const uint32_t live = chk ? tail_live(pk) : 0u;
+      tc_wait_st();
+      tc_fence_before();
+      __syncwarp();
+      if (lane == 0) {
+        if (chk) {
+          st_async_remote(live_word, live, bar_aready, 0);
+          mbar_arrive_expect_tx_remote(bar_aready, 0, 4);
+        } else {
+          mbar_arrive_remote(bar_aready, 0);
+        }
+      }
     };
     const long long stride = 2LL * npairs * (2 * ROWS);
     const int di = (int)(stride / a.M), dj = (int)(stride % a.M);
@@ -520,8 +572,7 @@
         relu_h2_32<32, 8>(raw[1], bq, pk);
         tmem_st32<0>(tA + 64, pk);
         tmem_st32<32>(tA + 96, pk);
-        tc_wait_st();
-        signal(bar_aready);
+        signal_operand(l, pk);
         if (l == NHID - 1) tile_dep = (pk[7] | pk[23] | pk[39] | pk[63]) & a.zero;
         PROF_ADD(5);
       };
@@ -569,8 +620,7 @@
         relu_pack32<BF16, 48>(raw[3], bl + 224, pk);
         tmem_st32<0>(tA + 64, pk);
         tmem_st32<32>(tA + 96, pk);
-        tc_wait_st();
-        signal(bar_aready);
+        signal_operand(l, pk);
         if (l == NHID - 1) tile_dep = (pk[7] | pk[23] | pk[39] | pk[63]) & a.zero;
         PROF_ADD(5);
       }
@@ -652,8 +702,9 @@
     constexpr uint32_t idesc32 = make_idesc(fmt, 256, 32);
     const uint32_t sb4 = sbase >> 4;
     uint32_t ph_a[2] = {0, 0}, ph_free[2] = {0, 0};
+    uint32_t skipped = 0;
     PROF_DECL;
-    auto group = [&](auto L, auto S, auto H) {
+    auto group = [&](auto L, auto S, auto H, uint32_t live) {
       constexpr int l = decltype(L)::value, s = decltype(S)::value, h = decltype(H)::value;
       PROF_ADD(2);
       mbar_wait(BAR(h ? BAR_DFREE1 : BAR_DFREE0), ph_free[h] ^ 1);
@@ -666,7 +717,7 @@
       constexpr uint32_t idesc = l < NHID ? idesc128 : idesc32;
       constexpr uint32_t dcol = h ? TM_DHI : TM_DLO, acol = s ? TM_A1 : TM_A0;
       if (elect_one()) {
-        mma_group<dcol, acol, boff, lbo, idesc>(tmem_base, sb4, std::make_integer_sequence<int, ksteps>{});
+        mma_group<dcol, acol, boff, lbo, idesc>(tmem_base, sb4, live, std::make_integer_sequence<int, ksteps>{});
         mma_commit_2cta(BAR(BAR_DFULL00 + s * 2 + h));
       }
       __syncwarp();
@@ -677,9 +728,16 @@
       mbar_wait(BAR(s ? BAR_AREADY1 : BAR_AREADY0), ph_a[s]);
       ph_a[s] ^= 1;
       tc_fence_after();
+      uint32_t live = 0xffu;
+      if (l > 0 && ((a.skip_layers >> (l > 0 ? l - 1 : 0)) & 1u)) {
+        const uint4* w = reinterpret_cast<const uint4*>(smem + OFF_LIVE) + s * 2;
+        const uint4 x = w[0], y = w[1];
+        live = x.x | x.y | x.z | x.w | y.x | y.y | y.z | y.w;
+        skipped += (uint32_t)(l < NHID ? 2 : 1) * (uint32_t)(16 - TAIL0 - __popc(live));
+      }
       PROF_ADD(0);
-      group(L, S, std::integral_constant<int, 0>{});
-      if constexpr (l < NHID) group(L, S, std::integral_constant<int, 1>{});
+      group(L, S, std::integral_constant<int, 0>{}, live);
+      if constexpr (l < NHID) group(L, S, std::integral_constant<int, 1>{}, live);
     };
     using I0 = std::integral_constant<int, 0>;
     using I1 = std::integral_constant<int, 1>;
@@ -701,6 +759,12 @@
     }
     PROF_ADD(2);
     PROF_FLUSH(a, MMA_WARP);
+    if (lane == 0 && n_it > 0) {
+      constexpr unsigned long long per_tile = (2 * NHID + 1) * (HID / 16);
+      const unsigned long long all = (unsigned long long)n_it * 2ull * per_tile;
+      atomicAdd(a.ksteps, all - skipped);
+      atomicAdd(a.ksteps + 1, all);
+    }
   }
   if ((warp == MMA_WARP + 1 || warp == MMA_WARP + 2) && a.use_writers) {
     const int slot = warp - (MMA_WARP + 1);
@@ -747,6 +811,77 @@
 
 inline size_t canon(int n, int k, int rows) {
   return (size_t)(k / 8) * rows * 16 + (size_t)(n / 8) * 128 + (size_t)(n % 8) * 16 + (size_t)(k % 8) * 2;
+}
+
+void fill_images(uint8_t* host, int O, const float* const (&W)[4], const float* const (&b)[4], const int (&perm)[NHID][HID]) {
+  for (int fmt = 0; fmt < 2; ++fmt)
+    for (int rank = 0; rank < 2; ++rank) {
+      uint8_t* img = host + (size_t)(fmt * 2 + rank) * IMG_BYTES;
+      auto put = [&](size_t off, float v) {
+        const uint16_t u = fmt ? f2bf(v) : f2h(v);
+        std::memcpy(img + off, &u, 2);
+      };
+      for (int l = 0; l < NHID; ++l)
+        for (int h = 0; h < 2; ++h)
+          for (int n = 0; n < 64; ++n) {
+            const int feat = perm[l][128 * h + 64 * rank + n];
+            for (int k = 0; k < HID; ++k)
+              put(OFF_WH + (l * 2 + h) * SZ_WHH + canon(n, k, 64), W[l][(size_t)feat * HID + (l ? perm[l - 1][k] : k)]);
+          }
+      for (int n = 0; n < 16; ++n) {
+        const int o = 16 * rank + n;
+        for (int k = 0; k < HID; ++k) put(OFF_W5 + canon(n, k, 16), o < O ? W[3][(size_t)o * HID + perm[NHID - 1][k]] : 0.f);
+      }
+      float* bias = reinterpret_cast<float*>(img + OFF_BIAS);
+      for (int l = 0; l < NHID; ++l)
+        for (int k = 0; k < HID; ++k) bias[l * HID + k] = b[l][perm[l][k]];
+      for (int o = 0; o < 16; ++o) bias[NHID * HID + o] = o < O ? b[NHID][o] : 0.f;
+    }
+}
+
+constexpr int CNT_PAIRS = 16;
+__global__ void __launch_bounds__(HID) feature_count_kernel(const float* __restrict__ q, int q_stride, int n,
+                                                            const float* __restrict__ obs, int M, int P, NetDev net,
+                                                            long long n_pairs, unsigned* __restrict__ counts) {
+  __shared__ float h[2][CNT_PAIRS][HID];
+  __shared__ float xs[CNT_PAIRS][2][3 * MAXD];
+  const int k = threadIdx.x;
+  const long long p0 = (long long)blockIdx.x * CNT_PAIRS;
+  if (k < CNT_PAIRS) {
+    const long long r = min(p0 + k, n_pairs - 1) * ((long long)n * M) / n_pairs;
+    const int i = (int)(r / M), j = (int)(r % M);
+    for (int c = 0; c < net.d; ++c) {
+      const float v = q[(size_t)i * q_stride + c];
+      xs[k][0][3 * c] = v; xs[k][0][3 * c + 1] = sinf(v); xs[k][0][3 * c + 2] = cosf(v);
+    }
+    for (int c = 0; c < P; ++c) {
+      const float v = obs[(size_t)j * 4 + c];
+      xs[k][1][3 * c] = v; xs[k][1][3 * c + 1] = sinf(v); xs[k][1][3 * c + 2] = cosf(v);
+    }
+  }
+  __syncthreads();
+  for (int p = 0; p < CNT_PAIRS; ++p)
+    h[0][p][k] = fmaxf(l1_feature(net.Wf[0], net.b[0], k, xs[p][0], net.d, 0, net.nin) +
+                           l1_feature(net.Wf[0], nullptr, k, xs[p][1], P, net.d, net.nin), 0.f);
+  for (int l = 1; l <= NHID; ++l) {
+    __syncthreads();
+    const float (*hin)[HID] = h[(l - 1) & 1];
+    float acc[CNT_PAIRS];
+#pragma unroll
+    for (int p = 0; p < CNT_PAIRS; ++p) acc[p] = net.b[l][k];
+    for (int i = 0; i < HID; ++i) {
+      const float w = net.Wf[l][(size_t)i * HID + k];
+#pragma unroll
+      for (int p = 0; p < CNT_PAIRS; ++p) acc[p] = fmaf(w, hin[p][i], acc[p]);
+    }
+    unsigned fired = 0;
+#pragma unroll
+    for (int p = 0; p < CNT_PAIRS; ++p) {
+      h[l & 1][p][k] = fmaxf(acc[p], 0.f);
+      fired += (acc[p] > 0.f && p0 + p < n_pairs) ? 1u : 0u;
+    }
+    atomicAdd(counts + (l - 1) * HID + k, fired);
+  }
 }
 
 }
@@ -764,30 +899,12 @@
     return 1;
   }
   std::vector<uint8_t> host((size_t)4 * IMG_BYTES, 0);
-  for (int fmt = 0; fmt < 2; ++fmt)
-    for (int rank = 0; rank < 2; ++rank) {
-      uint8_t* img = host.data() + (size_t)(fmt * 2 + rank) * IMG_BYTES;
-      auto put = [&](size_t off, float v) {
-        const uint16_t u = fmt ? f2bf(v) : f2h(v);
-        std::memcpy(img + off, &u, 2);
-      };
-      for (int h = 0; h < 2; ++h)
-        for (int n = 0; n < 64; ++n) {
-          const int feat = 128 * h + 64 * rank + n;
-          for (int l = 0; l < NHID; ++l)
-            for (int k = 0; k < HID; ++k)
-              put(OFF_WH + (l * 2 + h) * SZ_WHH + canon(n, k, 64), net->W_host[l + 1][(size_t)feat * HID + k]);
-        }
-      for (int n = 0; n < 16; ++n) {
-        const int o = 16 * rank + n;
-        for (int k = 0; k < HID; ++k)
-          put(OFF_W5 + canon(n, k, 16), o < c->O ? net->W_host[4][(size_t)o * HID + k] : 0.f);
-      }
-      float* bias = reinterpret_cast<float*>(img + OFF_BIAS);
-      for (int l = 0; l < NHID; ++l)
-        for (int k = 0; k < HID; ++k) bias[l * HID + k] = net->b_host[l + 1][k];
-      for (int o = 0; o < 16; ++o) bias[NHID * HID + o] = o < c->O ? net->b_host[4][o] : 0.f;
-    }
+  int identity[NHID][HID];
+  for (int l = 0; l < NHID; ++l)
+    for (int k = 0; k < HID; ++k) identity[l][k] = k;
+  const float* const W[4] = {net->W_host[1], net->W_host[2], net->W_host[3], net->W_host[4]};
+  const float* const b[4] = {net->b_host[1], net->b_host[2], net->b_host[3], net->b_host[4]};
+  fill_images(host.data(), c->O, W, b, identity);
   CUDA_TRY(cudaMemcpy(dev, host.data(), host.size(), cudaMemcpyHostToDevice));
   t->img[0] = dev;
   t->img[1] = nullptr;
@@ -805,6 +922,60 @@
   return 0;
 }
 
+int tc_order_features(dsmppi_ctx* c, const float* q, int q_stride, int n, cudaStream_t st) {
+  TcImages* t = static_cast<TcImages*>(c->tc_blob);
+  const long long total = (long long)n * c->M;
+  const long long n_pairs = total < (1LL << 15) ? total : (1LL << 15);
+  unsigned* dcnt = nullptr;
+  CUDA_TRY(cudaMalloc(reinterpret_cast<void**>(&dcnt), NHID * HID * sizeof(unsigned)));
+  std::vector<unsigned> cnt(NHID * HID);
+  int rc = cudaMemsetAsync(dcnt, 0, NHID * HID * sizeof(unsigned), st) != cudaSuccess;
+  if (!rc) {
+    feature_count_kernel<<<(unsigned)((n_pairs + CNT_PAIRS - 1) / CNT_PAIRS), HID, 0, st>>>(q, q_stride, n, c->obs,
+                                                                                           c->M, c->P, c->net, n_pairs, dcnt);
+    rc = cudaGetLastError() != cudaSuccess;
+  }
+  if (!rc) rc = cudaMemcpyAsync(cnt.data(), dcnt, cnt.size() * sizeof(unsigned), cudaMemcpyDeviceToHost, st) != cudaSuccess;
+  if (!rc) rc = cudaStreamSynchronize(st) != cudaSuccess;
+  cudaFree(dcnt);
+  if (rc) { dsmppi_set_error("feature count of the prefilter order failed"); return 1; }
+  c->launches++;
+  int perm[NHID][HID];
+  uint32_t skip = 0;
+  for (int l = 0; l < NHID; ++l) {
+    const unsigned* cl = cnt.data() + l * HID;
+    for (int k = 0; k < HID; ++k) perm[l][k] = k;
+    std::stable_sort(perm[l], perm[l] + HID, [&](int x, int y) { return cl[x] > cl[y]; });
+    unsigned long long tail = 0;
+    for (int k = HID - 16; k < HID; ++k) tail += cl[perm[l][k]];
+    if (tail * 256 < (unsigned long long)n_pairs) skip |= 1u << l;
+  }
+  std::vector<float> W[4], b[4];
+  for (int l = 0; l < 4; ++l) {
+    W[l].resize((size_t)(l < NHID ? HID : c->O) * HID);
+    b[l].resize(l < NHID ? HID : c->O);
+    CUDA_TRY(cudaMemcpy(W[l].data(), l < NHID ? c->net.Wb[l + 1] : c->net.W4, W[l].size() * sizeof(float),
+                        cudaMemcpyDeviceToHost));
+    CUDA_TRY(cudaMemcpy(b[l].data(), c->net.b[l + 1], b[l].size() * sizeof(float), cudaMemcpyDeviceToHost));
+  }
+  std::vector<uint8_t> host((size_t)4 * IMG_BYTES, 0);
+  const float* const Wp[4] = {W[0].data(), W[1].data(), W[2].data(), W[3].data()};
+  const float* const bp[4] = {b[0].data(), b[1].data(), b[2].data(), b[3].data()};
+  fill_images(host.data(), c->O, Wp, bp, perm);
+  for (int img = 0; img < 4; ++img)
+    for (int off = OFF_WH; off < OFF_BIAS; off += 2) {
+      uint16_t u;
+      std::memcpy(&u, host.data() + (size_t)img * IMG_BYTES + off, 2);
+      const uint16_t e = img < 2 ? 0x7C00 : 0x7F80;
+      if ((u & e) == e) skip = 0;
+    }
+  CUDA_TRY(cudaMemcpyAsync(t->img[0], host.data(), host.size(), cudaMemcpyHostToDevice, st));
+  CUDA_TRY(cudaStreamSynchronize(st));
+  c->pass1_ordered = 1;
+  c->pass1_skip_layers = c->pass1_skip ? skip : 0u;
+  return 0;
+}
+
 void tc_free_images(dsmppi_ctx* c) {
   if (!c->tc_blob) return;
   TcImages* t = static_cast<TcImages*>(c->tc_blob);
@@ -857,6 +1028,7 @@
   REQUIRE(c->tc_blob, "tensor-core images not built");
   TcImages* t = static_cast<TcImages*>(c->tc_blob);
   const bool bf16 = mode == DSMPPI_PASS1_TC_BF16;
+  if (!c->pass1_ordered && tc_order_features(c, q, q_stride, n, st)) return 1;
   if (c->obs_tables_dirty) {
     if (tc_set_obstacles(c, st)) return 1;
     c->obs_tables_dirty = 0;
@@ -879,6 +1051,8 @@
   a.zero = 0u;
   a.use_writers = 1;
   a.nonfinite = c->counters + 9;
+  a.skip_layers = c->pass1_skip_layers;
+  a.ksteps = reinterpret_cast<unsigned long long*>(c->counters + 10);
   a.prof = nullptr;
 #ifdef DSMPPI_TC_PROF
   a.prof = reinterpret_cast<long long*>(c->stage);
```

Measured after the change: 1.836 million (median of 6 runs). 1.07x the previous value.
